# honglianghe/CDNet

Measured on AMD Instinct MI355X. Metric: tiles/sec (train fwd+bwd+Adam), 256x256, higher is better.
Workload: dtype fp32

## Files before the change

cdnet_amd/_lib.py:

```python
import ctypes as C
import os

_HERE = os.path.dirname(os.path.abspath(__file__))
LIB_PATH = os.environ.get('CDNET_LIB_PATH') or os.path.join(_HERE, 'libcdnet_hip.so')

_vp, _i, _sz, _f, _u = C.c_void_p, C.c_int, C.c_size_t, C.c_float, C.c_uint

class WgradReduceDesc(C.Structure):
    _fields_ = [('slab', C.c_void_p), ('dw', C.c_void_p)] + [(n, C.c_int) for n in (
        'ksplit', 'npar', 'ci_blocks', 'co_blocks', 'taps', 'CI', 'CO', 'Csrc_real', 'Cin_real', 'src_coff', 'Cout', 'mode', 'block0', 'blocks')]

class DilatedConvArgs(C.Structure):
    _fields_ = [(n, C.c_void_p) for n in ('in_', 'w', 'scale', 'shift', 'out')] + [(n, C.c_int) for n in (
        'N', 'H', 'W', 'Cin', 'in_cstride', 'Cout', 'out_cstride', 'out_coff', 'taps', 'dilation', 'leaky')] + [
        ('slope', C.c_float), ('f32', C.c_int), ('out_nchw', C.c_int)]

class DilatedBwdDataArgs(C.Structure):
    _fields_ = [(n, C.c_void_p) for n in ('g', 'w', 'dx')] + [(n, C.c_int) for n in (
        'N', 'H', 'W', 'Cout', 'g_cstride', 'Cin', 'dx_cstride', 'dx_coff', 'taps', 'dilation', 'accumulate', 'f32')]

class DilatedWgradArgs(C.Structure):
    _fields_ = [(n, C.c_void_p) for n in ('x', 'g', 'dw', 'ws')] + [('ws_bytes', C.c_size_t)] + [(n, C.c_int) for n in (
        'N', 'H', 'W', 'Cin', 'x_cstride', 'Cout', 'g_cstride', 'taps', 'dilation')]

class SliceBnFwdArgs(C.Structure):
    _fields_ = [(n, C.c_void_p) for n in ('z', 'out', 'gamma', 'beta', 'running_mean', 'running_var', 'mean', 'invstd', 'ws')] + [
        ('ws_floats', C.c_size_t), ('P', C.c_longlong)] + [(n, C.c_int) for n in ('C', 'z_cstride', 'out_cstride', 'out_coff')] + [
        (n, C.c_float) for n in ('eps', 'momentum', 'p_drop')] + [('layer', C.c_int), ('key', C.c_ulonglong)]

class SliceBnBwdArgs(C.Structure):
    _fields_ = [(n, C.c_void_p) for n in ('dy', 'z', 'mean', 'invstd', 'gamma', 'dgamma', 'dbeta', 'g', 'ws')] + [
        ('ws_floats', C.c_size_t), ('P', C.c_longlong)] + [(n, C.c_int) for n in ('C', 'z_cstride', 'dy_cstride', 'dy_coff', 'g_cstride')] + [
        (n, C.c_float) for n in ('slope', 'p_drop')] + [('layer', C.c_int), ('key', C.c_ulonglong)]


SIGNATURES = {
    'cdnet_abi_version': (_i, []),
    'cdnet_abi_sizeof': (_sz, [C.c_char_p]),
    'cdnet_last_error': (C.c_char_p, []),
    'cdnet_build_info': (C.c_char_p, []),
    'cdnet_spin': (_i, [_i, _vp]),
    'cdnet_box_copy': (_i, [_vp, _vp, _sz, _vp]),
    'cdnet_box_mfma': (_i, [_vp, _vp, _vp, _i, _i, _i, _vp]),
    'cdnet_ddm_codes': (_i, [_vp, _i, _i, _i, _i, _vp, _i, _i, _vp, _vp, _vp]),
    'cdnet_ddm_normalize': (_i, [_vp, _vp, _i, _i, _i, _vp, _vp]),
    'cdnet_probmaps': (_i, [_vp, _vp, _i, _i, _i, _i, _vp, _vp, _vp]),
    'cdnet_tta_boost_argmax': (_i, [_vp, _vp, _vp, _vp, _i, _i, _vp, _i, _i, _vp, _vp, _vp, _vp, _vp, _vp]),
    'cdnet_fuse_sum': (_i, [_vp, _i, _i, _i, _i, _i, _i, _vp, _i, _i, _vp]),
    'cdnet_upsample_bilinear_backward': (_i, [_vp, _i, _i, _i, _i, _i, _i, _i, _i, _vp, _vp]),
    'cdnet_s2d_to_nhwc': (_i, [_vp, _i, _i, _i, _i, _vp, _vp]),
    'cdnet_fuse_sum_f32': (_i, [_vp, _i, _i, _i, _i, _i, _i, _vp, _i, _i, _vp]),
    'cdnet_upsample_bilinear_backward_f32': (_i, [_vp, _i, _i, _i, _i, _i, _i, _i, _i, _vp, _vp]),
    'cdnet_s2d_to_nhwc_f32': (_i, [_vp, _i, _i, _i, _i, _vp, _vp]),
    'cdnet_bn_backward_stats': (_i, [_vp, _vp, _vp, _vp, _vp, _sz, _vp, _vp]),
    'cdnet_bn_backward_apply': (_i, [_vp, _vp, _vp, _vp]),
    'cdnet_bn_backward_finalize': (_i, [_vp, _vp, _vp, _vp, _vp, _i, _vp, _vp]),
    'cdnet_conv_ws_eligible': (_i, [_vp]),
    'cdnet_grad_sum': (_i, [_vp, _i, _vp, C.c_longlong, _i, _vp, _vp]),
    'cdnet_grad_sum_f32': (_i, [_vp, _i, _vp, C.c_longlong, _i, _vp, _vp]),
    'cdnet_label_pair_histogram': (_i, [_vp, _vp, _i, _i, _i, _i, _vp, _vp, _vp, _vp, _vp, _vp]),
    'cdnet_remap_label': (_i, [_vp, _i, _i, _i, _vp, _vp, _vp, _vp]),
    'cdnet_label_areas': (_i, [_vp, _i, _i, _i, _vp, _vp, _vp]),
    'cdnet_label_apply': (_i, [_vp, _i, _i, _i, _vp, _vp, _vp]),
    'cdnet_label_csr_workspace_bytes': (_sz, [_i]),
    'cdnet_label_csr': (_i, [_vp, _i, _i, _i, _vp, _sz, _vp, _vp, _vp, _vp, _vp]),
    'cdnet_hausdorff_tile_pixels': (_i, []),
    'cdnet_hausdorff_chunk_pixels': (_i, []),
    'cdnet_hausdorff_pairs': (_i, [_vp] * 8 + [_i, _i, _i, _vp, _i, _vp, _i, _vp, _vp, _vp]),
    'cdnet_watershed_workspace_bytes': (_sz, [_i, _i, _i]),
    'cdnet_watershed_process': (_i, [_vp, _i, _i, _i, _i, _vp, _sz, _vp, _vp, _vp, _vp]),
    'cdnet_fill_label_process': (_i, [_vp, _i, _i, _i, _i, _vp, _sz, _vp, _vp]),
    'cdnet_label_process': (_i, [_vp, _i, _i, _i, _i, _vp, _sz, _vp, _vp]),
    'cdnet_instance_redilate_workspace_bytes': (_sz, [_i, _i, _i, _i]),
    'cdnet_instance_redilate': (_i, [_vp, _i, _i, _i, _i, _i, _vp, _sz, _vp, _vp, _vp]),
    'cdnet_instance_redilate_lds_rows': (_i, []),
    'cdnet_instance_redilate_lds_cols': (_i, []),
    'cdnet_label_count': (_i, [_vp, _i, _i, _i, _vp, _vp, _vp, _vp]),
    'cdnet_tile_postproc_workspace_bytes': (_sz, [_i, _i, _i, _i]),
    'cdnet_tile_postproc': (_i, [_vp, _vp, _vp, _i, _i, _i, _i, _vp, _i, _i, _i, _i, _vp, _sz] + [_vp] * 10),
    'cdnet_cc_workspace_bytes': (_sz, [_i, _i, _i]),
    'cdnet_cc_chain': (_i, [_vp, _i, _i, _i, _i, _i, _i, _vp, _sz, _vp, _vp, _vp, _vp, _vp, _vp]),
    'cdnet_mask_views_argmax': (_i, [_vp, _i, _i, _i, _vp, _i, _i, _vp, _vp, _vp]),
    'cdnet_tile_mask_postproc_workspace_bytes': (_sz, [_i, _i, _i, _i]),
    'cdnet_tile_mask_postproc': (_i, [_vp, _i, _i, _i, _i, _i, _i, _vp, _sz] + [_vp] * 8),
    'cdnet_dilate_labels': (_i, [_vp, _i, _i, _i, _i, _vp, _vp]),
    'cdnet_conv_packed_weight_elems': (_sz, [_i] * 6),
    'cdnet_pack_conv_weights': (_i, [_vp, _vp] + [_i] * 7 + [_vp]),
    'cdnet_pack_conv_weights_scaled': (_i, [_vp, _vp, _vp] + [_i] * 7 + [_vp]),
    'cdnet_pack_batch_table_bytes': (_sz, [_i]),
    'cdnet_pack_conv_weights_batch': (_i, [_vp, _i, _vp, _sz, _i, _vp]),
    'cdnet_conv_forward': (_i, [_vp, _vp]),
    'cdnet_dilated_packed_weight_elems': (_sz, [_i, _i, _i, _i]),
    'cdnet_dilated_pack_weights': (_i, [_vp, _vp, _i, _i, _i, _i, _vp]),
    'cdnet_dilated_conv_forward': (_i, [_vp, _vp]),
    'cdnet_dilated_pack_weights_bwd': (_i, [_vp, _vp, _i, _i, _i, _i, _vp]),
    'cdnet_dilated_conv_backward_data': (_i, [_vp, _vp]),
    'cdnet_dilated_wgrad_workspace_bytes': (_sz, [_i] * 6),
    'cdnet_dilated_conv_backward_weight': (_i, [_vp, _vp]),
    'cdnet_slice_bn_workspace_floats': (_sz, [C.c_longlong, _i]),
    'cdnet_slice_bn_train_forward': (_i, [_vp, _vp]),
    'cdnet_slice_bn_train_backward': (_i, [_vp, _vp]),
    'cdnet_dropout_mask': (_i, [C.c_ulonglong, _i, _sz, _f, _vp, _vp]),
    'cdnet_src_materialize': (_i, [_vp, _i, _i, _i, _vp, _vp]),
    'cdnet_input_pack': (_i, [_vp, _i, _i, _i, _i, _vp, _vp]),
    'cdnet_input_pack_f32': (_i, [_vp, _i, _i, _i, _i, _vp, _vp]),
    'cdnet_bn_fold_eval': (_i, [_vp, _vp, _vp, _vp, _vp, _f, _i, _vp, _vp, _vp]),
    'cdnet_bn_finalize_train': (_i, [_vp, _i, _i, _f, _vp, _vp, _vp, _f, _f, _vp, _vp, _vp, _vp, _vp, _vp, _vp]),
    'cdnet_dam_head_forward': (_i, [_vp, _vp, _vp, _vp, _i, _i, _i, _vp, _vp, _vp, _vp]),
    'cdnet_final_conv1x1': (_i, [_vp, _vp, _vp, _i, _i, _i, _i, _vp, _vp]),
    'cdnet_bias_grad_workspace_floats': (_sz, [_i]),
    'cdnet_bias_grad': (_i, [_vp, _sz, _i, _vp, _sz, _vp, _vp]),
    'cdnet_bias_grad_f32': (_i, [_vp, _sz, _i, _vp, _sz, _vp, _vp]),
    'cdnet_final_conv1x1_backward_workspace_floats': (_sz, []),
    'cdnet_final_conv1x1_backward': (_i, [_vp, _vp, _vp, _i, _i, _i, _i, _vp, _vp, _sz, _vp, _vp, _vp]),
    'cdnet_conv_wgrad_slab_floats': (_sz, [_i] * 6),
    'cdnet_conv_backward_weight': (_i, [_vp, _i, _i, _i, _vp] + [_i] * 9 + [_vp, _vp, _i, _vp]),
    'cdnet_conv_backward_weight_last_form': (_i, []),
    'cdnet_wgrad_reduce_desc_fill': (_i, [_i] * 9 + [_vp, _vp, _i, _i, _vp]),
    'cdnet_wgrad_reduce_batch': (_i, [_vp, _i, _i, _vp]),
    'cdnet_bn_backward_workspace_floats': (_sz, [_i]),
    'cdnet_bn_backward': (_i, [_vp, _vp, _vp, _vp, _vp, _sz, _vp, _vp, _vp]),
    'cdnet_dam_head_backward_workspace_floats': (_sz, [_i, _i, _i]),
    'cdnet_dam_head_backward': (_i, [_vp] * 7 + [_i, _i, _i, _vp, _vp, _vp, _vp, _sz, _vp, _vp]),
    'cdnet_dam_head_backward_fused_blocks': (_i, []),
    'cdnet_dam_head_backward_fused_scratch_bytes': (_i, []),
    'cdnet_dam_head_backward_fused_workspace_floats': (_sz, []),
    'cdnet_dam_head_backward_fused': (_i, [_vp] * 7 + [_i, _i, _i, _vp, _vp, _vp, _vp, _sz, _vp, _vp]),
    'cdnet_dam_loss_workspace_floats': (_sz, [_i, _i]),
    'cdnet_dam_loss': (_i, [_vp] * 7 + [_i, _i, _i, _i, _vp, _sz, _vp, _vp, _vp, _vp, _vp]),
    'cdnet_dam_loss_classes_workspace_floats': (_sz, [_i, _i, _i]),
    'cdnet_dam_loss_classes': (_i, [_vp] * 7 + [_i, _i, _i, _i, _i, _vp, _sz, _vp, _vp, _vp, _vp, _vp]),
    'cdnet_dam_loss_terms': (_i, [_vp] * 7 + [_i, _i, _i, _i, _i, _vp, _sz, _vp, _vp, _vp, _vp, _vp, _u]),
    'cdnet_mask_loss_workspace_floats': (_sz, [_i, _i]),
    'cdnet_mask_loss': (_i, [_vp, _vp, _vp, _i, _i, _i, _u, _vp, _sz, _vp, _vp, _vp]),
    'cdnet_variance_loss_workspace_bytes': (_sz, [_i, _i, _i, _i]),
    'cdnet_variance_loss': (_i, [_vp, _vp, _i, _i, _i, _i, _i, _f, _vp, _sz, _vp, _vp, _vp, _vp, _vp, _vp]),
    'cdnet_boundary_loss_workspace_bytes': (_sz, [_i, _i, _i, _i, _i]),
    'cdnet_boundary_loss': (_i, [_vp, _vp, _i, _i, _i, _i, _i, _f, _vp, _sz, _vp, _vp, _vp, _vp]),
    'cdnet_boundary_loss_scratch_bytes': (_i, []),
    'cdnet_dam_val_sums_workspace_floats': (_sz, [_i, _i]),
    'cdnet_dam_val_sums': (_i, [_vp] * 8 + [_i, _i, _i, _vp, _sz, _vp, _vp]),
    'cdnet_dam_val_sums_classes_workspace_floats': (_sz, [_i, _i, _i]),
    'cdnet_dam_val_sums_classes': (_i, [_vp] * 8 + [_i, _i, _i, _i, _vp, _sz, _vp, _vp]),
    'cdnet_adam_step': (_i, [_vp, _vp, _vp, _vp, _sz, _f, _f, _f, _f, _f, _i, _f, _vp]),
    'cdnet_moment_step': (_i, [_vp, _vp, _vp, _vp, _vp, _sz, C.c_double, C.c_double, _f, _i, _i, _f, _f, _f, _f, _i, _f, _vp]),
    'cdnet_sgd_step': (_i, [_vp, _vp, _vp, _sz, _f, _f, _f, _i, _f, _vp]),
    'cdnet_window_pack': (_i, [_vp] + [_i] * 9 + [_vp, _vp]),
    'cdnet_window_pack_f32': (_i, [_vp] + [_i] * 9 + [_vp, _vp]),
    'cdnet_window_stitch': (_i, [_vp] + [_i] * 9 + [_vp, _vp]),
    'cdnet_label_encoding_workspace_bytes': (_sz, [_i, _i, _i, _i]),
    'cdnet_label_encoding_instances_workspace_bytes': (_sz, [_i, _i, _i, _i]),
    'cdnet_label_encoding_instances': (_i, [_vp, _i, _i, _i, _i, _vp, _vp, _vp, _sz, _vp, _vp, _vp, _vp, _vp, _vp]),
    'cdnet_augment_workspace_bytes': (_sz, [_i, _i, _i]),
    'cdnet_augment_batch': (_i, [_vp, _vp, _i, _i, _vp, _vp, _sz, _vp, _vp, _vp, _i, _vp, _vp, _vp]),
    'cdnet_augment_geo_workspace_bytes': (_sz, [_i, _i, _i, _i]),
    'cdnet_augment_batch_geo': (_i, [_vp, _vp, _vp, _vp, _i, _i, _i, _vp, _vp, _sz, _vp, _vp, _vp, _i, _vp, _vp, _vp]),
    'cdnet_label_encoding': (_i, [_vp, _i, _i, _i, _i, _vp, _vp, _vp, _sz, _vp, _vp, _vp, _vp, _vp, _vp]),
    'cdnet_weight_map_radius': (_i, [C.c_double, C.c_double]),
    'cdnet_weight_map': (_i, [_vp, _i, _i, C.c_double, C.c_double, _vp, _vp]),
}

_lib = None


class CdnetHipError(RuntimeError):
    pass


def load():
    global _lib
    if _lib is not None:
        return _lib
    import torch
    if not os.path.exists(LIB_PATH):
        raise CdnetHipError('libcdnet_hip.so is not built: run `python -m cdnet_amd.csrc.build` '
                            '(or __graft_entry__.build()). There is no CPU fallback.')
    lib = C.CDLL(LIB_PATH)
    for name, (res, args) in SIGNATURES.items():
        fn = getattr(lib, name)
        fn.restype = res
        fn.argtypes = args
    if lib.cdnet_abi_version() != 5:
        raise CdnetHipError('ABI version mismatch (libcdnet_hip.so is version %d, this binding 5): rebuild with python -m cdnet_amd.csrc.build' % lib.cdnet_abi_version())
    _lib = lib
    return lib


def check(status, what=''):
    if status != 0:
        msg = load().cdnet_last_error().decode(errors='replace')
        raise CdnetHipError('%s failed (code %d): %s' % (what, status, msg))


def call(name, *args):
    check(getattr(load(), name)(*args), name)


def entry(name, f32):
    return name + '_f32' if f32 else name


_RAW_STREAM = None


def stream_ptr():
    global _RAW_STREAM
    if _RAW_STREAM is None:
        import torch
        get, dev = getattr(torch._C, '_cuda_getCurrentRawStream', None), getattr(torch._C, '_cuda_getDevice', None)
        if get is not None and dev is not None:
            _RAW_STREAM = lambda: get(dev())
        else:
            _RAW_STREAM = lambda: torch.cuda.current_stream().cuda_stream
    return C.c_void_p(_RAW_STREAM())


def ptr(t):
    if t is None:
        return None
    assert t.is_cuda and t.is_contiguous(), 'ABI needs contiguous device tensors'
    return C.c_void_p(t.data_ptr())
```

cdnet_amd/csrc/bn_bwd.hip:

```cpp
#include "train_util.h"
#include "bn_sums.h"

using namespace cdnet;

namespace {

struct GradIn {
    const unsigned short *g;
    int Hg, Wg;
    int oy, ox;
    int pooled;
    int coff, cstride;
};

struct BnBwdArgs {
    const unsigned short *raw;
    const unsigned short *res;
    int f16;
    const float *scale, *shift;
    int relu;
    const float *mean, *invstd;
    GradIn gin[3];
    int ngin;
    int N, H, W, C;
// ... 356 lines not shown
                if (RES) v = outmask ? r[u][j] : v + r[u][j];
                float gs = g[u][0][j];
#pragma unroll
                for (int k = 1; k < NG; ++k) gs += g[u][k][j];
                const float dz = (!valid || (relu && !(v > 0.f))) ? 0.f : gs;
                const float xh = (x[u][j] - mu[j]) * is[j];
                if (APPLY) { o[j] = k1[j] * (dz - k2[j] - xh * k3[j]); z[j] = dz; }
                else { s1[j] += dz; s2[j] = fmaf(dz, xh, s2[j]); z[j] = dz; }
            }
            if (APPLY && valid) {
                const unsigned pw = A.rev ? npix - 1 - p : p;
                *reinterpret_cast<f32x4 *>(draw + (size_t)pw * A.C + c0) = o;
                if (RES) *reinterpret_cast<f32x4 *>(dzo + (size_t)pw * A.C + c0) = z;
            }
            if (!APPLY && RES && dzo && valid) *reinterpret_cast<f32x4 *>(dzo + (size_t)p * A.C + c0) = z;
        }
    }
    if (!APPLY) bn_write_partial<4>(A.partial, A.C, VPP, s1, s2);
}

template <int NF, bool APPLY>
__global__ __launch_bounds__(256) void bn_bwd_window32_kernel(BnBwdArgs A, int kp) {
    const int VPP = A.C / 4;
    const int slot = (int)threadIdx.x % VPP, c0 = slot * 4;
    float sc[4], sh[4], mu[4], is[4], k1[4], k2[4], k3[4], s1[4], s2[4];
    bn_load_const(A, c0, APPLY, sc, sh, mu, is, k1, k2, k3);
#pragma unroll
    for (int j = 0; j < 4; ++j) { s1[j] = 0.f; s2[j] = 0.f; }
    const unsigned H = A.H, W = A.W, Hp = (H + 1) / 2, Wp = (W + 1) / 2, nwin = (unsigned)A.N * Hp * Wp;
    const unsigned ppb = 256 / VPP;
    const bool relu = A.relu != 0;
    const GradIn gp = A.gin[kp];
    const float *gpool_p = reinterpret_cast<const float *>(gp.g);
    const float *raw = reinterpret_cast<const float *>(A.raw);
    float *draw = reinterpret_cast<float *>(A.draw);
    const float *gf[NF > 0 ? NF : 1];
    int gcs[NF > 0 ? NF : 1], gco[NF > 0 ? NF : 1];
    {
        int m = 0;
        for (int k = 0; k < A.ngin && m < NF; ++k)
            if (k != kp) { gf[m] = reinterpret_cast<const float *>(A.gin[k].g); gcs[m] = A.gin[k].cstride; gco[m] = A.gin[k].coff; ++m; }
    }
    for (unsigned w0 = first_pixel(ppb, VPP); w0 < nwin; w0 += gridDim.x * ppb) {
        const unsigned w = (APPLY && A.rev) ? nwin - 1 - w0 : w0;
        const unsigned n = w / (Hp * Wp), r = w - n * Hp * Wp;
        const unsigned py = r / Wp, px = r - py * Wp;
        f32x4 x[4], g[4][NF > 0 ? NF : 1], gv;
        unsigned pix[4];
        bool ok[4];
#pragma unroll
        for (int q = 0; q < 4; ++q) {
            unsigned yy = 2 * py + (q >> 1), xx = 2 * px + (q & 1);
            ok[q] = yy < H && xx < W;
            yy = yy < H ? yy : H - 1;
            xx = xx < W ? xx : W - 1;
            pix[q] = (n * H + yy) * W + xx;
            x[q] = *reinterpret_cast<const f32x4 *>(raw + (size_t)pix[q] * A.C + c0);
#pragma unroll
            for (int m = 0; m < NF; ++m)
                g[q][m] = *reinterpret_cast<const f32x4 *>(gf[m] + (size_t)pix[q] * gcs[m] + gco[m] + c0);
        }
        const bool pok = py < (unsigned)gp.Hg && px < (unsigned)gp.Wg;
        {
            const unsigned cy = pok ? py : 0, cx = pok ? px : 0;
            gv = *reinterpret_cast<const f32x4 *>(gpool_p + (((size_t)n * gp.Hg + cy) * gp.Wg + cx) * gp.cstride + gp.coff + c0);
        }
        f32x4 o[4];
#pragma unroll
        for (int j = 0; j < 4; ++j) {
            float a[4];
#pragma unroll
            for (int q = 0; q < 4; ++q) {
                const float v = fmaf(x[q][j], sc[j], sh[j]);
                a[q] = relu ? fmaxf(v, 0.f) : v;
            }
            int bi = 0;
            float best = a[0];
#pragma unroll
            for (int q = 1; q < 4; ++q)
                if (ok[q] && a[q] > best) { best = a[q]; bi = q; }
            const float gpool = pok ? gv[j] : 0.f;
#pragma unroll
            for (int q = 0; q < 4; ++q) {
                const float pt = (bi == q) ? gpool : 0.f;
                float gsum;
                if (NF == 0) gsum = 0.f + pt;
                else if (NF == 1) gsum = (0.f + (kp == 0 ? pt : g[q][0][j])) + (kp == 0 ? g[q][0][j] : pt);
                else gsum = ((0.f + (kp == 0 ? pt : g[q][0][j])) + (kp == 0 ? g[q][0][j] : (kp == 1 ? pt : g[q][NF - 1][j]))) +
                            (kp == 2 ? pt : g[q][NF - 1][j]);
                const float dz = (!ok[q] || (relu && !(a[q] > 0.f))) ? 0.f : gsum;
                const float xh = (x[q][j] - mu[j]) * is[j];
                if (APPLY) o[q][j] = k1[j] * (dz - k2[j] - xh * k3[j]);
                else { s1[j] += dz; s2[j] = fmaf(dz, xh, s2[j]); }
            }
        }
        if (APPLY) {
#pragma unroll
            for (int q = 0; q < 4; ++q)
                if (ok[q]) *reinterpret_cast<f32x4 *>(draw + (size_t)pix[q] * A.C + c0) = o[q];
        }
    }
    if (!APPLY) bn_write_partial<4>(A.partial, A.C, VPP, s1, s2);
}

template <bool F32, bool APPLY>
__global__ __launch_bounds__(256) void bn_bwd_generic_kernel(BnBwdArgs A) {
    const int VPP = A.C / 8;
    const int slot = (int)threadIdx.x % VPP, c0 = slot * 8;
    float sc[8], sh[8], mu[8], is[8], k1[8], k2[8], k3[8], s1[8], s2[8];
    bn_load_const(A, c0, APPLY, sc, sh, mu, is, k1, k2, k3);
#pragma unroll
    for (int j = 0; j < 8; ++j) { s1[j] = 0.f; s2[j] = 0.f; }
    const unsigned HW = (unsigned)(A.H * A.W), npix = (unsigned)A.N * HW;
    const unsigned ppb = 256 / VPP;
    const unsigned step = gridDim.x * ppb;
    for (unsigned p0 = first_pixel(ppb, VPP); p0 < npix; p0 += step * BN_U) {
        float dz[BN_U][8], xh[BN_U][8];
#pragma unroll
        for (int u = 0; u < BN_U; ++u) {
            const unsigned p = p0 + u * step;
            if (p < npix) dz8_at<F32>(A, p, HW, c0, sc, sh, mu, is, dz[u], xh[u]);
            else if (!APPLY) {
#pragma unroll
                for (int j = 0; j < 8; ++j) { dz[u][j] = 0.f; xh[u][j] = 0.f; }
            }
        }
#pragma unroll
        for (int u = 0; u < BN_U; ++u) {
            const unsigned p = p0 + u * step;
            if (!APPLY) {
#pragma unroll
                for (int j = 0; j < 8; ++j) { s1[j] += dz[u][j]; s2[j] = fmaf(dz[u][j], xh[u][j], s2[j]); }
                continue;
            }
            if (p >= npix) continue;
            float o32[8];
#pragma unroll
            for (int j = 0; j < 8; ++j) o32[j] = k1[j] * (dz[u][j] - k2[j] - xh[u][j] * k3[j]);
            if (F32) {
                if (A.draw) stf8(A.draw, (size_t)p * A.C + c0, o32);
                if (A.dz_out) stf8(A.dz_out, (size_t)p * A.C + c0, dz[u]);
                continue;
            }
            V16 o, z;
#pragma unroll
            for (int j = 0; j < 8; ++j) { o.h[j] = f2bf(o32[j]); z.h[j] = f2bf(dz[u][j]); }
            if (A.draw) *reinterpret_cast<uint4 *>(A.draw + (size_t)p * A.C + c0) = o.u;
            if (A.dz_out) *reinterpret_cast<uint4 *>(A.dz_out + (size_t)p * A.C + c0) = z.u;
        }
    }
    if (!APPLY) bn_write_partial<8>(A.partial, A.C, VPP, s1, s2);
}

__global__ __launch_bounds__(256) void bn_bwd_finalize_kernel(const float *__restrict__ partial, int nb, int C, float M, const float *gamma,
                                                              const float *invstd, float *dgamma, float *dbeta, float *k1, float *k2,
                                                              float *k3) {
    const int c = blockIdx.x;
    double s1, s2;
    bn_sum_partials(partial, nb, C, c, s1, s2);
    if (threadIdx.x == 0) {
        if (dbeta) dbeta[c] = (float)s1;
        if (dgamma) dgamma[c] = (float)s2;
        k1[c] = gamma[c] * invstd[c];
        k2[c] = (float)(s1 / M);
        k3[c] = (float)(s2 / M);
    }
}

__global__ void bn_ktab_copy_kernel(const float *scale, const float *shift, const float *mean, const float *invstd, int C, float *ktab) {
    const int c = blockIdx.x * blockDim.x + threadIdx.x;
    if (c < C) { ktab[c] = scale[c]; ktab[C + c] = shift[c]; ktab[2 * C + c] = mean[c]; ktab[3 * C + c] = invstd[c]; }
}

}

static int fill_bn_args(const cdnet_bn_bwd_args *a, BnBwdArgs &A, const char *who) {
    CDNET_REQUIRE(a && a->raw, "%s: null pointer", who);
    CDNET_REQUIRE(a->C % 8 == 0 && a->C >= 8 && a->C <= 2048 , "%s: C=%d unsupported", who, a->C);
    CDNET_REQUIRE(a->ngin >= 1 && a->ngin <= 3, "%s: ngin=%d", who, a->ngin);
    A.raw = a->raw; A.res = a->res; A.f16 = a->f16; A.scale = a->scale; A.shift = a->shift; A.relu = a->relu;
    A.mean = a->mean; A.invstd = a->invstd;
    for (int k = 0; k < 3; ++k) {
        A.gin[k].g = a->gin[k].g; A.gin[k].Hg = a->gin[k].Hg; A.gin[k].Wg = a->gin[k].Wg;
        A.gin[k].oy = a->gin[k].oy; A.gin[k].ox = a->gin[k].ox; A.gin[k].pooled = a->gin[k].pooled;
        A.gin[k].coff = a->gin[k].coff; A.gin[k].cstride = a->gin[k].cstride ? a->gin[k].cstride : a->C;
        if (k < a->ngin) CDNET_REQUIRE(a->gin[k].g, "%s: null gradient input %d", who, k);
    }
    A.ngin = a->ngin; A.N = a->N; A.H = a->H; A.W = a->W; A.C = a->C;
    A.partial = nullptr; A.k1 = A.k2 = A.k3 = nullptr; A.draw = nullptr; A.dz_out = nullptr;
    return CDNET_OK;
}

enum BnPath { BN_WINDOW, BN_FLAT, BN_GENERIC };
struct BnPlan {
    BnPath path;
    bool f32;
    int nb;
    int kp, nflat;
    bool flat_sources;
};

static size_t bn_npix(const BnBwdArgs &A) { return (size_t)A.N * A.H * A.W; }

static BnPlan bn_plan_plain(const BnBwdArgs &A) {
    const bool f32 = A.f16 == 2;
    return BnPlan{BN_FLAT, f32, bn_grid(bn_npix(A), A.C, f32 ? 4 : 8, BN_U), 0, 0, true};
}

static BnPlan bn_plan(const BnBwdArgs &A, const void *draw, const void *dz_out) {
    bool simple = true;
    int npool = 0, kp = 0, nflat = 0;
    for (int k = 0; k < A.ngin; ++k) {
        const GradIn &g = A.gin[k];
        const bool same = !g.pooled && g.oy == 0 && g.ox == 0 && g.Hg == A.H && g.Wg == A.W;
        simple = simple && same;
        if (g.pooled) { ++npool; kp = k; }
        else if (same) ++nflat;
    }
    const bool window = npool == 1 && nflat == A.ngin - 1 && nflat <= 2 && A.mean && A.scale && !A.res && draw && !dz_out;
    const bool flat = !window && simple && A.mean && A.scale && draw && ((A.res != nullptr) == (dz_out != nullptr));
    const bool f32 = A.f16 == 2, fits32 = A.C <= 1024;
    BnPlan P{BN_GENERIC, f32, 0, kp, nflat, flat};
    if (window && (!f32 || (fits32 && A.shift && A.invstd))) P.path = BN_WINDOW;
    else if (flat && (!f32 || fits32)) P.path = BN_FLAT;
    const int V = f32 && P.path != BN_GENERIC ? 4 : 8;
    P.nb = window ? bn_grid((size_t)A.N * ((A.H + 1) / 2) * ((A.W + 1) / 2), A.C, V, 1) : bn_grid(bn_npix(A), A.C, V, BN_U);
    return P;
}

template <bool APPLY>
static void launch(const BnPlan &P, const BnBwdArgs &A, hipStream_t st) {
    auto window = [&](auto nf) {
        constexpr int NF = decltype(nf)::value;
        if (P.f32) bn_bwd_window32_kernel<NF, APPLY><<<P.nb, 256, 0, st>>>(A, P.kp);
        else bn_bwd_window_kernel<NF, APPLY><<<P.nb, 256, 0, st>>>(A, P.kp);
    };
    auto flat = [&](auto ng, auto res) {
        constexpr int NG = decltype(ng)::value;
        constexpr bool RES = decltype(res)::value;
        if (P.f32) bn_bwd_flat32_kernel<NG, RES, APPLY><<<P.nb, 256, 0, st>>>(A);
        else bn_bwd_flat_kernel<NG, RES, APPLY><<<P.nb, 256, 0, st>>>(A);
    };
    using std::integral_constant;
    using std::true_type;
    using std::false_type;
    switch (P.path) {
        case BN_WINDOW:
            if (P.nflat == 0) window(integral_constant<int, 0>{});
            else if (P.nflat == 1) window(integral_constant<int, 1>{});
            else window(integral_constant<int, 2>{});
            break;
        case BN_FLAT:
            switch (A.ngin * 2 + (A.res ? 1 : 0)) {
                case 2: flat(integral_constant<int, 1>{}, false_type{}); break;
                case 3: flat(integral_constant<int, 1>{}, true_type{}); break;
                case 4: flat(integral_constant<int, 2>{}, false_type{}); break;
                case 5: flat(integral_constant<int, 2>{}, true_type{}); break;
                case 6: flat(integral_constant<int, 3>{}, false_type{}); break;
                default: flat(integral_constant<int, 3>{}, true_type{}); break;
            }
            break;
        case BN_GENERIC:
            if (P.f32) bn_bwd_generic_kernel<true, APPLY><<<P.nb, 256, 0, st>>>(A);
            else bn_bwd_generic_kernel<false, APPLY><<<P.nb, 256, 0, st>>>(A);
            break;
    }
}

static void bn_finalize(const BnBwdArgs &A, const float *partial, int nb, const float *gamma, float *dgamma, float *dbeta, float *k,
                        hipStream_t st) {
    bn_bwd_finalize_kernel<<<A.C, 256, 0, st>>>(partial, nb, A.C, (float)bn_npix(A), gamma, A.invstd, dgamma, dbeta, k, k + A.C, k + 2 * A.C);
}

static void bn_set_coeffs(BnBwdArgs &A, const float *k) { A.k1 = k; A.k2 = k + A.C; A.k3 = k + 2 * A.C; }

static BnBwdArgs bn_dz_as_source(const BnBwdArgs &A, const unsigned short *dz) {
    BnBwdArgs B = A;
    B.ngin = 1;
    B.gin[0].g = dz; B.gin[0].Hg = A.H; B.gin[0].Wg = A.W; B.gin[0].oy = 0; B.gin[0].ox = 0; B.gin[0].pooled = 0;
    B.gin[0].coff = 0; B.gin[0].cstride = A.C;
    B.res = nullptr; B.relu = 0; B.dz_out = nullptr;
    return B;
}

extern "C" int cdnet_bn_backward(const cdnet_bn_bwd_args *a, const float *gamma, float *dgamma, float *dbeta, float *workspace,
                                 size_t workspace_floats, uint16_t *draw, uint16_t *dz_out, void *stream) {
    BnBwdArgs A;
    int rc = fill_bn_args(a, A, "cdnet_bn_backward");
    if (rc) return rc;
    hipStream_t st = (hipStream_t)stream;
    const size_t npix = bn_npix(A);
    CDNET_REQUIRE(npix * (size_t)A.C < ((size_t)1 << 32) && npix < ((size_t)1 << 31), "cdnet_bn_backward: tensor too large for 32-bit pixel indexing");
    const BnPlan P = bn_plan(A, draw, dz_out);
    CDNET_REQUIRE(A.relu != 2 || (P.flat_sources && A.res), "cdnet_bn_backward: relu = 2 (mask from the stored output) needs same-size gradient sources and res");
    static const bool dz_reuse = !(getenv("CDNET_BN_DZ_REUSE") && atoi(getenv("CDNET_BN_DZ_REUSE")) == 0);
    const bool reuse = dz_reuse && P.path == BN_FLAT && A.mean && A.res && dz_out;
    A.draw = draw;
    A.rev = 1;
    if (A.mean) {
        CDNET_REQUIRE(gamma && A.invstd && workspace, "cdnet_bn_backward: BatchNorm layer needs gamma/invstd/workspace");
        const size_t need = (size_t)P.nb * 2 * A.C + 3 * (size_t)A.C;
        if (workspace_floats < need) { set_error("cdnet_bn_backward: workspace %zu < %zu floats", workspace_floats, need); return CDNET_E_WORKSPACE; }
        A.partial = workspace;
        A.dz_out = dz_reuse ? dz_out : nullptr;
        float *k = workspace + (size_t)P.nb * 2 * A.C;
        launch<false>(P, A, st);
        bn_finalize(A, A.partial, P.nb, gamma, dgamma, dbeta, k, st);
        bn_set_coeffs(A, k);
    }
    A.dz_out = dz_out;
    launch<true>(P, reuse ? bn_dz_as_source(A, dz_out) : A, st);
    return check_launch("cdnet_bn_backward");
}

static bool bn_plain_case(const BnBwdArgs &A, bool masked = false) {
    const GradIn &g = A.gin[0];
    return A.ngin == 1 && !g.pooled && g.oy == 0 && g.ox == 0 && g.Hg == A.H && g.Wg == A.W && A.mean && A.scale && A.shift && A.invstd && !A.res &&
           (A.relu == 1 || (masked && A.relu == 0)) && (g.cstride == 0 || g.cstride == A.C) && g.coff == 0;
}

extern "C" int cdnet_bn_backward_stats(const cdnet_bn_bwd_args *a, const float *gamma, float *dgamma, float *dbeta, float *workspace,
                                       size_t workspace_floats, float *ktab, void *stream) {
    BnBwdArgs A;
    int rc = fill_bn_args(a, A, "cdnet_bn_backward_stats");
    if (rc) return rc;
    CDNET_REQUIRE(bn_plain_case(A) && A.f16 != 2 && gamma && workspace && ktab, "cdnet_bn_backward_stats: plain 16-bit case only (one same-size gradient, BatchNorm + ReLU, no residual)");
    hipStream_t st = (hipStream_t)stream;
    const size_t npix = bn_npix(A);
    CDNET_REQUIRE(npix * (size_t)A.C < ((size_t)1 << 32) && npix < ((size_t)1 << 31), "cdnet_bn_backward_stats: tensor too large for 32-bit pixel indexing");
    const BnPlan P = bn_plan_plain(A);
    const size_t need = (size_t)P.nb * 2 * A.C;
    if (workspace_floats < need) { set_error("cdnet_bn_backward_stats: workspace %zu < %zu floats", workspace_floats, need); return CDNET_E_WORKSPACE; }
    A.partial = workspace;
    A.rev = 0;
    bn_ktab_copy_kernel<<<cdiv(A.C, 256), 256, 0, st>>>(A.scale, A.shift, A.mean, A.invstd, A.C, ktab);
    launch<false>(P, A, st);
    bn_finalize(A, A.partial, P.nb, gamma, dgamma, dbeta, ktab + 4 * A.C, st);
    return check_launch("cdnet_bn_backward_stats");
}

extern "C" int cdnet_bn_backward_finalize(const cdnet_bn_bwd_args *a, const float *gamma, float *dgamma, float *dbeta, const float *partial,
                                          int nb, float *ktab, void *stream) {
    BnBwdArgs A;
    int rc = fill_bn_args(a, A, "cdnet_bn_backward_finalize");
    if (rc) return rc;
    CDNET_REQUIRE(bn_plain_case(A) && gamma && partial && ktab && nb >= 1, "cdnet_bn_backward_finalize: plain case only");
    bn_finalize(A, partial, nb, gamma, dgamma, dbeta, ktab + 4 * A.C, (hipStream_t)stream);
    return check_launch("cdnet_bn_backward_finalize");
}

extern "C" int cdnet_bn_backward_apply(const cdnet_bn_bwd_args *a, const float *ktab, uint16_t *draw, void *stream) {
    BnBwdArgs A;
    int rc = fill_bn_args(a, A, "cdnet_bn_backward_apply");
    if (rc) return rc;
    CDNET_REQUIRE(bn_plain_case(A, true) && ktab && draw, "cdnet_bn_backward_apply: plain case only");
    CDNET_REQUIRE(A.f16 != 2 || A.C <= 1024, "cdnet_bn_backward_apply(f32): C=%d > 1024", A.C);
    A.rev = 1;
    A.draw = draw;
    bn_set_coeffs(A, ktab + 4 * A.C);
    launch<true>(bn_plan_plain(A), A, (hipStream_t)stream);
    return check_launch("cdnet_bn_backward_apply");
}

extern "C" size_t cdnet_bn_backward_workspace_floats(int C) { return (size_t)BN_MAX_BLOCKS * 2 * C + 3 * (size_t)C; }
```

cdnet_amd/csrc/bn_sums.h:

```cpp
#pragma once
#include <hip/hip_runtime.h>

namespace cdnet {

__device__ __forceinline__ void bn_sum_partials(const float *__restrict__ part, int T, int C, int c, double &s, double &q) {
    __shared__ double s_s[256], s_q[256];
    const int lane = threadIdx.x;
    s = 0.0; q = 0.0;
    for (int t = lane; t < T; t += 256) {
        s += (double)part[((size_t)t * 2) * C + c];
        q += (double)part[((size_t)t * 2 + 1) * C + c];
    }
    s_s[lane] = s; s_q[lane] = q;
    __syncthreads();
#pragma unroll
    for (int o = 128; o > 0; o >>= 1) {
        if (lane < o) { s_s[lane] += s_s[lane + o]; s_q[lane] += s_q[lane + o]; }
        __syncthreads();
    }
    s = s_s[0]; q = s_q[0];
}

}
```

cdnet_amd/csrc/conv.hip:

```cpp
#include <type_traits>
#include <vector>
#include "common.h"
#include "conv_args.h"
#include "launch.h"
#include "xform.h"
#include "stage16.h"
#include <stdlib.h>

using namespace cdnet;

namespace {

__device__ int g_dbg_dummy;

struct PackDesc {
    const float *w;
    unsigned short *out;
    int Cout, Cin, KH, KW, CK, BN, nchunk, ntile, TAPS, mode, parity;
    unsigned block0, nblocks;
    int split;
    const float *scale;
};

__device__ __forceinline__ void pack_range(const PackDesc &d, size_t first, size_t stride) {
    const float *__restrict__ w = d.w;
    unsigned short *__restrict__ out = d.out;
    const int Cout = d.Cout, Cin = d.Cin, KH = d.KH, KW = d.KW, CK = d.CK, BN = d.BN, nchunk = d.nchunk, TAPS = d.TAPS, mode = d.mode,
              parity = d.parity;
    const size_t total = (size_t)d.ntile * nchunk * TAPS * (CK / 16) * 2 * BN * (d.split ? 2 : 1);
    for (size_t i = first; i < total; i += stride) {
        size_t r = i;
        int tap = r % TAPS; r /= TAPS;
        int col = r % BN; r /= BN;
        int half = r % 2; r /= 2;
        int kc = r % (CK / 16); r /= (CK / 16);
        int hl = 0;
        if (d.split) { hl = r % 2; r /= 2; }
        int chunk = r % nchunk; r /= nchunk;
        int tile = (int)r;
        int co = tile * BN + col;
        const size_t ovec = ((((((size_t)tile * nchunk + chunk) * (d.split ? 2 : 1) + hl) * TAPS + tap) * (CK / 16) + kc) * 2 + half) * BN + col;
        unsigned short o8[8];
#pragma unroll
        for (int j = 0; j < 8; ++j) {
        int ci = chunk * CK + kc * 16 + half * 8 + j;
        float v = 0.f;
        if (co < Cout && ci < Cin) {
            if (mode == 0) {
                v = w[(((size_t)co * Cin + ci) * KH + tap / KW) * KW + tap % KW];
            } else if (mode == 1) {
                int kh = KH - 1 - tap / KW, kw = KW - 1 - tap % KW;
                v = w[(((size_t)ci * Cout + co) * KH + kh) * KW + kw];
            } else if (mode == 2) {
                int a = parity >> 1, b = parity & 1, ty = tap >> 1, tx = tap & 1;
                int kh = a == 0 ? (ty == 0 ? 1 : 3) : (ty == 0 ? 0 : 2);
                int kw = b == 0 ? (tx == 0 ? 1 : 3) : (tx == 0 ? 0 : 2);
                v = w[(((size_t)ci * Cout + co) * 4 + kh) * 4 + kw];
            } else if (mode == 3) {
                int a = parity >> 1, b = parity & 1;
                v = w[(((size_t)ci * Cout + co) * 2 + a) * 2 + b];
            } else if (mode == 7) {
                const int Ct = Cout / 4;
                const int a = co / (2 * Ct), b = (co / Ct) & 1, c = co % Ct;
                const int tf = 8 - tap;
                const int kh = 2 * (tf / 3 - 1) + a + 1, kw = 2 * (tf % 3 - 1) + b + 1;
                if (kh >= 0 && kh < 3 && kw >= 0 && kw < 3) v = w[(((size_t)ci * Ct + c) * 3 + kh) * 3 + kw];
            } else {
                const int Ct = Cin / 4;
                const int a = ci / (2 * Ct), b = (ci / Ct) & 1, c = ci % Ct;
                if (mode == 4) {
                    const int kh = 2 * (tap / 3) + a - 1, kw = 2 * (tap % 3) + b - 1;
                    if (kh >= 0 && kh < 4 && kw >= 0 && kw < 4) v = w[(((size_t)co * Ct + c) * 4 + kh) * 4 + kw];
                } else if (mode == 5) {
                    v = w[(((size_t)co * Ct + c) * 2 + a) * 2 + b];
                } else {
                    const int kh = 2 * (tap / 3 - 1) + a + 1, kw = 2 * (tap % 3 - 1) + b + 1;
                    if (kh >= 0 && kh < 3 && kw >= 0 && kw < 3) v = w[(((size_t)co * Ct + c) * 3 + kh) * 3 + kw];
                }
            }
        }
        if (d.scale && co < Cout) v *= d.scale[co];
        const unsigned short hi = f2bf(v);
        o8[j] = hl ? f2bf(v - bf2f(hi)) : hi;
        }
        uint4 ov;
        ov.x = o8[0] | ((unsigned)o8[1] << 16); ov.y = o8[2] | ((unsigned)o8[3] << 16);
        ov.z = o8[4] | ((unsigned)o8[5] << 16); ov.w = o8[6] | ((unsigned)o8[7] << 16);
        reinterpret_cast<uint4 *>(out)[ovec] = ov;
    }
}

__global__ void pack_weights_kernel(PackDesc d) {
    pack_range(d, (size_t)blockIdx.x * blockDim.x + threadIdx.x, (size_t)gridDim.x * blockDim.x);
}

__global__ void pack_weights_batch_kernel(const PackDesc *__restrict__ table, int n) {
    int lo = 0, hi = n - 1;
    while (lo < hi) {
        const int mid = (lo + hi + 1) >> 1;
        if (table[mid].block0 <= blockIdx.x) lo = mid; else hi = mid - 1;
    }
    const PackDesc d = table[lo];
    pack_range(d, (size_t)(blockIdx.x - d.block0) * blockDim.x + threadIdx.x, (size_t)d.nblocks * blockDim.x);
}

__device__ __forceinline__ V16 max8(V16 a, V16 b, bool nonneg) {
    V16 o;
    if (nonneg) {
        o.u = __builtin_bit_cast(uint4, xf_max_nonneg_bf8(__builtin_bit_cast(u32x4, a.u), __builtin_bit_cast(u32x4, b.u)));
        return o;
    }
#pragma unroll
    for (int j = 0; j < 8; ++j) o.h[j] = bf2f(a.h[j]) >= bf2f(b.h[j]) ? a.h[j] : b.h[j];
    return o;
}

constexpr int XF_MAX = 2048;

__device__ __forceinline__ void load_chan_xf(ChanXf &t, const ConvSrc &s, const float *xf, int xfs, int c) {
    t.on = s.scale != nullptr;
    if (!t.on) return;
    const float4 *ps = reinterpret_cast<const float4 *>(xf ? xf + c : s.scale + c);
    const float4 *ph = reinterpret_cast<const float4 *>(xf ? xf + xfs + c : s.shift + c);
    float4 a = ps[0], b = ps[1], cc = ph[0], d = ph[1];
    t.sc[0] = a.x; t.sc[1] = a.y; t.sc[2] = a.z; t.sc[3] = a.w; t.sc[4] = b.x; t.sc[5] = b.y; t.sc[6] = b.z; t.sc[7] = b.w;
    t.sh[0] = cc.x; t.sh[1] = cc.y; t.sh[2] = cc.z; t.sh[3] = cc.w; t.sh[4] = d.x; t.sh[5] = d.y; t.sh[6] = d.z; t.sh[7] = d.w;
}

template <int TH, int CK>
struct HaloImg {
    static constexpr bool SWZ = (TH == 16 && CK == 16);
    static constexpr int PSTR = SWZ ? CK * 2 : CK * 2 + 16;
    __device__ __forceinline__ static int off(int pix, int hy, int slot) { return pix * PSTR + (SWZ ? ((slot ^ (hy & 1)) * 16) : slot * 16); }
};

template <int TH, int TW, int CK>
__device__ __forceinline__ void stage_input(const ConvSrc &s, int cc0, int n, int y0, int x0, int H, int W,
                                            unsigned char *lds_a, int tid, const float *xf = nullptr, int xfs = 0) {
    constexpr int VPP = CK / 8;
    constexpr int HW_ = TW + 2, NPIX = (TH + 2) * (TW + 2);
    const int slot = tid % VPP;
    ChanXf t;
    load_chan_xf(t, s, xf, xfs, cc0 + slot * 8);
    const bool relu = s.relu != 0;
    const bool f16 = s.f16 != 0;
    const bool plain = !t.on && !relu && s.res == nullptr && !f16;
    const int Hl = s.pool ? (s.Hs + (s.pool == 2)) / 2 : s.Hs, Wl = s.pool ? (s.Ws + (s.pool == 2)) / 2 : s.Ws;
    const size_t rs = s.row_stride ? (size_t)s.row_stride : (size_t)s.Ws * s.C;
    const size_t img = (size_t)n * s.Hs * rs;
    for (int v = tid; v < NPIX * VPP; v += 256) {
        const int pix = v / VPP;
        const int hy = pix / HW_, hx = pix - hy * HW_;
        const int y = y0 - 1 + hy, x = x0 - 1 + hx;
        V16 val;
        val.u = make_uint4(0, 0, 0, 0);
        const int ys = y - s.off_y, xs = x - s.off_x;
        if (y >= 0 && y < H && x >= 0 && x < W && ys >= 0 && ys < Hl && xs >= 0 && xs < Wl) {
            if (!s.pool) {
                const size_t e = img + (size_t)ys * rs + (size_t)xs * s.C + cc0 + slot * 8;
                V16 raw;
                raw.u = *reinterpret_cast<const uint4 *>(s.x + e);
                if (plain) val = raw;
                else if (s.res) { V16 r; r.u = *reinterpret_cast<const uint4 *>(s.res + e); val = xform8(raw, &r, t, relu, f16); }
                else val = xform8(raw, nullptr, t, relu, f16);
            } else {
#pragma unroll
                for (int q = 0; q < 4; ++q) {
                    const int yy = 2 * ys + (q >> 1), xx = 2 * xs + (q & 1);
                    if (q != 0 && (yy >= s.Hs || xx >= s.Ws)) continue;
                    const size_t e = img + (size_t)yy * rs + (size_t)xx * s.C + cc0 + slot * 8;
                    V16 raw;
                    raw.u = *reinterpret_cast<const uint4 *>(s.x + e);
                    V16 tv = plain ? raw : xform8(raw, nullptr, t, relu, f16);
                    val = q == 0 ? tv : max8(val, tv, relu);
                }
            }
        }
        *reinterpret_cast<uint4 *>(lds_a + HaloImg<TH, CK>::off(pix, hy, slot)) = val.u;
    }
}

#ifndef CDNET_CONV_XCD
#define CDNET_CONV_XCD 1
#endif
#ifndef CDNET_CONV_GLDS
#define CDNET_CONV_GLDS 1
#endif
#ifndef CDNET_CONV_ADEPTH
#define CDNET_CONV_ADEPTH 1
#endif
template <int TH, int TW, int CK, int BN, int TAPS>
struct ConvLds {
    static constexpr bool DEEP = (CK == 16 && TH == 16);
    static constexpr bool GLDS = CDNET_CONV_GLDS && DEEP;
    static constexpr int ADEPTH = DEEP ? CDNET_CONV_ADEPTH : 1;
    static constexpr int PSTR = HaloImg<TH, CK>::PSTR;
    static constexpr int A_BYTES = (TH + 2) * (TW + 2) * PSTR;
    static constexpr int B_BYTES = TAPS * CK * BN * 2;
    static constexpr int STAGE = A_BYTES + (GLDS ? 2 : 1) * B_BYTES;
    static constexpr int OUT_BYTES = TH * TW * (BN * 2 + 8);
    static constexpr int STATS_BYTES = 4 * 2 * BN * 4;
    static constexpr int MAIN = ((STAGE > OUT_BYTES + STATS_BYTES ? STAGE : OUT_BYTES + STATS_BYTES) + 15) / 16 * 16;
    static int bytes(int ctot) { return MAIN + 2 * ((ctot + 7) / 8 * 8) * 4; }
};

template <int TH, int TW, int CK, int BN, int TAPS>
struct Prefetch {
    static constexpr int VPP = CK / 8;
    static constexpr int NPIX = (TH + 2) * (TW + 2);
    static constexpr int NA = (NPIX * VPP + 255) / 256;
    static constexpr bool GLDS = ConvLds<TH, TW, CK, BN, TAPS>::GLDS;
    static constexpr int NB = (TAPS * CK * BN * 2 / 16 + 255) / 256;
    static constexpr int ADEPTH = ConvLds<TH, TW, CK, BN, TAPS>::ADEPTH;
    struct ASlot {
        uint4 a[NA];
        unsigned valid;
        bool pooled;
    };
    ASlot s[ADEPTH];
    uint4 b[GLDS ? 1 : NB];
    int eoff[2][NA];
    unsigned tvalid[2];
};

template <int SI, int TH, int TW, int CK, int BN, int TAPS>
__device__ __forceinline__ void prep_source(Prefetch<TH, TW, CK, BN, TAPS> &P, const ConvSrc &s, int y0, int x0, int H, int W, int tid) {
    using PF = Prefetch<TH, TW, CK, BN, TAPS>;
    constexpr int HW_ = TW + 2;
    const int slot = tid % PF::VPP;
    const int rs = s.row_stride ? s.row_stride : s.Ws * s.C;
    P.tvalid[SI] = 0;
#pragma unroll
    for (int i = 0; i < PF::NA; ++i) {
        const int v = tid + i * 256;
        const int pix = v / PF::VPP;
        const int hy = pix / HW_, hx = pix - hy * HW_;
        const int y = y0 - 1 + hy, x = x0 - 1 + hx;
        const int ys = y - s.off_y, xs = x - s.off_x;
        const bool inr = v < PF::NPIX * PF::VPP;
        const bool ok = inr && (unsigned)y < (unsigned)H && (unsigned)x < (unsigned)W && (unsigned)ys < (unsigned)s.Hs && (unsigned)xs < (unsigned)s.Ws;
        P.eoff[SI][i] = ok ? ys * rs + xs * s.C + slot * 8 : -1;
// ... 870 lines not shown
    };
    auto serial_epilogue = [&](const f32x16 (&P)[MPW][NPW], int j) {
        const int par = j & 1;
        if (STATS) {
#pragma unroll
            for (int u = 0; u < NU; ++u) stat_unit(P, u, par);
            stats_tile = t_lo + j;
            stats_par = par;
        }
#pragma unroll
        for (int u = 0; u < NU; ++u) img_unit(P, u);
    };

    __syncthreads();
    tile_step(F_{}, accA, accB, 0);
    int j = 1;
    for (; j + 1 < ntl; j += 2) {
        tile_step(T_{}, accB, accA, j);
        tile_step(T_{}, accA, accB, j + 1);
    }
    if (j < ntl) {
        tile_step(T_{}, accB, accA, j);
        serial_epilogue(accB, j);
    } else {
        serial_epilogue(accA, ntl - 1);
    }
    __syncthreads();
    flush_stats();
#ifdef CDNET_WS_STAMPS
    if (stamp_on) { for (int i = 0; i < sn; ++i) g_ws_stamps[i] = s_stamp[i]; g_ws_stamps[sn] = 0; }
#endif
}

template <int BN, int TAPS>
int try_launch_conv_ws(const ConvArgs &A, hipStream_t st, bool dry_run = false) {
    using L = WsLds<BN, TAPS>;
    int ctot = 0;
    if (A.ws == 2) return -1;
    if (A.eres) return -1;
    if (A.nchunk < 4 || A.nchunk % 4 != 0) return -1;
    if ((A.src[0].C / 16) & 1) return -1;
    const bool stream = A.nchunk != 4;
    if (A.H % 16 != 0 || A.W % 16 != 0) return -1;
    for (int i = 0; i < A.nsrc; ++i) {
        if (A.src[i].pool || A.src[i].relu == 3) return -1;
        ctot += A.src[i].C;
        if (!in_mover_reach(A.src[i], (long long)A.N * A.npar, 2)) return -1;
    }
#ifdef CDNET_WS_STAMPS
    const int smem = L::bytes(4, ctot, 2) + 2 * 384 * 8;
#else
    const int smem = L::bytes(4, ctot, 2);
#endif
    if (smem > 160 * 1024) return -1;
    const int T = (A.W / 16) * (A.H / 16) * A.N;
    int n_cu = 0;
    if (const int rc = cu_count(&n_cu)) return rc;
    const int ctiles = cdiv(A.Cout, BN);
    const int Gmax = n_cu / ctiles > 0 ? n_cu / ctiles : 1;
    if (!(A.debug & CONV_DBG_PERSIST_SMALL) && ((long long)T * A.nchunk < 12LL * Gmax || (T < Gmax && A.nchunk < 16))) return -1;
    bool all_plain = true, all_fast = true;
    for (int i = 0; i < A.nsrc; ++i) {
        const ConvSrc &s = A.src[i];
        all_plain = all_plain && !s.scale && !s.relu && !s.res && !s.f16;
        all_fast = all_fast && s.scale && s.relu && !s.res && s.f16 == 1;
    }
    dim3 grid(persistent_grid(n_cu, ctiles, T, 0, 0), ctiles, 1);
    const int xf = all_plain ? 0 : (all_fast ? 1 : 2);
    if (dry_run) return CDNET_OK;
    return with_bool(A.stats != nullptr, [&](auto st_c) {
        return with_int<0, 1, 2>(xf, [&](auto xf_c) {
            return with_bool(stream, [&](auto sm_c) {
                return launch_lds<conv_ws_kernel<BN, TAPS, decltype(xf_c)::value, decltype(st_c)::value, decltype(sm_c)::value>>(
                    grid, 512, 160 * 1024, smem, st, "hipFuncSetAttribute(conv_ws)", "conv_ws_kernel", A);
            });
        });
    });
}

template <int TAPS>
int dispatch_conv(const ConvArgs &A, hipStream_t st) {
    const int key = A.tile * 10000 + A.CK * 100 + (A.BN == 128 ? 99 : A.BN);
    switch (key) {
        case 16 * 10000 + 16 * 100 + 32: return launch_conv<16, 16, 16, 32, 4, 1, TAPS>(A, st);
        case 16 * 10000 + 16 * 100 + 64: return launch_conv<16, 16, 16, 64, 4, 1, TAPS>(A, st);
        case 16 * 10000 + 32 * 100 + 32: return launch_conv<16, 16, 32, 32, 4, 1, TAPS>(A, st);
        case 16 * 10000 + 32 * 100 + 64: return launch_conv<16, 16, 32, 64, 4, 1, TAPS>(A, st);
        case 16 * 10000 + 32 * 100 + 99: return launch_conv<16, 16, 32, 128, 2, 2, TAPS>(A, st);
        case 16 * 10000 + 64 * 100 + 64: return launch_conv<16, 16, 64, 64, 4, 1, TAPS>(A, st);
        case 8 * 10000 + 32 * 100 + 64: return launch_conv<8, 8, 32, 64, 2, 2, TAPS>(A, st);
        case 8 * 10000 + 32 * 100 + 99: return launch_conv<8, 8, 32, 128, 2, 2, TAPS>(A, st);
        case 8 * 10000 + 64 * 100 + 64: return launch_conv<8, 8, 64, 64, 2, 2, TAPS>(A, st);
        default:
            set_error("cdnet_conv: unsupported configuration tile=%d CK=%d BN=%d", A.tile, A.CK, A.BN);
            return CDNET_E_ARG;
    }
}

__global__ __launch_bounds__(256) void materialize_kernel(const ConvSrc s, int N, int H, int W, unsigned short *__restrict__ out) {
    const int VPP = s.C / 8;
    const size_t total = (size_t)N * H * W * VPP;
    const bool relu = s.relu != 0, f16 = s.f16 != 0;
    const int Hl = s.pool ? (s.Hs + (s.pool == 2)) / 2 : s.Hs, Wl = s.pool ? (s.Ws + (s.pool == 2)) / 2 : s.Ws;
    const size_t rs = s.row_stride ? (size_t)s.row_stride : (size_t)s.Ws * s.C;
    for (size_t i = (size_t)blockIdx.x * 256 + threadIdx.x; i < total; i += (size_t)gridDim.x * 256) {
        const int slot = (int)(i % VPP);
        const size_t pix = i / VPP;
        const int x = (int)(pix % W), y = (int)((pix / W) % H), n = (int)(pix / ((size_t)W * H));
        ChanXf t;
        load_chan_xf(t, s, nullptr, 0, slot * 8);
        const bool plain = !t.on && !relu && s.res == nullptr && !f16;
        const size_t img = (size_t)n * s.Hs * rs;
        V16 val;
        val.u = make_uint4(0, 0, 0, 0);
        const int ys = y - s.off_y, xs = x - s.off_x;
        if (ys >= 0 && ys < Hl && xs >= 0 && xs < Wl) {
            if (!s.pool) {
                const size_t e = img + (size_t)ys * rs + (size_t)xs * s.C + slot * 8;
                V16 raw;
                raw.u = *reinterpret_cast<const uint4 *>(s.x + e);
                if (plain) val = raw;
                else if (s.res) { V16 r; r.u = *reinterpret_cast<const uint4 *>(s.res + e); val = xform8(raw, &r, t, relu, f16); }
                else val = xform8(raw, nullptr, t, relu, f16);
            } else {
                V16 raw[4];
                bool ok[4];
#pragma unroll
                for (int q = 0; q < 4; ++q) {
                    int yy = 2 * ys + (q >> 1), xx = 2 * xs + (q & 1);
                    ok[q] = q == 0 || (yy < s.Hs && xx < s.Ws);
                    yy = yy < s.Hs ? yy : s.Hs - 1;
                    xx = xx < s.Ws ? xx : s.Ws - 1;
                    raw[q].u = *reinterpret_cast<const uint4 *>(s.x + img + (size_t)yy * rs + (size_t)xx * s.C + slot * 8);
                }
#pragma unroll
                for (int q = 0; q < 4; ++q) {
                    const V16 tv = plain ? raw[q] : xform8(raw[q], nullptr, t, relu, f16);
                    val = q == 0 ? tv : (ok[q] ? max8(val, tv, relu) : val);
                }
            }
        }
        *reinterpret_cast<uint4 *>(out + pix * s.C + slot * 8) = val.u;
    }
}

}

extern "C" size_t cdnet_conv_packed_weight_elems(int Cout, int Cin_padded_chunks, int taps, int CK, int BN, int npar) {
    return (size_t)npar * cdiv(Cout, BN) * Cin_padded_chunks * taps * CK * BN;
}

static int fill_pack_desc(PackDesc &d, const float *w, void *packed, int Cout, int Cin, int KH, int KW, int CK, int BN, int mode, int p,
                          const char *who) {
    const int split = (mode & 16) ? 1 : 0;
    mode &= 15;
    CDNET_REQUIRE(w && packed, "%s: null pointer", who);
    CDNET_REQUIRE(CK % 16 == 0 && BN % 32 == 0 && Cin % CK == 0 && mode >= 0 && mode <= 7, "%s: Cin=%d CK=%d BN=%d mode=%d", who, Cin, CK, BN, mode);
    const int taps = mode == 2 ? 4 : (mode == 3 ? 1 : ((mode == 4 || mode == 6 || mode == 7) ? 9 : (mode == 5 ? 1 : KH * KW)));
    const int nchunk = Cin / CK, ntile = cdiv(Cout, BN);
    const size_t per = (size_t)ntile * nchunk * taps * CK * BN * (split ? 2 : 1);
    d.split = split;
    d.scale = nullptr;
    d.w = w; d.out = (unsigned short *)packed + (size_t)p * per;
    d.Cout = Cout; d.Cin = Cin; d.KH = KH; d.KW = KW; d.CK = CK; d.BN = BN; d.nchunk = nchunk; d.ntile = ntile; d.TAPS = taps; d.mode = mode;
    d.parity = p;
    d.block0 = 0;
    d.nblocks = (unsigned)((per + 2047) / 2048);
    if (d.nblocks > 4096) d.nblocks = 4096;
    return CDNET_OK;
}

extern "C" int cdnet_pack_conv_weights(const float *w, void *packed, int Cout, int Cin, int KH, int KW, int CK, int BN,
                                       int mode, void *stream) {
    const int npar = ((mode & 15) == 2 || (mode & 15) == 3) ? 4 : 1;
    for (int p = 0; p < npar; ++p) {
        PackDesc d;
        int rc = fill_pack_desc(d, w, packed, Cout, Cin, KH, KW, CK, BN, mode, p, "cdnet_pack_conv_weights");
        if (rc) return rc;
        pack_weights_kernel<<<d.nblocks, 256, 0, (hipStream_t)stream>>>(d);
    }
    return check_launch("cdnet_pack_conv_weights");
}

extern "C" int cdnet_pack_conv_weights_scaled(const float *w, const float *cout_scale, void *packed, int Cout, int Cin, int KH, int KW, int CK,
                                              int BN, int mode, void *stream) {
    CDNET_REQUIRE(cout_scale && (mode & 15) == 0, "cdnet_pack_conv_weights_scaled: forward Conv2d packs (mode 0) with a scale vector");
    PackDesc d;
    int rc = fill_pack_desc(d, w, packed, Cout, Cin, KH, KW, CK, BN, mode, 0, "cdnet_pack_conv_weights_scaled");
    if (rc) return rc;
    d.scale = cout_scale;
    pack_weights_kernel<<<d.nblocks, 256, 0, (hipStream_t)stream>>>(d);
    return check_launch("cdnet_pack_conv_weights_scaled");
}

extern "C" size_t cdnet_pack_batch_table_bytes(int n_jobs) { return (size_t)n_jobs * 4 * sizeof(PackDesc); }

extern "C" int cdnet_pack_conv_weights_batch(const cdnet_pack_job *jobs, int n_jobs, void *table, size_t table_bytes, int upload,
                                             void *stream) {
    CDNET_REQUIRE(jobs && n_jobs > 0 && table, "cdnet_pack_conv_weights_batch: null pointer / no jobs");
    CDNET_REQUIRE(table_bytes >= cdnet_pack_batch_table_bytes(n_jobs), "cdnet_pack_conv_weights_batch: table too small");
    static thread_local std::vector<PackDesc> host;
    host.clear();
    unsigned blocks = 0;
    for (int j = 0; j < n_jobs; ++j) {
        const cdnet_pack_job &J = jobs[j];
        const int npar = ((J.mode & 15) == 2 || (J.mode & 15) == 3) ? 4 : 1;
        for (int p = 0; p < npar; ++p) {
            PackDesc d;
            int rc = fill_pack_desc(d, J.w, J.packed, J.Cout, J.Cin, J.KH, J.KW, J.CK, J.BN, J.mode, p, "cdnet_pack_conv_weights_batch");
            if (rc) return rc;
            d.block0 = blocks;
            blocks += d.nblocks;
            host.push_back(d);
        }
    }
    hipStream_t st = (hipStream_t)stream;
    if (upload) {
        if (hipMemcpyAsync(table, host.data(), host.size() * sizeof(PackDesc), hipMemcpyHostToDevice, st) != hipSuccess ||
            hipStreamSynchronize(st) != hipSuccess)
            return check_launch("cdnet_pack_conv_weights_batch(upload)");
    }
    pack_weights_batch_kernel<<<blocks, 256, 0, st>>>((const PackDesc *)table, (int)host.size());
    return check_launch("cdnet_pack_conv_weights_batch");
}

extern "C" int cdnet_conv_forward(const cdnet_conv_args *args, void *stream) {
    CDNET_REQUIRE(args, "cdnet_conv_forward: null args");
    const ConvArgs &A = *reinterpret_cast<const ConvArgs *>(args);
    CDNET_REQUIRE(A.nsrc >= 1 && A.nsrc <= 2 && A.w && (A.out || A.dot_out), "cdnet_conv_forward: bad pointers / nsrc=%d", A.nsrc);
    CDNET_REQUIRE(!A.dot_out || (A.dot_w && !A.f32 && !A.pool_out), "cdnet_conv_forward: dot_out needs dot_w, the 16-bit path and no pool_out");
    CDNET_REQUIRE(A.N > 0 && A.H > 0 && A.W > 0 && A.Cout > 0 && A.Cout % 8 == 0, "cdnet_conv_forward: bad size (Cout must be a multiple of 8)");
    {
        int ctot_xf = 0;
        for (int i = 0; i < A.nsrc; ++i) ctot_xf += A.src[i].C;
        CDNET_REQUIRE(ctot_xf <= XF_MAX, "cdnet_conv_forward: %d source channels exceed the %d-entry scale/shift table", ctot_xf, XF_MAX);
    }
    CDNET_REQUIRE(A.ws == 0 || A.ws == 2, "cdnet_conv_forward: ws must be 0 or 2 (BatchNorm-backward statistics epilogue)");
    if (A.f32) {
        CDNET_REQUIRE(A.f32 == 1, "cdnet_conv_forward: f32 must be 0 or 1");
        for (int i = 0; i < A.nsrc; ++i)
            CDNET_REQUIRE(A.src[i].f16 == 2, "cdnet_conv_forward(f32): every source must be fp32 (f16 = 2)");
    } else {
        for (int i = 0; i < A.nsrc; ++i)
            CDNET_REQUIRE(A.src[i].f16 == 0 || A.src[i].f16 == 1, "cdnet_conv_forward: fp32 sources need args.f32 = 1");
    }
    if (A.eres && A.ws != 2) {
        CDNET_REQUIRE(A.ostride == 1 && A.npar == 1 && A.out_coff == 0 && A.out_cstride == A.Cout && !A.stats && !A.orelu &&
                      !A.out_f16 && ((A.eres_scale == nullptr) == (A.eres_shift == nullptr)),
                      "cdnet_conv_forward: fused residual epilogue needs a dense bf16 output, no statistics and no ReLU before the add");
    }
    int nchunk = 0;
    for (int i = 0; i < A.nsrc; ++i) {
        CDNET_REQUIRE(A.src[i].x && A.src[i].C % A.CK == 0, "cdnet_conv_forward: source %d channels %d not a multiple of CK=%d",
                      i, A.src[i].C, A.CK);
        CDNET_REQUIRE(!(A.src[i].pool && A.src[i].res), "cdnet_conv_forward: pool+residual source unsupported");
        nchunk += A.src[i].C / A.CK;
    }
    const bool padded = A.nchunk == nchunk + 1 && A.taps == 9 && A.nsrc == 2 && !A.f32;
    CDNET_REQUIRE(nchunk == A.nchunk || padded, "cdnet_conv_forward: nchunk %d != %d", A.nchunk, nchunk);
    CDNET_REQUIRE((A.taps == 9 && A.npar == 1 && A.ostride == 1) || (A.taps == 1 && A.npar == 1 && A.ostride == 1) ||
                  (A.taps == 4 && A.npar == 4 && A.ostride == 2) || (A.taps == 1 && A.npar == 4 && A.ostride == 2),
                  "cdnet_conv_forward: taps=%d npar=%d ostride=%d", A.taps, A.npar, A.ostride);
    CDNET_REQUIRE(A.out_cstride % 8 == 0 && A.out_coff % 8 == 0, "cdnet_conv_forward: output channel slice must be 16-byte aligned");
    hipStream_t st = (hipStream_t)stream;
    CDNET_REQUIRE(A.taps1 == 0 || A.taps1 == A.taps || (A.taps1 == 1 && A.taps == 9 && A.nsrc == 2), "cdnet_conv_forward: taps1 = %d (0, taps, or 1 beside a nine-tap first source)", A.taps1);
    if (A.f32) return conv_forward_f32(A, st);
    {
        const int rc = conv_forward_ws16(A, st);
        if (rc >= 0) return rc;
        CDNET_REQUIRE(A.taps1 == 0 || A.taps1 == A.taps, "cdnet_conv_forward: a one-tap second source runs on conv_ws16_kernel only (ask cdnet_conv_ws_eligible)");
        CDNET_REQUIRE(!A.pool_out, "cdnet_conv_forward: the fused max-pool output needs conv_ws16_kernel's out-image form (ask cdnet_conv_ws_eligible)");
        CDNET_REQUIRE(!A.dot_out, "cdnet_conv_forward: the fused 1x1 classifier (dot_out) needs conv_ws16_kernel's out-image form with resident weights (ask cdnet_conv_ws_eligible)");
        CDNET_REQUIRE(!padded, "cdnet_conv_forward: a padding chunk (nchunk = real + 1) runs on conv_ws16_kernel only (ask cdnet_conv_ws_eligible)");
    }
    static const int dbg = getenv("CDNET_CONV_DEBUG") ? atoi(getenv("CDNET_CONV_DEBUG")) : 0;
    if (!(A.debug & CONV_DBG_ONE_TILE) && A.taps == 9 && A.npar == 1 && A.ostride == 1 && A.tile == 16 && A.CK == 16 && (A.BN == 64 || A.BN == 32)) {
        const int rc = A.BN == 64 ? try_launch_conv_ws<64, 9>(A, st) : try_launch_conv_ws<32, 9>(A, st);
        if (rc >= 0) return rc;
    }
    for (int i = 0; i < A.nsrc; ++i)
        CDNET_REQUIRE(A.src[i].relu >= 0 && A.src[i].relu <= 2, "cdnet_conv_forward: source %d: relu = %d (the BatchNorm-backward source of round 2, relu = 3, was removed)", i, A.src[i].relu);
    CDNET_REQUIRE(A.ws != 2, "cdnet_conv_forward: the BatchNorm-backward statistics epilogue (ws = 2) exists in fp32 mode on conv_ws32_kernel only "
                             "(ask cdnet_conv_ws_eligible first)");
    if (dbg) { ConvArgs B = A; B.debug = dbg; if (B.taps == 9) return dispatch_conv<9>(B, st); }
    if (A.debug & CONV_DBG_ONE_TILE) { ConvArgs B = A; B.debug = 0; if (B.taps == 9) return dispatch_conv<9>(B, st); if (B.taps == 4) return dispatch_conv<4>(B, st); return dispatch_conv<1>(B, st); }
    if (A.taps == 9) return dispatch_conv<9>(A, st);
    if (A.taps == 4) return dispatch_conv<4>(A, st);
    return dispatch_conv<1>(A, st);
}

extern "C" int cdnet_conv_ws_eligible(const cdnet_conv_args *args) {
    if (!args) return 0;
    const ConvArgs &A = *reinterpret_cast<const ConvArgs *>(args);
    if (A.f32) return (!A.dot_out && conv_forward_f32_ws(A, nullptr, true) == CDNET_OK) ? 1 : 0;
    if (conv_forward_ws16(A, nullptr, true) == CDNET_OK) return 2;
    if ((A.taps1 != 0 && A.taps1 != A.taps) || A.pool_out || A.dot_out) return 0;
    if (A.debug & CONV_DBG_ONE_TILE) return 0;
    if (!(A.taps == 9 && A.npar == 1 && A.ostride == 1 && A.tile == 16 && A.CK == 16 && (A.BN == 64 || A.BN == 32))) return 0;
    const int rc = A.BN == 64 ? try_launch_conv_ws<64, 9>(A, nullptr, true) : try_launch_conv_ws<32, 9>(A, nullptr, true);
    return rc == CDNET_OK ? 1 : 0;
}

extern "C" int cdnet_src_materialize(const cdnet_conv_src *src, int N, int H, int W, uint16_t *out, void *stream) {
    CDNET_REQUIRE(src && out && src->x && N > 0 && H > 0 && W > 0, "cdnet_src_materialize: bad args");
    const ConvSrc &s = *reinterpret_cast<const ConvSrc *>(src);
    CDNET_REQUIRE(s.C >= 8 && s.C % 8 == 0 && s.Hs > 0 && s.Ws > 0, "cdnet_src_materialize: C=%d must be a multiple of 8", s.C);
    CDNET_REQUIRE(!(s.pool && s.res), "cdnet_src_materialize: pooled sources carry no residual");
    CDNET_REQUIRE((s.scale == nullptr) == (s.shift == nullptr), "cdnet_src_materialize: scale and shift come together");
    if (s.f16 == 2) return materialize_f32(s, N, H, W, out, (hipStream_t)stream);
    const size_t total = (size_t)N * H * W * (s.C / 8);
    size_t g = (total + 255) / 256;
    g = g > 8192 ? 8192 : g;
    materialize_kernel<<<(int)g, 256, 0, (hipStream_t)stream>>>(s, N, H, W, out);
    return check_launch("cdnet_src_materialize");
}
```

cdnet_amd/csrc/dilated_train.hip:

```cpp
#include "common.h"
#include "bn_sums.h"
#include "launch.h"
#include "split_bf16.h"

using namespace cdnet;

namespace {

constexpr int STRIP = 32;
constexpr int ROW = 36;
constexpr int WG_WAVES = 4;
constexpr int WGRAD_WGS = 512;

__device__ __forceinline__ f32x4 load4(const float *p, bool ok, int c, int cend) {
    f32x4 v = {0.f, 0.f, 0.f, 0.f};
    if (ok && c < cend) {
        v = *reinterpret_cast<const f32x4 *>(p);
#pragma unroll
        for (int j = 0; j < 4; ++j) v[j] = c + j < cend ? v[j] : 0.f;
    }
    return v;
}

__device__ __forceinline__ void frag(const float *tile, int s, int h, int i, u32x4 &hi, u32x4 &lo) {
// ... 25 lines not shown
__global__ __launch_bounds__(WG_WAVES * 64) void dilated_wgrad_kernel(const cdnet_dilated_wgrad_args A, const WgradGeom G) {
    __shared__ __attribute__((aligned(16))) float s_g[STRIP * ROW];
    __shared__ __attribute__((aligned(16))) float s_x[WG_WAVES][STRIP * ROW];
    const int tid = threadIdx.x, lane = tid & 63, wave = tid >> 6, i = lane & 31, h = lane >> 5;
    const int co0 = blockIdx.z * 32, ci0 = ((int)blockIdx.y * WG_WAVES + wave) * 32;
    const bool live = ci0 < A.Cin;
    float *sx = s_x[wave];

    f32x16 acc[TAPS];
#pragma unroll
    for (int t = 0; t < TAPS; ++t)
#pragma unroll
        for (int r = 0; r < 16; ++r) acc[t][r] = 0.f;

    const int q0 = blockIdx.x * G.strips_per_slab;
    const int q1 = q0 + G.strips_per_slab < G.nstrips ? q0 + G.strips_per_slab : G.nstrips;
    for (int q = q0; q < q1; ++q) {
        const int x0 = (q % G.tiles_x) * STRIP, row = q / G.tiles_x, y = row % A.H, n = row / A.H;
        __syncthreads();
        {
            const int pp = tid >> 3, c = co0 + (tid & 7) * 4;
            const bool ok = x0 + pp < A.W;
            const size_t off = (((size_t)n * A.H + y) * A.W + (size_t)(ok ? x0 + pp : 0)) * (size_t)A.g_cstride + (size_t)(c < A.Cout ? c : 0);
            *reinterpret_cast<f32x4 *>(&s_g[pp * ROW + (tid & 7) * 4]) = load4(A.g + off, ok, c, A.Cout);
        }
        __syncthreads();
        u32x4 ah[2], al[2];
#pragma unroll
        for (int s = 0; s < 2; ++s) frag(s_g, s, h, i, ah[s], al[s]);
#pragma unroll
        for (int tap = 0; tap < TAPS; ++tap) {
            const long long dy = TAPS == 9 ? (long long)(tap / 3 - 1) * A.dilation : 0;
            const long long dx = TAPS == 9 ? (long long)(tap % 3 - 1) * A.dilation : 0;
            const long long yy = y + dy;
            long long lo = -(x0 + dx), hi = (long long)A.W - 1 - x0 - dx;
            if (lo < 0) lo = 0;
            if (hi > A.W - 1 - x0) hi = A.W - 1 - x0;
            if (hi > STRIP - 1) hi = STRIP - 1;
            if (yy < 0 || yy >= A.H || lo > hi) continue;
            if (live) {
#pragma unroll
                for (int k = 0; k < 4; ++k) {
                    const int idx = lane + 64 * k, pp = idx >> 3, c = ci0 + (idx & 7) * 4;
                    const long long px = x0 + pp + dx;
                    const bool ok = pp >= lo && pp <= hi;
                    const size_t off = (((size_t)n * A.H + (size_t)yy) * A.W + (size_t)(ok ? px : 0)) * (size_t)A.x_cstride + (size_t)(c < A.Cin ? c : 0);
                    *reinterpret_cast<f32x4 *>(&sx[pp * ROW + (idx & 7) * 4]) = load4(A.x + off, ok, c, A.Cin);
                }
            }
            __syncthreads();
            if (live) {
#pragma unroll
                for (int s = 0; s < 2; ++s) {
                    u32x4 bh, bl;
                    frag(sx, s, h, i, bh, bl);
                    const bf16x8 a_hi = __builtin_bit_cast(bf16x8, ah[s]), a_lo = __builtin_bit_cast(bf16x8, al[s]);
                    const bf16x8 b_hi = __builtin_bit_cast(bf16x8, bh), b_lo = __builtin_bit_cast(bf16x8, bl);
                    acc[tap] = mfma3(acc[tap], a_hi, a_lo, b_hi, b_lo);
                }
            }
        }
    }
    if (!live) return;
    float *slab = static_cast<float *>(A.ws) + (size_t)blockIdx.x * TAPS * G.CoP * G.CiP;
#pragma unroll
    for (int tap = 0; tap < TAPS; ++tap)
#pragma unroll
        for (int r = 0; r < 16; ++r) {
            const int co = co0 + (r & 3) + 8 * (r >> 2) + 4 * h;
            slab[((size_t)tap * G.CoP + co) * G.CiP + ci0 + i] = acc[tap][r];
        }
}

__global__ __launch_bounds__(256) void dilated_wgrad_reduce_kernel(const float *ws, float *dw, int Cin, int Cout, int taps, const WgradGeom G) {
    const size_t e = (size_t)blockIdx.x * blockDim.x + threadIdx.x, total = (size_t)Cout * Cin * taps;
    if (e >= total) return;
    const int tap = (int)(e % taps), ci = (int)((e / taps) % Cin), co = (int)(e / taps / Cin);
    const size_t per = (size_t)taps * G.CoP * G.CiP;
    const float *p = ws + ((size_t)tap * G.CoP + co) * G.CiP + ci;
    float s = 0.f;
    for (int k = 0; k < G.nslab; ++k) s += p[(size_t)k * per];
    dw[e] = s;
}

__host__ __device__ __forceinline__ unsigned long long mix64(unsigned long long z) {
    z = (z ^ (z >> 30)) * 0xBF58476D1CE4E5B9ull;
    z = (z ^ (z >> 27)) * 0x94D049BB133111EBull;
    return z ^ (z >> 31);
}

__host__ __device__ __forceinline__ unsigned long long layer_key(unsigned long long key, int layer) {
    return mix64(key + 0x9E3779B97F4A7C15ull * (unsigned long long)(unsigned)(layer + 1));
}

__host__ __device__ __forceinline__ unsigned drop_threshold(float p) { return (unsigned)(p * 16777216.0f); }

__device__ __forceinline__ bool keep(unsigned long long lkey, unsigned long long idx, unsigned thr) {
    return (unsigned)(mix64(lkey + 0x9E3779B97F4A7C15ull * (idx + 1)) >> 40) >= thr;
}

__global__ __launch_bounds__(256) void dropout_mask_kernel(unsigned long long lkey, size_t count, unsigned thr, uint8_t *mask) {
    for (size_t i = (size_t)blockIdx.x * blockDim.x + threadIdx.x; i < count; i += (size_t)gridDim.x * blockDim.x)
        mask[i] = keep(lkey, i, thr) ? 1 : 0;
}

constexpr int BN_TILES = 1024;

struct BnGeom { int T; long long tile; };

BnGeom bn_geom(long long P) {
    BnGeom G;
    long long T = (P + 63) / 64;
    if (T > BN_TILES) T = BN_TILES;
    G.tile = (P + T - 1) / T;
    G.T = (int)((P + G.tile - 1) / G.tile);
    return G;
}

template <bool BWD>
__global__ __launch_bounds__(256) void bn_tile_sums_kernel(const float *__restrict__ z, int zs, const float *__restrict__ dy, int dys, int dyo,
                                                           const float *__restrict__ mean, const float *__restrict__ invstd, long long P, int C,
                                                           long long tile, unsigned long long lkey, unsigned thr, float keep_scale,
                                                           float *__restrict__ part) {
    __shared__ float s_a[8][32], s_b[8][32];
    const int cl = threadIdx.x & 31, r = threadIdx.x >> 5, c = blockIdx.y * 32 + cl;
    const long long p0 = (long long)blockIdx.x * tile, p1 = p0 + tile < P ? p0 + tile : P;
    float a = 0.f, b = 0.f;
    if (c < C) {
        const float mu = BWD ? mean[c] : 0.f, is = BWD ? invstd[c] : 0.f;
        for (long long p = p0 + r; p < p1; p += 8) {
            const float v = z[(size_t)p * zs + c];
            if constexpr (BWD) {
                float d = dy[(size_t)p * dys + dyo + c];
                if (thr) d = keep(lkey, (unsigned long long)p * C + c, thr) ? d * keep_scale : 0.f;
                a += d;
                b += d * ((v - mu) * is);
            } else {
                a += v;
                b += v * v;
            }
        }
    }
    s_a[r][cl] = a;
    s_b[r][cl] = b;
    __syncthreads();
    if (r == 0 && c < C) {
#pragma unroll
        for (int k = 1; k < 8; ++k) { a += s_a[k][cl]; b += s_b[k][cl]; }
        part[((size_t)blockIdx.x * 2) * C + c] = a;
        part[((size_t)blockIdx.x * 2 + 1) * C + c] = b;
    }
}

__global__ __launch_bounds__(256) void bn_bwd_final_kernel(const float *__restrict__ part, int T, int C, float *dgamma, float *dbeta) {
    const int c = blockIdx.x;
    double s, q;
    bn_sum_partials(part, T, C, c, s, q);
    if (threadIdx.x == 0) {
        dbeta[c] = (float)s;
        dgamma[c] = (float)q;
    }
}

__global__ __launch_bounds__(256) void bn_fwd_apply_kernel(const float *__restrict__ z, int zs, const float *__restrict__ scale,
                                                           const float *__restrict__ shift, size_t total, int C, unsigned long long lkey,
                                                           unsigned thr, float keep_scale, float *__restrict__ out, int os, int oo) {
    for (size_t e = (size_t)blockIdx.x * blockDim.x + threadIdx.x; e < total; e += (size_t)gridDim.x * blockDim.x) {
        const int c = (int)(e % C);
        const size_t p = e / C;
        float v = z[p * zs + c] * scale[c] + shift[c];
        if (thr) v = keep(lkey, e, thr) ? v * keep_scale : 0.f;
        out[p * os + oo + c] = v;
    }
}

__global__ __launch_bounds__(256) void bn_bwd_apply_kernel(const float *__restrict__ z, int zs, const float *__restrict__ dy, int dys, int dyo,
                                                           const float *__restrict__ mean, const float *__restrict__ invstd,
                                                           const float *__restrict__ gamma, const float *__restrict__ dgamma,
                                                           const float *__restrict__ dbeta, size_t total, int C, float inv_count, float slope,
                                                           unsigned long long lkey, unsigned thr, float keep_scale, float *__restrict__ g, int gs) {
    for (size_t e = (size_t)blockIdx.x * blockDim.x + threadIdx.x; e < total; e += (size_t)gridDim.x * blockDim.x) {
        const int c = (int)(e % C);
        const size_t p = e / C;
        const float v = z[p * zs + c];
        float d = dy[p * dys + dyo + c];
        if (thr) d = keep(lkey, e, thr) ? d * keep_scale : 0.f;
        const float xhat = (v - mean[c]) * invstd[c];
        const float dz = gamma[c] * invstd[c] * (d - dbeta[c] * inv_count - xhat * (dgamma[c] * inv_count));
        g[p * gs + c] = v > 0.f ? dz : slope * dz;
    }
}

}

extern "C" size_t cdnet_dilated_wgrad_workspace_bytes(int N, int H, int W, int Cin, int Cout, int taps) {
    if (N < 1 || H < 1 || W < 1 || Cin < 1 || Cout < 1 || (taps != 1 && taps != 9)) return 0;
    if ((long long)N * H * cdiv(W, STRIP) >= (1ll << 31)) return 0;
    const WgradGeom G = wgrad_geom(N, H, W, Cin, Cout);
    return (size_t)G.nslab * taps * G.CoP * G.CiP * sizeof(float);
}

extern "C" int cdnet_dilated_conv_backward_weight(const cdnet_dilated_wgrad_args *args, void *stream) {
    CDNET_REQUIRE(args, "cdnet_dilated_conv_backward_weight: null args");
    const cdnet_dilated_wgrad_args &A = *args;
    CDNET_REQUIRE(A.x && A.g && A.dw && A.ws, "cdnet_dilated_conv_backward_weight: null x / g / dw / ws");
    CDNET_REQUIRE(A.taps == 1 || A.taps == 9, "cdnet_dilated_conv_backward_weight: taps %d (1 or 9)", A.taps);
    CDNET_REQUIRE(A.dilation >= 1, "cdnet_dilated_conv_backward_weight: dilation %d < 1", A.dilation);
    CDNET_REQUIRE(A.N >= 1 && A.H >= 1 && A.W >= 1 && A.Cin >= 1 && A.Cout >= 1,
                  "cdnet_dilated_conv_backward_weight: N %d H %d W %d Cin %d Cout %d must be positive", A.N, A.H, A.W, A.Cin, A.Cout);
    CDNET_REQUIRE(A.x_cstride >= A.Cin && A.x_cstride % 8 == 0,
                  "cdnet_dilated_conv_backward_weight: x_cstride %d must be a multiple of 8 and >= Cin %d", A.x_cstride, A.Cin);
    CDNET_REQUIRE(A.g_cstride >= A.Cout && A.g_cstride % 8 == 0,
                  "cdnet_dilated_conv_backward_weight: g_cstride %d must be a multiple of 8 and >= Cout %d", A.g_cstride, A.Cout);
    CDNET_REQUIRE((long long)A.N * A.H * cdiv(A.W, STRIP) < (1ll << 31), "cdnet_dilated_conv_backward_weight: image too large");
    const size_t need = cdnet_dilated_wgrad_workspace_bytes(A.N, A.H, A.W, A.Cin, A.Cout, A.taps);
    CDNET_REQUIRE(A.ws_bytes >= need, "cdnet_dilated_conv_backward_weight: workspace of %zu bytes, %zu needed", A.ws_bytes, need);
    const WgradGeom G = wgrad_geom(A.N, A.H, A.W, A.Cin, A.Cout);
    const dim3 grid((unsigned)G.nslab, (unsigned)cdiv(cdiv(A.Cin, 32), WG_WAVES), (unsigned)cdiv(A.Cout, 32));
    if (A.taps == 9) dilated_wgrad_kernel<9><<<grid, WG_WAVES * 64, 0, (hipStream_t)stream>>>(A, G);
    else dilated_wgrad_kernel<1><<<grid, WG_WAVES * 64, 0, (hipStream_t)stream>>>(A, G);
    const size_t total = (size_t)A.Cout * A.Cin * A.taps;
    dilated_wgrad_reduce_kernel<<<(unsigned)((total + 255) / 256), 256, 0, (hipStream_t)stream>>>(static_cast<const float *>(A.ws), A.dw, A.Cin,
                                                                                               A.Cout, A.taps, G);
    return check_launch("cdnet_dilated_conv_backward_weight");
}

extern "C" int cdnet_dropout_mask(unsigned long long key, int layer, size_t count, float p_drop, uint8_t *mask, void *stream) {
    CDNET_REQUIRE(mask, "cdnet_dropout_mask: null mask");
    CDNET_REQUIRE(count >= 1, "cdnet_dropout_mask: count must be positive");
    CDNET_REQUIRE(p_drop >= 0.f && p_drop < 1.f, "cdnet_dropout_mask: p_drop %g outside [0, 1)", (double)p_drop);
    CDNET_REQUIRE(layer >= 0, "cdnet_dropout_mask: layer %d < 0", layer);
    dropout_mask_kernel<<<lin_grid(count, 8192), 256, 0, (hipStream_t)stream>>>(layer_key(key, layer), count, drop_threshold(p_drop), mask);
    return check_launch("cdnet_dropout_mask");
}

extern "C" size_t cdnet_slice_bn_workspace_floats(long long P, int C) {
    if (P < 1 || C < 1) return 0;
    return (size_t)bn_geom(P).T * 2 * C + 2 * (size_t)C;
}

extern "C" int cdnet_slice_bn_train_forward(const cdnet_slice_bn_fwd_args *args, void *stream) {
    CDNET_REQUIRE(args, "cdnet_slice_bn_train_forward: null args");
    const cdnet_slice_bn_fwd_args &A = *args;
    CDNET_REQUIRE(A.z && A.out && A.gamma && A.beta && A.mean && A.invstd && A.ws, "cdnet_slice_bn_train_forward: null pointer");
    CDNET_REQUIRE((A.running_mean == nullptr) == (A.running_var == nullptr), "cdnet_slice_bn_train_forward: one running statistic without the other");
    CDNET_REQUIRE(A.P >= 1 && A.C >= 1, "cdnet_slice_bn_train_forward: P %lld, C %d must be positive", A.P, A.C);
    CDNET_REQUIRE(A.z_cstride >= A.C, "cdnet_slice_bn_train_forward: z_cstride %d < C %d", A.z_cstride, A.C);
    CDNET_REQUIRE(A.out_coff >= 0 && (long long)A.out_coff + A.C <= A.out_cstride,
                  "cdnet_slice_bn_train_forward: out_coff %d + C %d exceeds out_cstride %d", A.out_coff, A.C, A.out_cstride);
    CDNET_REQUIRE((const void *)A.z != (const void *)A.out, "cdnet_slice_bn_train_forward: out must not be z");
    CDNET_REQUIRE(A.p_drop >= 0.f && A.p_drop < 1.f, "cdnet_slice_bn_train_forward: p_drop %g outside [0, 1)", (double)A.p_drop);
    CDNET_REQUIRE(A.layer >= 0, "cdnet_slice_bn_train_forward: layer %d < 0", A.layer);
    CDNET_REQUIRE(A.ws_floats >= cdnet_slice_bn_workspace_floats(A.P, A.C), "cdnet_slice_bn_train_forward: workspace of %zu floats, %zu needed",
                  A.ws_floats, cdnet_slice_bn_workspace_floats(A.P, A.C));
    const BnGeom G = bn_geom(A.P);
    hipStream_t st = (hipStream_t)stream;
    float *part = A.ws, *scale = A.ws + (size_t)G.T * 2 * A.C, *shift = scale + A.C;
    const unsigned long long lkey = layer_key(A.key, A.layer);
    const unsigned thr = drop_threshold(A.p_drop);
    const float ks = 1.f / (1.f - A.p_drop);
    bn_tile_sums_kernel<false><<<dim3((unsigned)G.T, (unsigned)cdiv(A.C, 32)), 256, 0, st>>>(A.z, A.z_cstride, nullptr, 0, 0, nullptr, nullptr, A.P,
                                                                                            A.C, G.tile, lkey, thr, ks, part);
    int rc = check_launch("cdnet_slice_bn_train_forward");
    if (rc) return rc;
    rc = cdnet_bn_finalize_train(part, G.T, A.C, (float)A.P, A.gamma, A.beta, nullptr, A.eps, A.momentum, A.running_mean, A.running_var, scale,
                                 shift, A.mean, A.invstd, stream);
    if (rc) return rc;
    const size_t total = (size_t)A.P * A.C;
    bn_fwd_apply_kernel<<<lin_grid(total, 8192), 256, 0, st>>>(A.z, A.z_cstride, scale, shift, total, A.C, lkey, thr, ks, A.out, A.out_cstride,
                                                          A.out_coff);
    return check_launch("cdnet_slice_bn_train_forward");
}

extern "C" int cdnet_slice_bn_train_backward(const cdnet_slice_bn_bwd_args *args, void *stream) {
    CDNET_REQUIRE(args, "cdnet_slice_bn_train_backward: null args");
    const cdnet_slice_bn_bwd_args &A = *args;
    CDNET_REQUIRE(A.dy && A.z && A.mean && A.invstd && A.gamma && A.dgamma && A.dbeta && A.g && A.ws, "cdnet_slice_bn_train_backward: null pointer");
    CDNET_REQUIRE(A.P >= 1 && A.C >= 1, "cdnet_slice_bn_train_backward: P %lld, C %d must be positive", A.P, A.C);
    CDNET_REQUIRE(A.z_cstride >= A.C, "cdnet_slice_bn_train_backward: z_cstride %d < C %d", A.z_cstride, A.C);
    CDNET_REQUIRE(A.g_cstride >= A.C, "cdnet_slice_bn_train_backward: g_cstride %d < C %d", A.g_cstride, A.C);
    CDNET_REQUIRE(A.dy_coff >= 0 && (long long)A.dy_coff + A.C <= A.dy_cstride,
                  "cdnet_slice_bn_train_backward: dy_coff %d + C %d exceeds dy_cstride %d", A.dy_coff, A.C, A.dy_cstride);
    CDNET_REQUIRE((const void *)A.g != (const void *)A.dy && (const void *)A.g != (const void *)A.z, "cdnet_slice_bn_train_backward: g must not be dy or z");
    CDNET_REQUIRE(A.p_drop >= 0.f && A.p_drop < 1.f, "cdnet_slice_bn_train_backward: p_drop %g outside [0, 1)", (double)A.p_drop);
    CDNET_REQUIRE(A.layer >= 0, "cdnet_slice_bn_train_backward: layer %d < 0", A.layer);
    CDNET_REQUIRE(A.ws_floats >= cdnet_slice_bn_workspace_floats(A.P, A.C), "cdnet_slice_bn_train_backward: workspace of %zu floats, %zu needed",
                  A.ws_floats, cdnet_slice_bn_workspace_floats(A.P, A.C));
    const BnGeom G = bn_geom(A.P);
    hipStream_t st = (hipStream_t)stream;
    const unsigned long long lkey = layer_key(A.key, A.layer);
    const unsigned thr = drop_threshold(A.p_drop);
    const float ks = 1.f / (1.f - A.p_drop);
    bn_tile_sums_kernel<true><<<dim3((unsigned)G.T, (unsigned)cdiv(A.C, 32)), 256, 0, st>>>(A.z, A.z_cstride, A.dy, A.dy_cstride, A.dy_coff, A.mean,
                                                                                           A.invstd, A.P, A.C, G.tile, lkey, thr, ks, A.ws);
    bn_bwd_final_kernel<<<A.C, 256, 0, st>>>(A.ws, G.T, A.C, A.dgamma, A.dbeta);
    const size_t total = (size_t)A.P * A.C;
    bn_bwd_apply_kernel<<<lin_grid(total, 8192), 256, 0, st>>>(A.z, A.z_cstride, A.dy, A.dy_cstride, A.dy_coff, A.mean, A.invstd, A.gamma, A.dgamma,
                                                          A.dbeta, total, A.C, 1.f / (float)A.P, A.slope, lkey, thr, ks, A.g, A.g_cstride);
    return check_launch("cdnet_slice_bn_train_backward");
}
```

cdnet_amd/csrc/model.hip:

```cpp
#include <algorithm>
#include "common.h"
#include "head_feat.h"
#include "bn_sums.h"
#include "launch.h"
#include "xform.h"

using namespace cdnet;

namespace {

__device__ __forceinline__ float bf2f(unsigned short u) { return __uint_as_float((unsigned)u << 16); }
__device__ __forceinline__ unsigned short f2bf(float f) {
    __bf16 b = (__bf16)f;
    return __builtin_bit_cast(unsigned short, b);
}
__device__ __forceinline__ float h2f(unsigned short u) { return (float)__builtin_bit_cast(_Float16, u); }

__global__ __launch_bounds__(256) void input_pack_kernel(const float *__restrict__ x, int N, int C, int plane,
                                                         unsigned short *__restrict__ out) {
    const size_t total = (size_t)N * plane;
    for (size_t i = (size_t)blockIdx.x * blockDim.x + threadIdx.x; i < total; i += (size_t)gridDim.x * blockDim.x) {
        const size_t n = i / plane, p = i - n * plane;
        unsigned short v[16];
#pragma unroll
        for (int c = 0; c < 16; ++c) v[c] = c < C ? f2bf(x[(n * C + c) * plane + p]) : (unsigned short)0;
        uint4 *dst = reinterpret_cast<uint4 *>(out + i * 16);
        dst[0] = *reinterpret_cast<const uint4 *>(v);
        dst[1] = *reinterpret_cast<const uint4 *>(v + 8);
    }
}

__global__ __launch_bounds__(256) void input_pack_f32_kernel(const float *__restrict__ x, int N, int C, int plane, float *__restrict__ out) {
    const size_t total = (size_t)N * plane;
    for (size_t i = (size_t)blockIdx.x * blockDim.x + threadIdx.x; i < total; i += (size_t)gridDim.x * blockDim.x) {
        const size_t n = i / plane, p = i - n * plane;
        float v[16];
#pragma unroll
        for (int c = 0; c < 16; ++c) v[c] = c < C ? x[(n * C + c) * plane + p] : 0.f;
        float4 *dst = reinterpret_cast<float4 *>(out + i * 16);
#pragma unroll
        for (int k = 0; k < 4; ++k) dst[k] = make_float4(v[4 * k], v[4 * k + 1], v[4 * k + 2], v[4 * k + 3]);
    }
}

__global__ void bn_fold_eval_kernel(const float *g, const float *b, const float *rm, const float *rv, const float *bias,
                                    float eps, int C, float *scale, float *shift) {
    int c = blockIdx.x * blockDim.x + threadIdx.x;
    if (c >= C) return;
    float s = g[c] / sqrtf(rv[c] + eps);
    scale[c] = s;
    shift[c] = b[c] + ((bias ? bias[c] : 0.f) - rm[c]) * s;
}

__global__ __launch_bounds__(256) void bn_finalize_train_kernel(const float *__restrict__ stats, int T, int C, float count,
                                                                const float *g, const float *b, const float *bias,
                                                                float eps, float momentum, float *rm, float *rv,
                                                                float *scale, float *shift, float *mean_out,
                                                                float *invstd_out) {
    const int c = blockIdx.x;
    double s, q;
    bn_sum_partials(stats, T, C, c, s, q);
    if (threadIdx.x == 0) {
        double mean = s / count;
        double var = q / count - mean * mean;
        if (var < 0) var = 0;
        float invstd = (float)(1.0 / sqrt(var + (double)eps));
        float sc = g[c] * invstd;
        scale[c] = sc;
        shift[c] = b[c] - (float)mean * sc;
        if (mean_out) mean_out[c] = (float)mean;
        if (invstd_out) invstd_out[c] = invstd;
        if (rm) {
            float mb = (float)mean + (bias ? bias[c] : 0.f);
            rm[c] = (1.f - momentum) * rm[c] + momentum * mb;
            float unb = (float)(var * (count / (count > 1.f ? count - 1.f : 1.f)));
            rv[c] = (1.f - momentum) * rv[c] + momentum * unb;
        }
    }
}

template <int NC>
__device__ __forceinline__ void load_feat_f32(const HeadFeat &f, size_t pix, int c0, const float *s_sc, const float *s_sh, float *v) {
    const float4 *pr = reinterpret_cast<const float4 *>(reinterpret_cast<const float *>(f.raw) + pix * 64 + c0);
    const float4 *ps = f.res ? reinterpret_cast<const float4 *>(reinterpret_cast<const float *>(f.res) + pix * 64 + c0) : nullptr;
#pragma unroll
    for (int q = 0; q < NC / 4; ++q) {
        const float4 r = pr[q];
        float x[4] = {r.x, r.y, r.z, r.w};
        float rr[4] = {0.f, 0.f, 0.f, 0.f};
        if (ps) { const float4 t = ps[q]; rr[0] = t.x; rr[1] = t.y; rr[2] = t.z; rr[3] = t.w; }
#pragma unroll
        for (int j = 0; j < 4; ++j) {
            float t = x[j];
            if (f.scale) t = fmaf(t, s_sc[c0 + q * 4 + j], s_sh[c0 + q * 4 + j]);
            if (ps) t += rr[j];
            if (f.relu) t = fmaxf(t, 0.f);
            v[q * 4 + j] = t;
        }
    }
}

__device__ __forceinline__ void load_feat64(const HeadFeat &f, size_t pix, const float *s_sc, const float *s_sh, float *v) {
    if (f.f16 == 2) { load_feat_f32<64>(f, pix, 0, s_sc, s_sh, v); return; }
    const uint4 *pr = reinterpret_cast<const uint4 *>(f.raw + pix * 64);
    const uint4 *ps = f.res ? reinterpret_cast<const uint4 *>(f.res + pix * 64) : nullptr;
#pragma unroll
    for (int q = 0; q < 8; ++q) {
        uint4 r = pr[q];
        const unsigned short *h = reinterpret_cast<const unsigned short *>(&r);
        uint4 rr = make_uint4(0, 0, 0, 0);
        if (ps) rr = ps[q];
        const unsigned short *hr = reinterpret_cast<const unsigned short *>(&rr);
#pragma unroll
        for (int j = 0; j < 8; ++j) {
            float x = f.f16 ? h2f(h[j]) : bf2f(h[j]);
            if (f.scale || ps || f.relu) {
                if (f.scale) x = fmaf(x, s_sc[q * 8 + j], s_sh[q * 8 + j]);
                if (ps) x += f.f16 ? h2f(hr[j]) : bf2f(hr[j]);
                if (f.relu) x = fmaxf(x, 0.f);
                x = bf2f(f2bf(x));
            }
            v[q * 8 + j] = x;
        }
    }
}

struct FeatRaw16 {
    uint4 r[2], s[2];
};
__device__ __forceinline__ void load_raw16(const HeadFeat &f, size_t pix, int q, FeatRaw16 &R) {
    const uint4 *pr = reinterpret_cast<const uint4 *>(f.raw + pix * 64 + q * 16);
    R.r[0] = pr[0];
    R.r[1] = pr[1];
    R.s[0] = R.s[1] = make_uint4(0, 0, 0, 0);
    if (f.res) {
        const uint4 *ps = reinterpret_cast<const uint4 *>(f.res + pix * 64 + q * 16);
        R.s[0] = ps[0];
        R.s[1] = ps[1];
    }
}
__device__ __forceinline__ void feat_from_raw16(const HeadFeat &f, const FeatRaw16 &R, int q, const float *s_sc, const float *s_sh, float *v) {
    const bool has_res = f.res != nullptr;
    const bool fast = f.f16 && f.scale && f.relu;
#pragma unroll
    for (int h2 = 0; h2 < 2; ++h2) {
        const uint4 r = R.r[h2], rr = R.s[h2];
        if (f.f16 && !f.scale && f.relu && has_res) {
            xf_addrelu_f16_to_f32(__builtin_bit_cast(u32x4, r), __builtin_bit_cast(u32x4, rr), v + h2 * 8);
            continue;
        }
        if (fast) {
            const u32x4 a = __builtin_bit_cast(u32x4, r), b = __builtin_bit_cast(u32x4, rr);
            const int c0 = q * 16 + h2 * 8;
            if (has_res) xf_bnrelu_f16_to_f32<true>(a, b, s_sc + c0, s_sh + c0, v + h2 * 8);
            else xf_bnrelu_f16_to_f32<false>(a, a, s_sc + c0, s_sh + c0, v + h2 * 8);
            continue;
        }
        const unsigned short *h = reinterpret_cast<const unsigned short *>(&r);
        const unsigned short *hr = reinterpret_cast<const unsigned short *>(&rr);
#pragma unroll
        for (int j = 0; j < 8; ++j) {
            const int c = q * 16 + h2 * 8 + j;
            float x = f.f16 ? h2f(h[j]) : bf2f(h[j]);
            if (f.scale || has_res || f.relu) {
                if (f.scale) x = fmaf(x, s_sc[c], s_sh[c]);
                if (has_res) x += f.f16 ? h2f(hr[j]) : bf2f(hr[j]);
                if (f.relu) x = fmaxf(x, 0.f);
                x = bf2f(f2bf(x));
            }
            v[h2 * 8 + j] = x;
        }
    }
}
__device__ __forceinline__ void load_feat16(const HeadFeat &f, size_t pix, int q, const float *s_sc, const float *s_sh, float *v) {
    if (f.f16 == 2) { load_feat_f32<16>(f, pix, q * 16, s_sc, s_sh, v); return; }
    FeatRaw16 R;
    load_raw16(f, pix, q, R);
    feat_from_raw16(f, R, q, s_sc, s_sh, v);
}

template <int FM>
__global__ __launch_bounds__(256, (FM == 2 ? 1 : 4)) void dam_head_fwd_kernel(HeadFeat f1, HeadFeat f2, HeadFeat f3, const HeadW *__restrict__ hw,
                                                           int N, int plane, float *__restrict__ mask,
                                                           float *__restrict__ point, float *__restrict__ dirn) {
    __shared__ HeadW w;
    __shared__ float s_sc[3][64], s_sh[3][64];
    {
        const float *src = reinterpret_cast<const float *>(hw);
        float *dst = reinterpret_cast<float *>(&w);
        for (int i = threadIdx.x; i < (int)(sizeof(HeadW) / 4); i += 256) dst[i] = src[i];
        if (threadIdx.x < 64) {
            const HeadFeat *fs[3] = {&f1, &f2, &f3};
#pragma unroll
            for (int k = 0; k < 3; ++k) {
                s_sc[k][threadIdx.x] = fs[k]->scale ? fs[k]->scale[threadIdx.x] : 1.f;
                s_sh[k][threadIdx.x] = fs[k]->scale ? fs[k]->shift[threadIdx.x] : 0.f;
            }
        }
    }
    __syncthreads();
    const size_t total = (size_t)N * plane;
    const int q = threadIdx.x & 3;
    const bool all16 = FM != 2 || (f1.f16 != 2 && f2.f16 != 2 && f3.f16 != 2);
    auto conv = [&](const HeadFeat &f, const FeatRaw16 &R, int k, float *v) {
        if (FM == 1) {
#pragma unroll
            for (int h2 = 0; h2 < 2; ++h2)
                xf_bnrelu_f16_to_f32<true>(__builtin_bit_cast(u32x4, R.r[h2]), __builtin_bit_cast(u32x4, R.s[h2]), s_sc[k] + q * 16 + h2 * 8,
                                           s_sh[k] + q * 16 + h2 * 8, v + h2 * 8);
        } else {
            feat_from_raw16(f, R, q, s_sc[k], s_sh[k], v);
        }
    };
    auto fetch = [&](const HeadFeat &f, size_t pix, FeatRaw16 &R) {
// ... 470 lines not shown
    const size_t total = (size_t)N * Hs * Ws * VPP;
    const float sy = (float)Hs / (float)H, sx = (float)Ws / (float)W;
    for (size_t i = (size_t)blockIdx.x * blockDim.x + threadIdx.x; i < total; i += (size_t)gridDim.x * blockDim.x) {
        const int slot = (int)(i % VPP);
        const size_t pix = i / VPP;
        const int xs = (int)(pix % Ws), ys = (int)((pix / Ws) % Hs), n = (int)(pix / ((size_t)Ws * Hs));
        float acc[8];
#pragma unroll
        for (int j = 0; j < 8; ++j) acc[j] = 0.f;
        int ylo, yhi, xlo, xhi;
        upsample_window(ys, Hs, H, ylo, yhi);
        upsample_window(xs, Ws, W, xlo, xhi);
        for (int y = ylo; y < yhi; ++y) {
            float fy = ((float)y + 0.5f) * sy - 0.5f;
            fy = fy < 0.f ? 0.f : fy;
            const int y0 = (int)fy, y1 = y0 + (y0 < Hs - 1 ? 1 : 0);
            const float ly = fy - (float)y0;
            const float wy = (y0 == ys ? 1.f - ly : 0.f) + (y1 == ys ? ly : 0.f);
            if (wy == 0.f) continue;
            for (int x = xlo; x < xhi; ++x) {
                float fx = ((float)x + 0.5f) * sx - 0.5f;
                fx = fx < 0.f ? 0.f : fx;
                const int x0 = (int)fx, x1 = x0 + (x0 < Ws - 1 ? 1 : 0);
                const float lx = fx - (float)x0;
                const float wx = (x0 == xs ? 1.f - lx : 0.f) + (x1 == xs ? lx : 0.f);
                if (wx == 0.f) continue;
                float v[8];
                if (F32) {
                    const float4 *q = reinterpret_cast<const float4 *>(reinterpret_cast<const float *>(dout) + (((size_t)n * H + y) * W + x) * cstride + coff + slot * 8);
                    const float4 a = q[0], b = q[1];
                    v[0] = a.x; v[1] = a.y; v[2] = a.z; v[3] = a.w; v[4] = b.x; v[5] = b.y; v[6] = b.z; v[7] = b.w;
                } else {
                    bf8_to_f32(*reinterpret_cast<const uint4 *>(dout + (((size_t)n * H + y) * W + x) * cstride + coff + slot * 8), v);
                }
                const float wgt = wy * wx;
#pragma unroll
                for (int j = 0; j < 8; ++j) acc[j] = fmaf(wgt, v[j], acc[j]);
            }
        }
        if (F32) {
            float4 *o = reinterpret_cast<float4 *>(reinterpret_cast<float *>(din) + pix * C + slot * 8);
            o[0] = make_float4(acc[0], acc[1], acc[2], acc[3]);
            o[1] = make_float4(acc[4], acc[5], acc[6], acc[7]);
            continue;
        }
        unsigned short oh[8];
#pragma unroll
        for (int j = 0; j < 8; ++j) oh[j] = f2bf(acc[j]);
        uint4 ou;
        ou.x = oh[0] | ((unsigned)oh[1] << 16); ou.y = oh[2] | ((unsigned)oh[3] << 16);
        ou.z = oh[4] | ((unsigned)oh[5] << 16); ou.w = oh[6] | ((unsigned)oh[7] << 16);
        *reinterpret_cast<uint4 *>(din + pix * C + slot * 8) = ou;
    }
}

template <typename VT>
__global__ __launch_bounds__(256) void s2d_to_nhwc_kernel(const unsigned short *__restrict__ in_, int N, int H2, int W2, int C,
                                                          unsigned short *__restrict__ out_) {
    constexpr int EPV = 16 / sizeof(VT);
    const VT *in = reinterpret_cast<const VT *>(in_);
    VT *out = reinterpret_cast<VT *>(out_);
    const int VPP = C / EPV;
    const size_t total = (size_t)N * H2 * W2 * 4 * VPP;
    for (size_t i = (size_t)blockIdx.x * blockDim.x + threadIdx.x; i < total; i += (size_t)gridDim.x * blockDim.x) {
        const int slot = (int)(i % VPP);
        size_t r = i / VPP;
        const int ab = (int)(r & 3); r >>= 2;
        const int x2 = (int)(r % W2), y2 = (int)((r / W2) % H2), n = (int)(r / ((size_t)W2 * H2));
        const int a = ab >> 1, b = ab & 1;
        const uint4 v = *reinterpret_cast<const uint4 *>(in + (((size_t)n * H2 + y2) * W2 + x2) * 4 * C + (size_t)ab * C + slot * EPV);
        *reinterpret_cast<uint4 *>(out + (((size_t)n * 2 * H2 + 2 * y2 + a) * 2 * W2 + 2 * x2 + b) * C + slot * EPV) = v;
    }
}

struct GradSumArgs { const unsigned short *g[6]; int cstride[6], coff[6]; int nterm; const unsigned short *mask; size_t npix; int C; unsigned short *out; };

template <bool F32>
__global__ __launch_bounds__(256) void grad_sum_kernel(const GradSumArgs A) {
    const int VPP = A.C / 8;
    const size_t total = A.npix * VPP;
    for (size_t i = (size_t)blockIdx.x * blockDim.x + threadIdx.x; i < total; i += (size_t)gridDim.x * blockDim.x) {
        const int slot = (int)(i % VPP);
        const size_t pix = i / VPP;
        float acc[8], v[8];
#pragma unroll
        for (int j = 0; j < 8; ++j) acc[j] = 0.f;
        auto load8 = [&](const unsigned short *base, size_t e) {
            if (F32) {
                const float4 *p = reinterpret_cast<const float4 *>(reinterpret_cast<const float *>(base) + e);
                const float4 a = p[0], b = p[1];
                v[0] = a.x; v[1] = a.y; v[2] = a.z; v[3] = a.w; v[4] = b.x; v[5] = b.y; v[6] = b.z; v[7] = b.w;
            } else {
                bf8_to_f32(*reinterpret_cast<const uint4 *>(base + e), v);
            }
        };
#pragma unroll
        for (int k = 0; k < 6; ++k) {
            if (k < A.nterm) {
                load8(A.g[k], pix * A.cstride[k] + A.coff[k] + slot * 8);
#pragma unroll
                for (int j = 0; j < 8; ++j) acc[j] += v[j];
            }
        }
        if (A.mask) {
            load8(A.mask, pix * A.C + slot * 8);
#pragma unroll
            for (int j = 0; j < 8; ++j) acc[j] = v[j] > 0.f ? acc[j] : 0.f;
        }
        if (F32) {
            float4 *o = reinterpret_cast<float4 *>(reinterpret_cast<float *>(A.out) + pix * A.C + slot * 8);
            o[0] = make_float4(acc[0], acc[1], acc[2], acc[3]);
            o[1] = make_float4(acc[4], acc[5], acc[6], acc[7]);
        } else {
            unsigned short oh[8];
#pragma unroll
            for (int j = 0; j < 8; ++j) oh[j] = f2bf(acc[j]);
            uint4 ou;
            ou.x = oh[0] | ((unsigned)oh[1] << 16); ou.y = oh[2] | ((unsigned)oh[3] << 16);
            ou.z = oh[4] | ((unsigned)oh[5] << 16); ou.w = oh[6] | ((unsigned)oh[7] << 16);
            *reinterpret_cast<uint4 *>(A.out + pix * A.C + slot * 8) = ou;
        }
    }
}

}

extern "C" int cdnet_input_pack(const float *x, int N, int C, int H, int W, void *out, void *stream) {
    CDNET_REQUIRE(x && out, "cdnet_input_pack: null pointer");
    CDNET_REQUIRE(N > 0 && C > 0 && C <= 16 && H > 0 && W > 0, "cdnet_input_pack: bad size (C=%d must be <= 16)", C);
    input_pack_kernel<<<lin_grid((size_t)N * H * W, 4096), 256, 0, (hipStream_t)stream>>>(x, N, C, H * W, (unsigned short *)out);
    return check_launch("cdnet_input_pack");
}

extern "C" int cdnet_input_pack_f32(const float *x, int N, int C, int H, int W, float *out, void *stream) {
    CDNET_REQUIRE(x && out, "cdnet_input_pack_f32: null pointer");
    CDNET_REQUIRE(N > 0 && C > 0 && C <= 16 && H > 0 && W > 0, "cdnet_input_pack_f32: bad size (C=%d must be <= 16)", C);
    input_pack_f32_kernel<<<lin_grid((size_t)N * H * W, 4096), 256, 0, (hipStream_t)stream>>>(x, N, C, H * W, out);
    return check_launch("cdnet_input_pack_f32");
}

extern "C" int cdnet_bn_fold_eval(const float *gamma, const float *beta, const float *running_mean, const float *running_var,
                                  const float *conv_bias, float eps, int C, float *scale, float *shift, void *stream) {
    CDNET_REQUIRE(gamma && beta && running_mean && running_var && scale && shift && C > 0, "cdnet_bn_fold_eval: bad args");
    bn_fold_eval_kernel<<<cdiv(C, 256), 256, 0, (hipStream_t)stream>>>(gamma, beta, running_mean, running_var, conv_bias, eps, C,
                                                                      scale, shift);
    return check_launch("cdnet_bn_fold_eval");
}

extern "C" int cdnet_bn_finalize_train(const float *stats, int T, int C, float count, const float *gamma, const float *beta,
                                       const float *conv_bias, float eps, float momentum, float *running_mean,
                                       float *running_var, float *scale, float *shift, float *save_mean,
                                       float *save_invstd, void *stream) {
    CDNET_REQUIRE(stats && gamma && beta && scale && shift && T > 0 && C > 0 && count > 0, "cdnet_bn_finalize_train: bad args");
    bn_finalize_train_kernel<<<C, 256, 0, (hipStream_t)stream>>>(stats, T, C, count, gamma, beta, conv_bias, eps, momentum,
                                                                         running_mean, running_var, scale, shift, save_mean,
                                                                         save_invstd);
    return check_launch("cdnet_bn_finalize_train");
}

extern "C" int cdnet_dam_head_forward(const cdnet_head_feat *f1, const cdnet_head_feat *f2, const cdnet_head_feat *f3,
                                      const float *head_weights, int N, int H, int W, float *mask, float *point,
                                      float *direction, void *stream) {
    CDNET_REQUIRE(f1 && f2 && f3 && head_weights && mask && point && direction, "cdnet_dam_head_forward: null pointer");
    CDNET_REQUIRE(f1->raw && f2->raw && N > 0 && H > 0 && W > 0, "cdnet_dam_head_forward: bad args");
    const HeadFeat a = mk_hf(*f1), b = mk_hf(*f2), c = mk_hf(*f3);
    auto plain = [](const HeadFeat &f) { return f.f16 == 0 && !f.scale && !f.relu && !f.res; };
    auto train = [](const HeadFeat &f) { return f.f16 == 1 && f.scale && f.relu && f.res; };
    const int grid = lin_grid((size_t)N * H * W * 4, 4096);
    const HeadW *hw = reinterpret_cast<const HeadW *>(head_weights);
    const size_t total = (size_t)N * H * W;
    const int mgrid = (int)std::min<size_t>(2048, (total + 127) / 128);
    if (!c.raw) {
        CDNET_REQUIRE(plain(a) && plain(b), "cdnet_dam_head_forward: f3->raw = NULL (point given) needs plain bf16 f1 / f2");
        dam_head_mfma_kernel<false, false><<<mgrid, 256, 0, (hipStream_t)stream>>>(a.raw, b.raw, nullptr, hw, total, H * W, mask, point, direction);
        return check_launch("cdnet_dam_head_forward");
    }
    if (plain(a) && plain(b) && plain(c)) {
        dam_head_mfma_kernel<true, false><<<mgrid, 256, 0, (hipStream_t)stream>>>(a.raw, b.raw, c.raw, hw, total, H * W, mask, point, direction);
        return check_launch("cdnet_dam_head_forward");
    }
    auto plain32 = [](const HeadFeat &f) { return f.f16 == 2 && !f.scale && !f.relu && !f.res; };
    if (plain32(a) && plain32(b) && plain32(c)) {
        const int g32 = (int)std::min<size_t>(4096, (total + 63) / 64);
        dam_head_mfma_kernel<true, true><<<g32, 256, 0, (hipStream_t)stream>>>(a.raw, b.raw, c.raw, hw, total, H * W, mask, point, direction);
        return check_launch("cdnet_dam_head_forward");
    }
    if (train(a) && train(b) && train(c)) dam_head_fwd_kernel<1><<<grid, 256, 0, (hipStream_t)stream>>>(a, b, c, hw, N, H * W, mask, point, direction);
    else dam_head_fwd_kernel<2><<<grid, 256, 0, (hipStream_t)stream>>>(a, b, c, hw, N, H * W, mask, point, direction);
    return check_launch("cdnet_dam_head_forward");
}

extern "C" int cdnet_final_conv1x1(const cdnet_head_feat *f, const float *w, const float *b, int K, int N, int H, int W,
                                   float *out, void *stream) {
    CDNET_REQUIRE(f && f->raw && w && b && out, "cdnet_final_conv1x1: null pointer");
    CDNET_REQUIRE(K >= 1 && K <= 32 && N > 0 && H > 0 && W > 0, "cdnet_final_conv1x1: K=%d must be in [1,32]", K);
    final_conv1x1_kernel<<<lin_grid((size_t)N * H * W, 4096), 256, 0, (hipStream_t)stream>>>(mk_hf(*f), w, b, K, N, H * W, out);
    return check_launch("cdnet_final_conv1x1");
}

extern "C" int cdnet_window_pack(const float *img, int C, int H, int W, int view_xform, int tile_h, int tile_w, int stride, int ny,
                                 int nx, void *out_bf16_nhwc16, void *stream) {
    CDNET_REQUIRE(img && out_bf16_nhwc16, "cdnet_window_pack: null pointer");
    CDNET_REQUIRE(C > 0 && C <= 16 && H > 0 && W > 0 && tile_h > 0 && tile_w > 0 && stride > 0 && ny > 0 && nx > 0 &&
                  view_xform >= 0 && view_xform < 8, "cdnet_window_pack: bad arguments");
    window_pack_kernel<<<lin_grid((size_t)ny * nx * tile_h * tile_w, 4096), 256, 0, (hipStream_t)stream>>>(
        img, C, H, W, view_xform, tile_h, tile_w, stride, ny, nx, (unsigned short *)out_bf16_nhwc16);
    return check_launch("cdnet_window_pack");
}

extern "C" int cdnet_window_pack_f32(const float *img, int C, int H, int W, int view_xform, int tile_h, int tile_w, int stride, int ny,
                                     int nx, float *out_f32_nhwc16, void *stream) {
    CDNET_REQUIRE(img && out_f32_nhwc16, "cdnet_window_pack_f32: null pointer");
    CDNET_REQUIRE(C > 0 && C <= 16 && H > 0 && W > 0 && tile_h > 0 && tile_w > 0 && stride > 0 && ny > 0 && nx > 0 &&
                  view_xform >= 0 && view_xform < 8, "cdnet_window_pack_f32: bad arguments");
    window_pack_f32_kernel<<<lin_grid((size_t)ny * nx * tile_h * tile_w, 4096), 256, 0, (hipStream_t)stream>>>(
        img, C, H, W, view_xform, tile_h, tile_w, stride, ny, nx, out_f32_nhwc16);
    return check_launch("cdnet_window_pack_f32");
}

extern "C" int cdnet_window_stitch(const float *tiles, int K, int tile_h, int tile_w, int stride, int overlap, int ny, int nx, int Hv,
                                   int Wv, float *out, void *stream) {
    CDNET_REQUIRE(tiles && out, "cdnet_window_stitch: null pointer");
    CDNET_REQUIRE(K > 0 && tile_h > 0 && tile_w > 0 && stride > 0 && ny > 0 && nx > 0 && Hv > 0 && Wv > 0 && overlap >= 0,
                  "cdnet_window_stitch: bad arguments");
    CDNET_REQUIRE((ny - 1) * stride + tile_h >= Hv && (nx - 1) * stride + tile_w >= Wv, "cdnet_window_stitch: windows do not cover the view");
    CDNET_REQUIRE((ny == 1 || tile_h >= stride + overlap / 2) && (nx == 1 || tile_w >= stride + overlap / 2),
                  "cdnet_window_stitch: tile %d x %d is smaller than stride + overlap / 2 = %d", tile_h, tile_w, stride + overlap / 2);
    window_stitch_kernel<<<lin_grid((size_t)K * Hv * Wv, 4096), 256, 0, (hipStream_t)stream>>>(tiles, K, tile_h, tile_w, stride, overlap / 2,
                                                                                         ny, nx, Hv, Wv, out);
    return check_launch("cdnet_window_stitch");
}


static int fuse_sum_impl(const cdnet_fuse_term *terms, int nterm, int N, int H, int W, int C, int relu, void *out, int out_cstride, int out_coff,
                         void *stream, bool f32) {
    CDNET_REQUIRE(terms && out && nterm >= 1 && nterm <= 4, "cdnet_fuse_sum: 1..4 terms");
    CDNET_REQUIRE(N > 0 && H > 0 && W > 0 && C >= 8 && C % 8 == 0, "cdnet_fuse_sum: bad size (C %% 8)");
    FuseArgs A;
    for (int k = 0; k < 4; ++k) {
        if (k < nterm) {
            CDNET_REQUIRE(terms[k].x && terms[k].Hs > 0 && terms[k].Ws > 0 && terms[k].Hs <= H && terms[k].Ws <= W, "cdnet_fuse_sum: term %d", k);
            CDNET_REQUIRE((terms[k].f16 == 2) == f32, "cdnet_fuse_sum: term %d storage %d does not match the %s entry point", k, terms[k].f16,
                          f32 ? "fp32" : "16-bit");
            A.t[k].x = terms[k].x; A.t[k].Hs = terms[k].Hs; A.t[k].Ws = terms[k].Ws;
            A.t[k].scale = terms[k].scale; A.t[k].shift = terms[k].shift; A.t[k].f16 = terms[k].f16;
            CDNET_REQUIRE((terms[k].scale == nullptr) == (terms[k].shift == nullptr), "cdnet_fuse_sum: scale and shift come together");
        } else { A.t[k].x = nullptr; A.t[k].Hs = A.t[k].Ws = 0; A.t[k].scale = A.t[k].shift = nullptr; A.t[k].f16 = 0; }
    }
    A.nterm = nterm; A.N = N; A.H = H; A.W = W; A.C = C; A.relu = relu; A.out = reinterpret_cast<unsigned short *>(out);
    A.out_cstride = out_cstride ? out_cstride : C; A.out_coff = out_coff;
    CDNET_REQUIRE(A.out_cstride % 8 == 0 && out_coff % 8 == 0 && out_coff + C <= A.out_cstride, "cdnet_fuse_sum: output channel slice");
    const size_t total = (size_t)N * H * W * (C / 8);
    const int grid = lin_grid(total, 4096);
    CDNET_REQUIRE(f32 || total < (1ull << 31), "cdnet_fuse_sum: more than 2^31 output vectors (the 16-bit kernels index in 32 bits)");
    if (f32) fuse_sum_kernel<true><<<grid, 256, 0, (hipStream_t)stream>>>(A);
    else {
        switch (nterm) {
            case 1: fuse_sum16_kernel<1><<<grid, 256, 0, (hipStream_t)stream>>>(A); break;
            case 2: fuse_sum16_kernel<2><<<grid, 256, 0, (hipStream_t)stream>>>(A); break;
            case 3: fuse_sum16_kernel<3><<<grid, 256, 0, (hipStream_t)stream>>>(A); break;
            default: fuse_sum16_kernel<4><<<grid, 256, 0, (hipStream_t)stream>>>(A); break;
        }
    }
    return check_launch("cdnet_fuse_sum");
}

extern "C" int cdnet_fuse_sum(const cdnet_fuse_term *terms, int nterm, int N, int H, int W, int C, int relu, uint16_t *out, int out_cstride,
                              int out_coff, void *stream) {
    return fuse_sum_impl(terms, nterm, N, H, W, C, relu, out, out_cstride, out_coff, stream, false);
}

extern "C" int cdnet_fuse_sum_f32(const cdnet_fuse_term *terms, int nterm, int N, int H, int W, int C, int relu, float *out, int out_cstride,
                                  int out_coff, void *stream) {
    return fuse_sum_impl(terms, nterm, N, H, W, C, relu, out, out_cstride, out_coff, stream, true);
}

static int upsample_bwd_impl(const void *dout, int N, int H, int W, int C, int dout_cstride, int dout_coff, int Hs, int Ws, void *din, void *stream,
                             bool f32) {
    CDNET_REQUIRE(dout && din && N > 0 && H >= Hs && W >= Ws && Hs > 0 && Ws > 0 && C % 8 == 0 && C >= 8, "cdnet_upsample_bilinear_backward: bad args");
    const int cs = dout_cstride ? dout_cstride : C;
    CDNET_REQUIRE(cs % 8 == 0 && dout_coff % 8 == 0 && dout_coff + C <= cs, "cdnet_upsample_bilinear_backward: channel slice");
    CDNET_REQUIRE((2ll * Hs + 1) * H + Hs < (1ll << 31) && (2ll * Ws + 1) * W + Ws < (1ll << 31),
                  "cdnet_upsample_bilinear_backward: (2 Hs + 1) H does not fit 32 bits");
    const unsigned short *d = reinterpret_cast<const unsigned short *>(dout);
    unsigned short *o = reinterpret_cast<unsigned short *>(din);
    if (f32) upsample_bwd_kernel<true><<<lin_grid((size_t)N * Hs * Ws * (C / 8), 4096), 256, 0, (hipStream_t)stream>>>(d, N, H, W, C, cs, dout_coff, Hs, Ws, o);
    else upsample_bwd_kernel<false><<<lin_grid((size_t)N * Hs * Ws * (C / 8), 4096), 256, 0, (hipStream_t)stream>>>(d, N, H, W, C, cs, dout_coff, Hs, Ws, o);
    return check_launch("cdnet_upsample_bilinear_backward");
}

extern "C" int cdnet_upsample_bilinear_backward(const uint16_t *dout, int N, int H, int W, int C, int dout_cstride, int dout_coff, int Hs, int Ws,
                                                uint16_t *din, void *stream) {
    return upsample_bwd_impl(dout, N, H, W, C, dout_cstride, dout_coff, Hs, Ws, din, stream, false);
}

extern "C" int cdnet_upsample_bilinear_backward_f32(const float *dout, int N, int H, int W, int C, int dout_cstride, int dout_coff, int Hs, int Ws,
                                                    float *din, void *stream) {
    return upsample_bwd_impl(dout, N, H, W, C, dout_cstride, dout_coff, Hs, Ws, din, stream, true);
}

extern "C" int cdnet_s2d_to_nhwc(const uint16_t *in, int N, int H2, int W2, int C, uint16_t *out, void *stream) {
    CDNET_REQUIRE(in && out && N > 0 && H2 > 0 && W2 > 0 && C % 8 == 0 && C >= 8, "cdnet_s2d_to_nhwc: bad args");
    s2d_to_nhwc_kernel<unsigned short><<<lin_grid((size_t)N * H2 * W2 * 4 * (C / 8), 4096), 256, 0, (hipStream_t)stream>>>(in, N, H2, W2, C, out);
    return check_launch("cdnet_s2d_to_nhwc");
}

extern "C" int cdnet_s2d_to_nhwc_f32(const float *in, int N, int H2, int W2, int C, float *out, void *stream) {
    CDNET_REQUIRE(in && out && N > 0 && H2 > 0 && W2 > 0 && C % 4 == 0 && C >= 4, "cdnet_s2d_to_nhwc_f32: bad args");
    s2d_to_nhwc_kernel<float><<<lin_grid((size_t)N * H2 * W2 * 4 * (C / 4), 4096), 256, 0, (hipStream_t)stream>>>(
// ... 27 lines not shown
```

cdnet_amd/models/dam/model_unet_rev1.py:

```python
import torch
import torch.nn as nn

from ... import _lib, runtime
from ...runtime import ConvLayer, Src, pooled, pad_offsets

VGG16_CFG = [64, 64, 'M', 128, 128, 'M', 256, 256, 256, 'M', 512, 512, 512, 'M', 512, 512, 512, 'M']


def vgg16_bn_features():
    layers, c = [], 3
    for v in VGG16_CFG:
        if v == 'M':
            layers.append(nn.MaxPool2d(kernel_size=2, stride=2))
        else:
            layers += [nn.Conv2d(c, v, kernel_size=3, padding=1), nn.BatchNorm2d(v), nn.ReLU(inplace=True)]
            c = v
    return nn.Sequential(*layers)


class revAttention(nn.Module):
    def __init__(self, in_channels):
        super().__init__()
        self.Conv1x1 = nn.Conv2d(in_channels, 1, kernel_size=1, bias=False)


def get_backbone(name, pretrained=True):
    if name != 'vgg16_bn':
        raise NotImplementedError('{} backbone model is not implemented so far.'.format(name))
    return vgg16_bn_features(), ['5', '12', '22', '32', '42'], '43'


class UpsampleBlock(nn.Module):
    def __init__(self, ch_in, ch_out=None, skip_in=0, use_bn=True, parametric=True):
        super().__init__()
        assert parametric and use_bn, 'only the parametric (transposed-conv) + BatchNorm decoder is on the CDNet path'
        self.up = nn.ConvTranspose2d(ch_in, ch_out, kernel_size=(4, 4), stride=2, padding=1, output_padding=0, bias=False)
        self.bn1 = nn.BatchNorm2d(ch_out)
        self.relu = nn.ReLU(inplace=True)
        self.conv2 = nn.Conv2d(ch_out + skip_in, ch_out, kernel_size=(3, 3), stride=1, padding=1, bias=False)
        self.bn2 = nn.BatchNorm2d(ch_out)


class ResidualUnit(nn.Module):
    def __init__(self, in_channels, out_channels):
        super().__init__()
        self.conv1 = nn.Conv2d(in_channels, out_channels, kernel_size=3, padding=1, bias=False)
        self.bn1 = nn.BatchNorm2d(out_channels)
        self.relu1 = nn.ReLU(inplace=True)
        self.conv2 = nn.Conv2d(out_channels, out_channels, kernel_size=3, padding=1, bias=False)
        self.bn2 = nn.BatchNorm2d(out_channels)
        self.relu2 = nn.ReLU(inplace=True)
        self.conv_1x1 = nn.Conv2d(in_channels, out_channels, kernel_size=1)


class _RU:

    def __init__(self, name, m):
        self.c1 = ConvLayer(name + '.conv1', 'conv3', m.conv1.weight, None, m.bn1)
        self.c2 = ConvLayer(name + '.conv2', 'conv3', m.conv2.weight, None, m.bn2)
        self.cr = ConvLayer(name + '.conv_1x1', 'conv1', m.conv_1x1.weight, m.conv_1x1.bias, None)
        self.cr.bias_grad_from = self.c2

    def layers(self):
        return [self.c1, self.c2, self.cr]

    def forward(self, x, training, store=False, dot=None):
        relu2 = not runtime.DEBUG_NORELU
        if not training:
            f = runtime.residual_unit_eval(self.c1, self.c2, self.cr, x, relu2, dot=dot)
            if f is not None:
                return f
        if runtime.RU_FUSE:
            h = self.c1.forward([x], training, relu=True)
            y = self.c2.forward([h], training, relu=False, out_dtype=runtime.raw_dtype())
            f = self.cr.forward([x], training, eres=Src(y.x, y.scale, y.shift, relu=relu2))
            self.c2.node_relu, self.c2.node_res = (2 if relu2 else 0), f.x
            self.cr.fused_res_of = self.c2
            return f
        self.cr.fused_res_of = None
        r = self.cr.forward([x], training, out_dtype=runtime.raw_dtype())
        h = self.c1.forward([x], training, relu=True)
        y = self.c2.forward([h], training, relu=False, out_dtype=runtime.raw_dtype())
        self.c2.node_relu, self.c2.node_res = relu2, r.x
        out = Src(y.x, y.scale, y.shift, relu=relu2, res=r.x)
        if store and runtime.RU_MATERIALIZE:
            lazy, out = out, runtime.materialize(out)
            out.grad_to = (lazy.x, 0)
        return out


class Unet(nn.Module):
    VARIANT = 'rev1'
    DIRECTION_OUT = 9

    def __init__(self, backbone_name='vgg16_bn', pretrained=True, encoder_freeze=False, classes=21,
                 decoder_filters=(256, 128, 64, 32, 16), parametric_upsampling=True, shortcut_features='default',
                 decoder_use_batchnorm=True):
        super().__init__()
        self.backbone_name = backbone_name
        self.backbone, self.shortcut_features, self.bb_out_name = get_backbone(backbone_name, pretrained=pretrained)
        shortcut_chs, bb_out_chs = [64, 128, 256, 512, 512], 512
        decoder_filters = decoder_filters[:len(self.shortcut_features)]
        decoder_filters_in = [bb_out_chs] + list(decoder_filters[:-1])
        num_blocks = len(self.shortcut_features)
        self.upsample_blocks = nn.ModuleList()
        for i, (fin, fout) in enumerate(zip(decoder_filters_in, decoder_filters)):
            self.upsample_blocks.append(UpsampleBlock(fin, fout, skip_in=shortcut_chs[num_blocks - i - 1],
                                                      parametric=parametric_upsampling, use_bn=decoder_use_batchnorm))
        self.final_conv = nn.Conv2d(decoder_filters[-1], classes, kernel_size=(1, 1))
        self.replaced_conv1 = False
        self.child0 = nn.Conv2d(1, 64, kernel_size=(3, 3), stride=(1, 1), padding=(1, 1))
        self.child_conv1 = nn.Conv2d(1, 64, kernel_size=(7, 7), stride=(2, 2), padding=(3, 3), bias=False)
        self.mask_feature = ResidualUnit(decoder_filters[-1], 64)
        self.direction_feature = ResidualUnit(64, 64)
        self.point_feature = ResidualUnit(64, 64)
        self.point_conv = nn.Conv2d(64, 1, kernel_size=1)
        self.directionAtt = revAttention(1)
        self.direction_conv = nn.Conv2d(64, self.DIRECTION_OUT, kernel_size=1)
        self.maskAtt = revAttention(self.DIRECTION_OUT)
        self.mask_conv = nn.Conv2d(64, 3, kernel_size=1)
        if self.VARIANT != 'rev1':
            self.residual = ResidualUnit(64, 64)
        if encoder_freeze:
            self.freeze_encoder()
        self._rt = None
        self._head_w = None
        self._head_ver = None

    def freeze_encoder(self):
        for p in self.backbone.parameters():
            p.requires_grad = False

    UNUSED_PREFIXES = ('final_conv.', 'child0.', 'child_conv1.')

    def _build_runtime(self):
        enc, i = [], 0
        mods = list(self.backbone.children())
        while i < len(mods):
            if isinstance(mods[i], nn.Conv2d):
                enc.append(('conv', ConvLayer('backbone.%d' % i, 'conv3', mods[i].weight, mods[i].bias, mods[i + 1]), str(i + 2)))
                i += 3
            else:
                enc.append(('pool', None, str(i)))
                i += 1
        dec = []
        for k, b in enumerate(self.upsample_blocks):
            dec.append((ConvLayer('upsample_blocks.%d.up' % k, 'convT4', b.up.weight, None, b.bn1),
                        ConvLayer('upsample_blocks.%d.conv2' % k, 'conv3', b.conv2.weight, None, b.bn2)))
        self._rt = dict(enc=enc, dec=dec, ru=[_RU('mask_feature', self.mask_feature),
                                               _RU('direction_feature', self.direction_feature),
                                               _RU('point_feature', self.point_feature)])
        if self.VARIANT != 'rev1':
            self._rt['ru_res'] = _RU('residual', self.residual)

    def conv_layers(self):
        if self._rt is None:
            self._build_runtime()
        out = [l for kind, l, _ in self._rt['enc'] if kind == 'conv']
        for up, c2 in self._rt['dec']:
            out += [up, c2]
        for ru in self._rt['ru']:
            out += ru.layers()
        if 'ru_res' in self._rt:
            out += self._rt['ru_res'].layers()
        return out

    def head_weight_block(self):
        ps = [self.point_conv.weight, self.direction_conv.weight, self.mask_conv.weight, self.point_conv.bias,
              self.direction_conv.bias, self.mask_conv.bias, self.directionAtt.Conv1x1.weight, self.maskAtt.Conv1x1.weight]
        if getattr(self, '_head_flat', None) is not None:
            return self._head_flat
        ver = tuple(p._version for p in ps)
        if self._head_w is None or self._head_ver != ver:
            with torch.no_grad():
                self._head_w = torch.cat([p.detach().reshape(-1).float() for p in ps]).contiguous()
            assert self._head_w.numel() == 855
            self._head_ver = ver
        return self._head_w

    def forward_features(self, x, training):
        if self._rt is None:
            self._build_runtime()
        if not x.is_cuda:
            raise RuntimeError('cdnet_amd.models.dam.model_unet_rev1.Unet runs on the MI355X only (no CPU fallback)')
        assert x.shape[1] == 3, 'the CDNet path feeds 3-channel tiles (child0/child_conv1 branches are never taken)'
        return self.forward_features_packed(runtime.input_pack(x.float()), training)

    def forward_features_packed(self, x16, training):
        if self._rt is None:
            self._build_runtime()
        t = Src(x16)
        t.is_input = True
        self._rt['enc'][0][1].needs_input_grad = False
        feats = {}
        enc, tp = self._rt['enc'], None
        for idx, (kind, layer, out_name) in enumerate(enc):
            if kind == 'conv':
                if not training and idx + 1 < len(enc) and enc[idx + 1][0] == 'pool' and not getattr(runtime, 'DEBUG_NORELU', False):
                    t, tp = layer.forward_eval_pool([t])
                else:
                    t = layer.forward([t], training)
            else:
                t, tp = (tp if tp is not None else pooled(t)), None
            if out_name in self.shortcut_features:
                feats[out_name] = t
            if out_name == self.bb_out_name:
                break
        for skip_name, (up, conv2) in zip(self.shortcut_features[::-1], self._rt['dec']):
            skip = feats[skip_name]
            u = up.forward([t], training)
            sh, sw = skip.logical_hw()
            uh, uw = u.logical_hw()
            u.off = pad_offsets((uh, uw), (sh, sw))
            tt = None if training else conv2.forward_eval_swapped([u, skip], H=sh, W=sw)
# ... 60 lines not shown
```

cdnet_amd/runtime.py:

```python
import ctypes as C
import weakref
import torch

from . import _lib, engine
from .engine import Src

BN_EPS = 1e-5
BN_MOMENTUM = 0.1

import os as _os

PRECISION = _os.environ.get('CDNET_PRECISION', 'bf16')
assert PRECISION in ('bf16', 'fp32'), PRECISION


def set_precision(p):
    global PRECISION
    assert p in ('bf16', 'fp32'), p
    if p != PRECISION:
        PRECISION = p
        WEIGHTS_EPOCH[0] += 1


def act_dtype():
    return torch.float32 if PRECISION == 'fp32' else torch.bfloat16


def raw_dtype():
    return torch.float32 if PRECISION == 'fp32' else torch.float16


DEBUG_NORELU = False
TAPE = None
WEIGHTS_EPOCH = [0]
LAYERS = weakref.WeakSet()


class HeadFeat(C.Structure):
    _fields_ = [('raw', C.c_void_p), ('res', C.c_void_p), ('scale', C.c_void_p), ('shift', C.c_void_p),
                ('relu', C.c_int), ('f16', C.c_int)]


def head_feat(s):
    assert not s.pool and s.off == (0, 0) and s.C == 64
    f = HeadFeat()
    f.raw, f.res = s.x.data_ptr(), (None if s.res is None else s.res.data_ptr())
    f.scale = None if s.scale is None else s.scale.data_ptr()
    f.shift = None if s.shift is None else s.shift.data_ptr()
    f.relu = int(s.relu)
    f.f16 = int(s.f16)
    return f


class ConvLayer:

    def __init__(self, name, kind, weight, bias=None, bn=None, cfg_override=None):
        assert kind in ('conv3', 'conv1', 'convT4', 'convT2', 'conv3s2')
        self.name, self.kind, self.weight, self.bias, self.bn = name, kind, weight, bias, bn
        self.cfg_override = cfg_override
        if kind == 'conv3s2':
            self.Cout, self.Cin = weight.shape[0], 4 * weight.shape[1]
        elif kind in ('conv3', 'conv1'):
            self.Cout, self.Cin = weight.shape[0], weight.shape[1]
        else:
            self.Cin, self.Cout = weight.shape[0], weight.shape[1]
        self.taps = {'conv3': 9, 'conv1': 1, 'convT4': 4, 'convT2': 1, 'conv3s2': 9}[kind]
        self.transposed = kind in ('convT4', 'convT2')
        self.pack_mode = {'conv3': 0, 'conv1': 0, 'convT4': 2, 'convT2': 3, 'conv3s2': 6}[kind]
        self.cfg = None
        self.cfg_f32 = False
        self.wp = None
        self.wp_version = None
        self.fold = None
        self.fold_version = None
        dev = weight.device
        if bn is not None:
            self.scale = torch.empty((self.Cout,), dtype=torch.float32, device=dev)
            self.shift = torch.empty((self.Cout,), dtype=torch.float32, device=dev)
            self.save_mean = torch.empty((self.Cout,), dtype=torch.float32, device=dev)
            self.save_invstd = torch.empty((self.Cout,), dtype=torch.float32, device=dev)
        self.stats = None
        self.saved = None
        self.node_relu, self.node_res = True, None
        self.needs_input_grad = True
        self.bias_grad_from = None
        self.wpb, self.wpb_version, self.cfg_bwd = None, None, None
        self.wp_padded = False
        LAYERS.add(self)

    def _version(self):
        v = self.weight._version
        if self.bias is not None:
            v = (v, self.bias._version)
        return v

    def prepare(self, src_channels, H, W, N=16):
        cin_total = sum(src_channels)
        f32 = PRECISION == 'fp32'
        if self.cfg is None or self.cfg_f32 != f32:
            self.cfg = engine.choose_cfg(src_channels, self.Cout, H, W, self.cfg_override, taps=self.taps, transposed=self.transposed, N=N,
                                         f32=f32)
            self.cfg_f32, self.wp, self.cfg_bwd, self.wpb = f32, None, None, None
        ver = (self.weight._version, WEIGHTS_EPOCH[0])
        if self.wp is None or self.wp_version != ver:
            pad = cin_total if cin_total != self.Cin else None
            self.wp_padded = pad is not None
            self.wp = engine.pack_weights(self.weight.detach(), self.cfg, self.pack_mode, Cin_pad=pad, out=self.wp, split=f32)
            self.wp_version = ver

    def backward_pack(self, cin_total, H, W):
        ver = (self.weight._version, WEIGHTS_EPOCH[0])
        f32 = self.cfg_f32
        if self.cfg_bwd is None:
            if self.transposed:
                self.cfg_bwd = engine.choose_cfg([2 * self.Cout, 2 * self.Cout], self.Cin, H, W, taps=(9 if self.kind == 'convT4' else 1), f32=f32)
            else:
                self.cfg_bwd = engine.choose_cfg([self.Cout], cin_total, H, W, taps=self.taps, f32=f32)
        if self.wpb is None or self.wpb_version != ver:
            if self.transposed:
                mode = 4 if self.kind == 'convT4' else 5
                self.wpb = engine.pack_weights(self.weight.detach(), self.cfg_bwd, mode, out=self.wpb, split=f32)
            else:
                assert cin_total == self.Cin, 'the RGB stem never needs an input gradient'
                self.wpb = engine.pack_weights(self.weight.detach(), self.cfg_bwd, 7 if self.kind == 'conv3s2' else 1, out=self.wpb, split=f32)
            self.wpb_version = ver
        return self.wpb, self.cfg_bwd

    def eval_fold(self):
        bn = self.bn
        ver = (bn.weight._version, bn.bias._version, bn.running_mean._version, bn.running_var._version,
               None if self.bias is None else self.bias._version, WEIGHTS_EPOCH[0])
        if self.fold is None or self.fold_version != ver:
            if self.fold is None:
                self.fold = (torch.empty_like(self.scale), torch.empty_like(self.shift))
            _lib.call('cdnet_bn_fold_eval', _lib.ptr(bn.weight.detach()), _lib.ptr(bn.bias.detach()),
                      _lib.ptr(bn.running_mean), _lib.ptr(bn.running_var),
                      None if self.bias is None else _lib.ptr(self.bias.detach()), BN_EPS, self.Cout,
                      _lib.ptr(self.fold[0]), _lib.ptr(self.fold[1]), _lib.stream_ptr())
            self.fold_version = ver
        return self.fold

    def eval_pack(self, src_channels, allow_f32=False):
        if not EVAL_FOLD_WEIGHTS or not getattr(self, 'fold_eval', True) or self.kind not in ('conv3', 'conv1') or self.bn is None:
            return None
        f32 = PRECISION == 'fp32'
        if f32 and not allow_f32:
            return None
        cin_total = sum(src_channels)
        pad = cin_total if cin_total != self.Cin else None
        sc, sh = self.eval_fold()
        ver = (self.weight._version, self.fold_version, WEIGHTS_EPOCH[0], tuple(self.cfg), f32)
        if getattr(self, 'wpe', None) is None or self.wpe_version != ver:
            self.wpe = engine.pack_weights(self.weight.detach(), self.cfg, 0, Cin_pad=pad, out=getattr(self, 'wpe', None), cout_scale=sc, split=f32)
            self.wpe_version = ver
        return self.wpe, sh

    def forward_eval_swapped(self, srcs, relu=True, H=None, W=None):
        if PRECISION != 'bf16' or self.kind != 'conv3' or self.bn is None or len(srcs) != 2 or not EVAL_FOLD_WEIGHTS or not getattr(self, 'fold_eval', True):
            return None
        a, b = srcs
        if (a.C // 16) % 2 == 0 or (b.C // 16) % 2 or a.C % 16 or b.C % 16 or a.C + b.C != self.Cin:
            return None
        if any(s.scale is not None or s.relu or s.res is not None or s.f16 or s.pool for s in srcs):
            return None
        if H is None:
            H, W = b.logical_hw()
        if H % 16 or W % 16:
            return None
        self.prepare([s.C for s in srcs], H, W, a.N)
        if tuple(self.cfg[:2]) != (16, 16):
            return None
        sc, sh = self.eval_fold()
        ver = (self.weight._version, self.fold_version, WEIGHTS_EPOCH[0], tuple(self.cfg), a.C)
        if getattr(self, 'wps', None) is None or self.wps_version != ver:
            w = self.weight.detach()
            wz = torch.zeros((w.shape[0], 16, w.shape[2], w.shape[3]), dtype=w.dtype, device=w.device)
            wperm = torch.cat([w[:, a.C:], w[:, :a.C], wz], 1).contiguous()
            self.wps = engine.pack_weights(wperm, self.cfg, 0, cout_scale=sc)
            self.wps_version = ver
        kw = dict(oshift=sh, orelu=relu and not DEBUG_NORELU, H=H, W=W, pad_chunks=1)
        key = (a.N, H, W, a.C, b.C, a.off, b.off, engine.CONV_DEBUG, PRECISION)
        elig = self.__dict__.setdefault('_swapped_eligible', {})
        if key not in elig:
            elig[key] = engine.conv_forward([b, a], self.wps, self.Cout, self.cfg, 9, query_ws=True, **kw) == 2
        if not elig[key]:
            return None
        out, _ = engine.conv_forward([b, a], self.wps, self.Cout, self.cfg, 9, **kw)
        return Src(out)

    def forward_eval_pool(self, srcs):
        H, W = srcs[0].logical_hw()
        if PRECISION == 'bf16' and H % 2 == 0 and W % 2 == 0:
            self.prepare([s.C for s in srcs], H, W, srcs[0].N)
            ep = self.eval_pack([s.C for s in srcs])
            if ep is not None:
                N = srcs[0].N
                out = torch.empty((N, H, W, self.Cout), dtype=torch.bfloat16, device=srcs[0].x.device)
                pout = torch.empty((N, H // 2, W // 2, self.Cout), dtype=torch.bfloat16, device=srcs[0].x.device)
                kw = dict(oshift=ep[1], orelu=True, H=H, W=W, out=out, pool_out=pout)
                if engine.conv_forward(srcs, ep[0], self.Cout, self.cfg, self.taps, self.transposed, query_ws=True, **kw) == 2:
                    engine.conv_forward(srcs, ep[0], self.Cout, self.cfg, self.taps, self.transposed, **kw)
                    return Src(out), Src(pout)
        if PRECISION == 'fp32' and H % 2 == 0 and W % 2 == 0 and self.bn is not None and not DEBUG_NORELU:
            self.prepare([s.C for s in srcs], H, W, srcs[0].N)
            sc, sh = self.eval_fold()
            N = srcs[0].N
            out = torch.empty((N, H, W, self.Cout), dtype=torch.float32, device=srcs[0].x.device)
            pout = torch.empty((N, H // 2, W // 2, self.Cout), dtype=torch.float32, device=srcs[0].x.device)
            kw = dict(oscale=sc, oshift=sh, orelu=True, H=H, W=W, out=out, pool_out=pout)
            if engine.conv_forward(srcs, self.wp, self.Cout, self.cfg, self.taps, self.transposed, query_ws=True, **kw) == 1:
                engine.conv_forward(srcs, self.wp, self.Cout, self.cfg, self.taps, self.transposed, **kw)
                return Src(out), Src(pout)
        return self.forward(srcs, False), None

    def forward(self, srcs, training, relu=True, H=None, W=None, out_dtype=None, eres=None, debug_or=0):
        if PRECISION == 'fp32':
            out_dtype = torch.float32
        elif out_dtype is None:
            out_dtype = torch.bfloat16
        if H is None:
            H, W = srcs[0].logical_hw()
        if DEBUG_NORELU:
            relu = False
        self.prepare([s.C for s in srcs], H, W, srcs[0].N)
        bias = None if self.bias is None else self.bias.detach()
        if self.bn is None:
            out, _ = engine.conv_forward(srcs, self.wp, self.Cout, self.cfg, self.taps, self.transposed, bias=bias, H=H, W=W,
                                         out_dtype=out_dtype, eres=eres)
            if training:
                self.saved = (srcs, out, H, W)
                self.node_relu, self.node_res = False, None
                if TAPE is not None:
                    TAPE.append(self)
            return Src(out)
        if not training:
            ep = self.eval_pack([s.C for s in srcs])
            if ep is not None:
                out, _ = engine.conv_forward(srcs, ep[0], self.Cout, self.cfg, self.taps, self.transposed, oshift=ep[1],
# ... 237 lines not shown
```

cdnet_amd/trainer.py:

```python
import ctypes as C
import os

import torch

from . import _lib, engine, optim, runtime, streams
from .allreduce import BucketReducer, bucketed_allreduce
from .engine import Src
from .optim import HEAD_PARAMS, FlatState
from .synth import synthetic_batch


class GradIn(C.Structure):
    _fields_ = [('g', C.c_void_p), ('Hg', C.c_int), ('Wg', C.c_int), ('oy', C.c_int), ('ox', C.c_int),
                ('pooled', C.c_int), ('coff', C.c_int), ('cstride', C.c_int), ('pad_', C.c_int)]


class BnBwdArgs(C.Structure):
    _fields_ = [('raw', C.c_void_p), ('res', C.c_void_p), ('scale', C.c_void_p), ('shift', C.c_void_p),
                ('mean', C.c_void_p), ('invstd', C.c_void_p), ('gin', GradIn * 3), ('ngin', C.c_int),
                ('f16', C.c_int), ('relu', C.c_int), ('N', C.c_int), ('H', C.c_int), ('W', C.c_int), ('C', C.c_int)]


_WGRAD_WGS_DEEP, _WGRAD_WGS_SHALLOW = 128, 160
_WGRAD_WGS_KQ = 128
# ... 285 lines not shown
                or owner.saved[1].dtype != torch.float32 or tuple(owner.saved[1].shape) != tuple(f3.x.shape):
            return None
        return owner

    def _classifier_backward(self, key, f, conv, dl):
        N, H, W, _ = f.x.shape
        K = conv.out_channels
        df = self.buf(key, (N, H, W, 64), runtime.act_dtype())
        ws = self._ws('slab', _lib.load().cdnet_final_conv1x1_backward_workspace_floats(), side=True)
        hf = runtime.head_feat(f)
        w = conv.weight.detach().reshape(K, 64)
        _lib.call('cdnet_final_conv1x1_backward', C.byref(hf), _lib.ptr(w), _lib.ptr(dl), K, N, H, W, _lib.ptr(df), _lib.ptr(ws),
                  ws.numel(), _lib.ptr(conv.weight.grad), _lib.ptr(conv.bias.grad), _lib.stream_ptr())
        return _G(df, H, W)

    def _run_tape(self, heads, params):
        grads = {}

        def add(t, g):
            grads.setdefault(id(t), []).append(g)
        for t, g in heads:
            add(t, g)
        self._overlap_begin()
        self._overlap_done(params)
        self._backward_tape(grads, add)

    def _backward_tape(self, grads, add):
        self._cat_cache = {}
        self._rd_pending, self._rd_params, self._rd_bytes = [], [], 0
        if len(self._rd_tables) > 16:
            self._rd_tables.clear()
        self._readers, self._producer, self._bn_partials = {}, {}, {}
        self._tape_pos = {id(Lt): k for k, Lt in enumerate(self.tape)}
        for Lt in self.tape:
            if isinstance(Lt, runtime.FuseNode):
                for t in Lt.saved[0]:
                    self._readers[id(t.x)] = self._readers.get(id(t.x), 0) + 1
                continue
            for sx in Lt.saved[0]:
                self._readers[id(sx.x)] = self._readers.get(id(sx.x), 0) + 1
                if sx.res is not None:
                    self._readers[id(sx.res)] = self._readers.get(id(sx.res), 0) + 1
            self._producer[id(Lt.saved[1])] = Lt
        side = self._side_stream()
        self._side_active = side is not None
        if self._packb_pending:
            torch.cuda.current_stream().wait_event(self._event('packb'))
            self._packb_pending = False
        for k, L in enumerate(reversed(self.tape)):
            if isinstance(L, runtime.FuseNode):
                L.backward(self, grads, add)
                continue
            gl = self.take(grads, id(L.saved[1]))
            if gl is None:
                continue
            owner = getattr(L, 'fused_res_of', None)
            if owner is not None:
                grads.setdefault(id(owner.saved[1]), []).extend(gl)
                owner.deferred_layer = L
                continue
            self._layer_backward(k, L, gl, grads, add, side)
            d = getattr(L, 'deferred_layer', None)
            if d is not None:
                L.deferred_layer = None
                self._layer_backward(('deferred', k), d, self.take(grads, id(d.saved[1])), grads, add, side)
        if side is not None:
            with _on_stream(side):
                self._flush_reduces()
            ev = self._event(-1)
            ev.record(side)
            torch.cuda.current_stream().wait_event(ev)
        else:
            self._flush_reduces()

    def _weights_done(self, params):
        if not self._rd_pending:
            self._overlap_done(params)
            return
        self._rd_params.append(params)
        if self._rd_bytes >= self._rd_mb * (1 << 20):
            self._flush_reduces()

    def _flush_reduces(self):
        if self._rd_pending:
            key = tuple(self._rd_pending)
            tab = self._rd_tables.get(key)
            if tab is None:
                lib = _lib.load()
                descs = (_lib.WgradReduceDesc * len(key))()
                b0 = 0
                for i, a in enumerate(key):
                    _lib.call('cdnet_wgrad_reduce_desc_fill', *a, b0, C.byref(descs[i]))
                    b0 += descs[i].blocks
                dev_tab = torch.frombuffer(bytearray(bytes(descs)), dtype=torch.uint8).to(self.dev)
                tab = self._rd_tables[key] = (dev_tab, len(key), b0)
            _lib.call('cdnet_wgrad_reduce_batch', _lib.ptr(tab[0]), tab[1], tab[2], _lib.stream_ptr())
        for params in self._rd_params:
            self._overlap_done(params)
        self._rd_pending, self._rd_params, self._rd_bytes = [], [], 0

    def _layer_backward(self, k, L, gl, grads, add, side):
        srcs, out, Hl, Wl = L.saved
        No, Ho, Wo, Co = out.shape
        params = (L.weight, L.bias, None if L.bn is None else L.bn.weight, None if L.bn is None else L.bn.bias)
        part = self._bn_partials.pop(id(out), None)
        if len(gl) == 1 and gl[0].masked:
            g = self._bn_backward_masked(L, out, gl[0], add)
        elif part is not None:
            assert len(gl) == 1, (L.name, len(gl))
            a, ktab = self._bn_backward_stats(L, out, gl[0], partial=part)
            g = self.buf(('draw', L.name), (No, Ho, Wo, Co), runtime.act_dtype())
            _lib.call('cdnet_bn_backward_apply', C.byref(a), _lib.ptr(ktab), _lib.ptr(g), _lib.stream_ptr())
        elif L.bn is not None or len(gl) > 1 or gl[0].pooled or gl[0].coff or (gl[0].cstride not in (0, Co)):
            g = self._bn_backward(L, out, gl, add)
        else:
            g = gl[0].t
        if side is None:
            self._weight_backward(L, srcs, g, Hl, Wl)
            self._weights_done(params)
            self._input_backward(L, srcs, g, Hl, Wl, add)
        else:
            ev = self._event(k)
            ev.record()
            beside = _RU_1X1_SIDE and L.kind == 'conv1' and isinstance(k, tuple) and getattr(L, 'needs_input_grad', True)
            if not beside:
                self._input_backward(L, srcs, g, Hl, Wl, add)
            side.wait_event(ev)
            with _on_stream(side):
                if beside:
                    ev2 = self._event(('beside', k))

                    def add_beside(tgt, g_):
                        g_.event = ev2
                        add(tgt, g_)
                    self._input_backward(L, srcs, g, Hl, Wl, add_beside)
                    ev2.record()
                self._weight_backward(L, srcs, g, Hl, Wl)
                self._weights_done(params)

    def _bn_backward_stats(self, L, out, g, partial):
        a = self._bn_args(L, out, [_G(g.t, g.Hg, g.Wg)], res=None, relu=1)
        ktab = self.buf(('ktab', L.name), (7, out.shape[3]), torch.float32)
        bn = L.bn
        _lib.call('cdnet_bn_backward_finalize', C.byref(a), _lib.ptr(bn.weight.detach()), _lib.ptr(bn.weight.grad), _lib.ptr(bn.bias.grad),
                  _lib.ptr(partial), partial.shape[0], _lib.ptr(ktab), _lib.stream_ptr())
        return a, ktab

    def _bn_backward_masked(self, L, out, g, add):
        No, Ho, Wo, Co = out.shape
        a = self._bn_args(L, out, [_G(g.t, g.Hg, g.Wg)], res=None, relu=0)
        draw = self.buf(('draw', L.name), (No, Ho, Wo, Co), runtime.act_dtype())
        ws = self._ws('bn', _lib.load().cdnet_bn_backward_workspace_floats(Co))
        bn = L.bn
        _lib.call('cdnet_bn_backward', C.byref(a), _lib.ptr(bn.weight.detach()), _lib.ptr(bn.weight.grad), _lib.ptr(bn.bias.grad),
                  _lib.ptr(ws), ws.numel(), _lib.ptr(draw), None, _lib.stream_ptr())
        add(L.node_res, _G(g.t, Ho, Wo))
        return draw

    def _stats_fusable(self, L, srcs, H, W, N, wpb, cfgb, cin_total):
        f32 = runtime.PRECISION == 'fp32'
        if not f32 or os.environ.get('CDNET_BN_STATS_FUSE', '1') != '1' or getattr(runtime, 'DEBUG_NORELU', False):
            return None
        if L.kind != 'conv3' or L.transposed or len(srcs) != 1:
            return None
        sx = srcs[0]
        if getattr(sx, 'is_input', False) or sx.scale is None or sx.shift is None or sx.relu is not True or sx.res is not None or sx.pool \
                or tuple(sx.off) != (0, 0) or sx.x.dtype != runtime.raw_dtype() or hasattr(sx, 'grad_to') or sx.row_stride:
            return None
        if f32 and cin_total % 64:
            return None
        P = self._producer.get(id(sx.x))
        if P is None or P.bn is None or getattr(P, 'node_res', None) is not None or getattr(P, 'node_relu', True) is not True \
                or self._readers.get(id(sx.x), 0) != 1 or tuple(sx.x.shape) != (N, H, W, cin_total):
            return None
        key = ('statsfusable', L.name, N, H, W, runtime.PRECISION)
        hit = self._bufs.get(key)
        if hit is None:
            part = torch.zeros((1024, 2, cin_total), dtype=torch.float32, device=self.dev)
            gin = self.buf(('din', L.name), (N, H, W, cin_total), runtime.act_dtype())
            gdummy = self.buf(('draw', L.name), (N, H, W, L.Cout), runtime.act_dtype())
            ok = engine.conv_forward([Src(gdummy)], wpb, cin_total, cfgb, taps=L.taps, out=gin, H=H, W=W, query_ws=True,
                                     bns=(sx.x, P.scale, P.shift, P.save_mean, P.save_invstd, part))
            hit = self._bufs[key] = (part if ok else False)
        if hit is False:
            return None
        return P, hit

    def _bn_args(self, L, out, gl, res, relu):
        a = BnBwdArgs()
        a.raw = out.data_ptr()
        a.res = None if res is None else res.data_ptr()
        if L.bn is not None:
            a.scale, a.shift = L.scale.data_ptr(), L.shift.data_ptr()
            a.mean, a.invstd = L.save_mean.data_ptr(), L.save_invstd.data_ptr()
        a.ngin = len(gl)
        assert 1 <= len(gl) <= 3, (L.name, len(gl))
        for k, g in enumerate(gl):
            a.gin[k].g = g.t.data_ptr()
            a.gin[k].Hg, a.gin[k].Wg, a.gin[k].oy, a.gin[k].ox = g.Hg, g.Wg, g.oy, g.ox
            a.gin[k].pooled, a.gin[k].coff, a.gin[k].cstride = int(g.pooled), g.coff, g.cstride or out.shape[3]
        a.f16 = {torch.bfloat16: 0, torch.float16: 1, torch.float32: 2}[out.dtype]
        a.relu = relu
        a.N, a.H, a.W, a.C = out.shape
        return a

    def _bn_backward(self, L, out, gl, add):
        No, Ho, Wo, Co = out.shape
        res = getattr(L, 'node_res', None)
        has_bn = L.bn is not None
        if len(gl) > 3:
            plain = [g for g in gl if not g.pooled and g.oy == 0 and g.ox == 0 and (g.Hg, g.Wg) == (Ho, Wo)]
            rest = [g for g in gl if g not in plain]
            assert len(rest) <= 2 and len(plain) >= 2, (L.name, len(gl))
            d = self.buf(('gsum', L.name), (No, Ho, Wo, Co), runtime.act_dtype())
            self.grad_sum(plain, None, No * Ho * Wo, Co, d)
            gl = rest + [_G(d, Ho, Wo)]
        a = self._bn_args(L, out, gl, res, int(getattr(L, 'node_relu', True)))
        draw = self.buf(('draw', L.name), (No, Ho, Wo, Co), runtime.act_dtype())
        dz = None
        if res is not None:
            dz = self.buf(('dz', L.name), (No, Ho, Wo, Co), runtime.act_dtype())
        ws = self._ws('bn', _lib.load().cdnet_bn_backward_workspace_floats(Co))
        bn = L.bn
        _lib.call('cdnet_bn_backward', C.byref(a), _lib.ptr(bn.weight.detach()) if has_bn else None,
                  _lib.ptr(bn.weight.grad) if has_bn else None, _lib.ptr(bn.bias.grad) if has_bn else None,
                  _lib.ptr(ws), ws.numel(), _lib.ptr(draw), _lib.ptr(dz), _lib.stream_ptr())
        if res is not None:
            add(getattr(L, 'node_res_grad_to', None) if getattr(L, 'node_res_grad_to', None) is not None else res, _G(dz, Ho, Wo))
            L.node_res_grad_to = None
        return draw

    def _side_stream(self):
        if not WGRAD_STREAM or self.dev.type != 'cuda':
            return None
        if self._wstream is None:
            self._wstream = streams.side_stream(self.dev)
            self._events = {}
        return self._wstream

    def _event(self, k):
        e = self._events.get(k)
        if e is None:
            e = self._events[k] = torch.cuda.Event()
        return e

    def _weight_backward(self, L, srcs, g, H, W):
        lib = _lib.load()
        N = g.shape[0]
        Cout = L.Cout
        cin_total = sum(s.C for s in srcs)
        cin_real = L.Cin
        mode = {'conv3': 0, 'conv1': 0, 'convT4': 2, 'convT2': 3, 'conv3s2': 6}[L.kind]
        taps, npar, ostride = L.taps, (4 if L.transposed else 1), (2 if L.transposed else 1)
        cap = _wgrad_wgs(self._side_active and getattr(L, 'needs_input_grad', True), H * W, Cout)
        coff = 0
        for s in srcs:
            ci_t = _choose_ci_tiles(s.C, Cout)
            CI, CO = ci_t * 32, (4 // ci_t) * 32
            other = -(-s.C // CI) * -(-Cout // CO) * npar
            ntiles = N * (-(-H // 8)) * (-(-W // 16))
            ksplit = max(1, min(ntiles, cap // other if other < cap else 1))
            nslab = lib.cdnet_conv_wgrad_slab_floats(s.C, Cout, taps, npar, ci_t, ksplit)
            defer = self._rd_mb > 0
            slab = self.buf(('wslab', L.name, coff), (nslab,), torch.float32) if defer else self._ws('slab', nslab, side=True)
            cs = engine.ConvSrc()
            s.fill(cs)
            csrc_real = min(s.C, cin_real - coff) if cin_total != cin_real else s.C
            _lib.call('cdnet_conv_backward_weight', C.byref(cs), coff, csrc_real, cin_real, _lib.ptr(g), Cout, N, H, W, taps,
                      npar, ostride, ci_t, ksplit, _lib.ptr(slab), _lib.ptr(L.weight.grad), mode | (_WGRAD_DEFER if defer else 0),
                      _lib.stream_ptr())
            if defer:
                self._rd_pending.append((s.C, coff, csrc_real, cin_real, Cout, taps, npar, ci_t, ksplit, slab.data_ptr(),
                                         L.weight.grad.data_ptr(), mode))
                self._rd_bytes += nslab * 4
            coff += s.C
        if L.bias is not None and L.bn is None:
            owner = getattr(L, 'bias_grad_from', None)
            if owner is not None:
                L.bias.grad.copy_(owner.bn.bias.grad)
            else:
                ws = self._ws('slab', lib.cdnet_bias_grad_workspace_floats(Cout), side=True)
                _lib.call(_lib.entry('cdnet_bias_grad', g.dtype == torch.float32), _lib.ptr(g), g.numel() // Cout, Cout,
                          _lib.ptr(ws), ws.numel(), _lib.ptr(L.bias.grad), _lib.stream_ptr())

    def _input_backward(self, L, srcs, g, H, W, add):
        if not getattr(L, 'needs_input_grad', True):
            return
        N = g.N if isinstance(g, Src) else g.shape[0]
        Cout = L.Cout
        cin_total = sum(s.C for s in srcs)
        wpb, cfgb = L.backward_pack(cin_total, H, W)
        if L.kind == 'conv3s2':
            Cp = cin_total // 4
            gs2d = self.buf(('ds2d', L.name), (N, H, W, cin_total), runtime.act_dtype())
            engine.conv_forward([Src(g)], wpb, cin_total, cfgb, taps=9, out=gs2d, H=H, W=W)
            gin = self.buf(('din', L.name), (N, 2 * H, 2 * W, Cp), runtime.act_dtype())
            _lib.call(_lib.entry('cdnet_s2d_to_nhwc', gin.dtype == torch.float32), _lib.ptr(gs2d), N, H, W, Cp, _lib.ptr(gin),
                      _lib.stream_ptr())
            add(srcs[0].x, _G(gin, 2 * H, 2 * W))
            return
        if not L.transposed:
            gin = self.buf(('din', L.name), (N, H, W, cin_total), runtime.act_dtype())
            fuse = None if isinstance(g, Src) else self._stats_fusable(L, srcs, H, W, N, wpb, cfgb, cin_total)
            if fuse is not None:
                P, part = fuse
                engine.conv_forward([Src(g)], wpb, cin_total, cfgb, taps=L.taps, out=gin, H=H, W=W,
                                    bns=(srcs[0].x, P.scale, P.shift, P.save_mean, P.save_invstd, part))
                self._bn_partials[id(srcs[0].x)] = part
            else:
                engine.conv_forward([g if isinstance(g, Src) else Src(g)], wpb, cin_total, cfgb, taps=L.taps, out=gin, H=H, W=W)
        else:
            gin = self.buf(('din', L.name), (N, H, W, cin_total), runtime.act_dtype())
            views = [Src(g, view=(a * 2 * W * Cout, H, W, 2 * Cout, 4 * W * Cout)) for a in (0, 1)]
            engine.conv_forward(views, wpb, cin_total, cfgb, taps=(9 if L.kind == 'convT4' else 1), out=gin, H=H, W=W)
        coff = 0
        for s in srcs:
            if getattr(s, 'is_input', False):
                coff += s.C
                continue
            tgt, pool = getattr(s, 'grad_to', (s.x, int(s.pool)))
            add(tgt, _G(gin, H, W, oy=s.off[0], ox=s.off[1], pooled=pool, coff=coff, cstride=cin_total))
            coff += s.C

    def _overlap_begin(self):
        self._ar = None
        if not self._reduce_active() or os.environ.get('CDNET_ALLREDUCE_OVERLAP', '1') == '0':
            return
        f = self.flat
        base = f.G.data_ptr()
        pend = {}
        owners = [p for L in self.tape if not isinstance(L, runtime.FuseNode) for p in (L.weight, L.bias, None if L.bn is None else L.bn.weight,
                                                 None if L.bn is None else L.bn.bias) if p is not None]
        for p in owners:
            off = (p.grad.data_ptr() - base) // 4
            if 0 <= off < f.n_used:
                pend[off] = off + p.numel()
        if f.n_head:
            pend[0] = f.n_head
        self._ar = BucketReducer(f.G, f.n_used, self.bucket, pend)

    def _overlap_done(self, params):
        if self._ar is None:
            return
        if params is None:
            self._ar.done([0])
        else:
            base = self.flat.G.data_ptr()
            self._ar.done([(p.grad.data_ptr() - base) // 4 for p in params if p is not None])

    def _reduce_active(self):
        return self.world > 1 or os.environ.get('CDNET_FORCE_ALLREDUCE', '0') == '1'

    def allreduce_and_step(self):
        f = self.flat
        gscale = 1.0
        works = None
        if self._reduce_active():
            if self._ar is not None:
                ranges = self._ar.finish(wait=False)
                works = self._ar.works
                self.ar_stats = dict(buckets=len(works), released_during_backward=self._ar.early)
                self._ar = None
            else:
                bucketed_allreduce(f.G, f.n_used, self.bucket)
            gscale = 1.0 / self.world
        f.step_count += 1
        step = self._rule_stepper(gscale)
        if works is None:
            step(0, f.n_used)
        else:
            for w, (a, b) in zip(works, ranges):
                w.wait()
                step(a, b)
        runtime.WEIGHTS_EPOCH[0] += 1
        self._repack_all()

    def _rule_stepper(self, gscale):
        return optim.stepper(self, gscale)

    def _repack_all(self):
        f = self.flat
        lo, hi = f.P.data_ptr(), f.P.data_ptr() + f.P.numel() * 4
        if self._pack_jobs is not None and self._pack_prec != runtime.PRECISION:
            self._pack_jobs = None
        if self._pack_jobs is None:
            groups = ([], []), ([], [])
            for L in runtime.LAYERS:
                if not (lo <= L.weight.data_ptr() < hi):
                    continue
                w = L.weight.detach()
                if L.wp is not None and not L.wp_padded:
                    groups[0][0].append(engine.pack_job(w, L.cfg, L.pack_mode, L.wp, split=L.cfg_f32)); groups[0][1].append((L, 'wp_version'))
                if L.wpb is not None:
                    mode = (4 if L.kind == 'convT4' else 5) if L.transposed else (7 if L.kind == 'conv3s2' else 1)
                    groups[1][0].append(engine.pack_job(w, L.cfg_bwd, mode, L.wpb, split=L.cfg_f32)); groups[1][1].append((L, 'wpb_version'))
            if not groups[0][0] or not groups[1][0] or self.flat.step_count < 1:
                return
            self._pack_jobs = []
            self._pack_prec = runtime.PRECISION
            for jobs, owners in groups:
                arr = (engine.PackJob * len(jobs))(*jobs)
                nbytes = _lib.load().cdnet_pack_batch_table_bytes(len(jobs))
                table = torch.empty((nbytes,), dtype=torch.uint8, device=f.P.device)
                self._pack_jobs.append((arr, len(jobs), table, owners, [True]))
        side = self._side_stream()
        for k, (arr, n, table, owners, first) in enumerate(self._pack_jobs):
            if k == 1 and side is not None and self._packb_stream:
                ev = self._event('adam')
                ev.record()
                side.wait_event(ev)
                with _on_stream(side):
                    _lib.call('cdnet_pack_conv_weights_batch', C.byref(arr), n, _lib.ptr(table), table.numel(), int(first[0]), _lib.stream_ptr())
                    self._event('packb').record()
                self._packb_pending = True
            else:
                _lib.call('cdnet_pack_conv_weights_batch', C.byref(arr), n, _lib.ptr(table), table.numel(), int(first[0]), _lib.stream_ptr())
            first[0] = False
            for L, attr in owners:
                setattr(L, attr, (L.weight._version, runtime.WEIGHTS_EPOCH[0]))

    def write_bn_counters(self):
        with torch.no_grad():
            unused = tuple(getattr(self.model, 'UNUSED_PREFIXES', ()))
            for name, mod in self.model.named_modules():
                if isinstance(mod, torch.nn.BatchNorm2d) and mod.num_batches_tracked is not None and not (name + '.').startswith(unused or ('\0',)):
                    mod.num_batches_tracked.fill_(self._bn_base + self._forwards)

    def refresh_parameters(self):
        if hasattr(self.model, 'sync_real_parameters') and getattr(self.model, '_rt', None) is not None:
            self.model._ensure_runtime()
        runtime.WEIGHTS_EPOCH[0] += 1

# ... 130 lines not shown
```

include/cdnet_hip.h:

```cpp
#ifndef CDNET_HIP_H
#define CDNET_HIP_H

#include <stddef.h>
#include <stdint.h>

#ifdef __cplusplus
extern "C" {
#endif

#define CDNET_OK            0
#define CDNET_E_ARG         1
#define CDNET_E_WORKSPACE   2
#define CDNET_E_LAUNCH      3

#define CDNET_ABI_VERSION   5

int         cdnet_abi_version(void);
size_t      cdnet_abi_sizeof(const char *struct_name);
const char *cdnet_last_error(void);
const char *cdnet_build_info(void);
int         cdnet_spin(int microseconds, void *stream);
int         cdnet_box_copy(const void *src, void *dst, size_t bytes, void *stream);
int         cdnet_box_mfma(const uint32_t *seed, float *sink, unsigned long long *stamps, int workgroups, int waves_per_wg, int iters, void *stream);

size_t cdnet_tile_postproc_workspace_bytes(int B, int C, int H, int W);
int cdnet_tile_postproc(const float *mask_logits, const float *dir_logits, const float *point, int B, int C, int H, int W,
                        const int8_t *lut_host, int nbr, int extra_zero, int min_area, int radius, void *workspace, size_t workspace_bytes,
                        float *prob, uint8_t *dcm, int32_t *minmax, uint8_t *pred, uint8_t *fill, uint8_t *small, int32_t *label,
                        int32_t *final_, int32_t *counts, void *stream);

int cdnet_ddm_codes(const uint8_t *dcm, int N, int H, int W, int classes, const int8_t *lut_host, int nbr,
                    int extra_zero, uint8_t *code, int32_t *minmax, void *stream);
int cdnet_ddm_normalize(const uint8_t *code, const int32_t *minmax, int N, int H, int W, float *out,
                        void *stream);

int cdnet_probmaps(const float *mask_logits, const float *dir_logits, int N, int C, int H, int W,
                   float *prob, uint8_t *dcm, void *stream);

int cdnet_tta_boost_argmax(const float *probs, const float *points, const uint8_t *codes, const int32_t *minmax,
                           int I, int V, const int *view_xform_host, int H, int W,
                           float *prob_mean, float *point_mean, uint8_t *ddm16, uint8_t *pred,
                           float *pmax_ws, void *stream);

size_t cdnet_watershed_workspace_bytes(int N, int H, int W);
int cdnet_watershed_process(const uint8_t *pred, int N, int H, int W, int min_size, void *workspace, size_t workspace_bytes,
                            uint8_t *dist, int32_t *marker, int32_t *labels, void *stream);
int cdnet_fill_label_process(const uint8_t *pred, int N, int H, int W, int min_size, void *workspace, size_t workspace_bytes,
                             int32_t *labels, void *stream);
int cdnet_label_process(const uint8_t *pred, int N, int H, int W, int min_size, void *workspace, size_t workspace_bytes,
                        int32_t *labels, void *stream);

size_t cdnet_instance_redilate_workspace_bytes(int N, int H, int W, int cap);
int cdnet_instance_redilate(const int32_t *label, int N, int H, int W, int r, int cap, void *workspace, size_t workspace_bytes,
                            int32_t *out, int32_t *err_flag, void *stream);
int cdnet_instance_redilate_lds_rows(void);
int cdnet_instance_redilate_lds_cols(void);
int cdnet_label_count(const int32_t *lab, int N, int plane, int cap, int32_t *seen, int32_t *counts, int32_t *err_flag, void *stream);

size_t cdnet_cc_workspace_bytes(int N, int H, int W);
int cdnet_cc_chain(const uint8_t *pred, int fg_value, int N, int H, int W, int min_area, int radius,
                   void *workspace, size_t workspace_bytes,
                   uint8_t *fill, uint8_t *small, int32_t *label, int32_t *final_, int32_t *counts,
                   void *stream);

int cdnet_mask_views_argmax(const float *logits, int I, int V, int K, const int *view_xform_host, int H, int W, float *prob_mean,
                            uint8_t *pred, void *stream);
size_t cdnet_tile_mask_postproc_workspace_bytes(int B, int K, int H, int W);
int cdnet_tile_mask_postproc(const float *logits, int B, int K, int H, int W, int min_area, int radius, void *workspace, size_t workspace_bytes,
                             float *prob, uint8_t *pred, uint8_t *fill, uint8_t *small, int32_t *label, int32_t *final_, int32_t *counts,
                             void *stream);
int cdnet_dilate_labels(const int32_t *label, int N, int H, int W, int radius, int32_t *out, void *stream);


typedef struct cdnet_conv_src {
    const uint16_t *x;
    const uint16_t *res;
    const float *scale;
    const float *shift;
    int C;
    int Hs, Ws;
    int pool;
    int relu;
    int off_y, off_x;
    int f16;
    int row_stride;
} cdnet_conv_src;

typedef struct cdnet_conv_args {
    cdnet_conv_src src[2];
    int nsrc;
    const uint16_t *w;
    const float *bias;
    const float *oscale;
    const float *oshift;
    int orelu;
    uint16_t *out;
    int Cout, out_cstride, out_coff;
    float *stats;
    int N, H, W;
    int taps;
    int npar;
    int ostride;
    int nchunk;
    int tile, CK, BN;
    int out_f16;
    int debug;
    int ws;
    int f32;
    const uint16_t *eres;
    const float *eres_scale, *eres_shift;
    int eres_f16, eres_relu;
    int taps1;
    int pad_;
    uint16_t *pool_out;
    const float *dot_w;
    const float *dot_b;
    float *dot_out;
} cdnet_conv_args;

size_t cdnet_conv_packed_weight_elems(int Cout, int nchunk, int taps, int CK, int BN, int npar);
#define CDNET_PACK_SPLIT 16
int cdnet_pack_conv_weights(const float *w, void *packed, int Cout, int Cin, int KH, int KW, int CK, int BN, int mode,
                            void *stream);
int cdnet_pack_conv_weights_scaled(const float *w, const float *cout_scale, void *packed, int Cout, int Cin, int KH, int KW, int CK,
                                   int BN, int mode, void *stream);
typedef struct cdnet_pack_job {
    const float *w;
    void *packed;
    int Cout, Cin, KH, KW, CK, BN, mode, pad_;
} cdnet_pack_job;
size_t cdnet_pack_batch_table_bytes(int n_jobs);
int cdnet_pack_conv_weights_batch(const cdnet_pack_job *jobs, int n_jobs, void *table, size_t table_bytes, int upload,
                                  void *stream);
int cdnet_conv_forward(const cdnet_conv_args *args, void *stream);

typedef struct cdnet_dilated_conv_args {
    const void *in;
    const void *w;
    const float *scale;
    const float *shift;
    void *out;
    int N, H, W;
    int Cin, in_cstride;
    int Cout, out_cstride, out_coff;
    int taps, dilation;
    int leaky;
    float slope;
    int f32, out_nchw;
} cdnet_dilated_conv_args;
size_t cdnet_dilated_packed_weight_elems(int Cin, int Cout, int taps, int f32);
int cdnet_dilated_pack_weights(const float *w, void *packed, int Cin, int Cout, int taps, int f32, void *stream);
int cdnet_dilated_conv_forward(const cdnet_dilated_conv_args *args, void *stream);


typedef struct cdnet_dilated_bwd_data_args {
    const void *g;
    const void *w;
    void *dx;
    int N, H, W;
    int Cout, g_cstride;
    int Cin, dx_cstride, dx_coff;
    int taps, dilation;
    int accumulate;
    int f32;
} cdnet_dilated_bwd_data_args;
int cdnet_dilated_pack_weights_bwd(const float *w, void *packed, int Cin, int Cout, int taps, int f32, void *stream);
int cdnet_dilated_conv_backward_data(const cdnet_dilated_bwd_data_args *args, void *stream);

typedef struct cdnet_dilated_wgrad_args {
    const float *x;
    const float *g;
    float *dw;
    void *ws;
    size_t ws_bytes;
    int N, H, W;
    int Cin, x_cstride;
    int Cout, g_cstride;
    int taps, dilation;
} cdnet_dilated_wgrad_args;
size_t cdnet_dilated_wgrad_workspace_bytes(int N, int H, int W, int Cin, int Cout, int taps);
int cdnet_dilated_conv_backward_weight(const cdnet_dilated_wgrad_args *args, void *stream);

typedef struct cdnet_slice_bn_fwd_args {
    const float *z;
    float *out;
    const float *gamma, *beta;
    float *running_mean, *running_var;
    float *mean, *invstd;
    float *ws;
    size_t ws_floats;
    long long P;
    int C, z_cstride, out_cstride, out_coff;
    float eps, momentum, p_drop;
    int layer;
    unsigned long long key;
} cdnet_slice_bn_fwd_args;
typedef struct cdnet_slice_bn_bwd_args {
    const float *dy;
    const float *z;
    const float *mean, *invstd, *gamma;
    float *dgamma, *dbeta;
    float *g;
    float *ws;
    size_t ws_floats;
    long long P;
    int C, z_cstride, dy_cstride, dy_coff, g_cstride;
    float slope, p_drop;
    int layer;
    unsigned long long key;
} cdnet_slice_bn_bwd_args;
size_t cdnet_slice_bn_workspace_floats(long long P, int C);
int cdnet_slice_bn_train_forward(const cdnet_slice_bn_fwd_args *args, void *stream);
int cdnet_slice_bn_train_backward(const cdnet_slice_bn_bwd_args *args, void *stream);
int cdnet_dropout_mask(unsigned long long key, int layer, size_t count, float p_drop, uint8_t *mask, void *stream);

int cdnet_input_pack(const float *x, int N, int C, int H, int W, void *out_bf16_nhwc16, void *stream);
int cdnet_input_pack_f32(const float *x, int N, int C, int H, int W, float *out_f32_nhwc16, void *stream);
int cdnet_bn_fold_eval(const float *gamma, const float *beta, const float *running_mean, const float *running_var,
                       const float *conv_bias, float eps, int C, float *scale, float *shift, void *stream);
int cdnet_bn_finalize_train(const float *stats, int T, int C, float count, const float *gamma, const float *beta,
                            const float *conv_bias, float eps, float momentum, float *running_mean,
                            float *running_var, float *scale, float *shift, float *save_mean, float *save_invstd,
                            void *stream);

typedef struct cdnet_head_feat {
    const uint16_t *raw;
    const uint16_t *res;
    const float *scale;
    const float *shift;
    int relu;
    int f16;
} cdnet_head_feat;

#define CDNET_HEAD_WEIGHT_FLOATS 855
int cdnet_dam_head_forward(const cdnet_head_feat *f1, const cdnet_head_feat *f2, const cdnet_head_feat *f3,
                           const float *head_weights, int N, int H, int W, float *mask, float *point,
                           float *direction, void *stream);
int cdnet_final_conv1x1(const cdnet_head_feat *f, const float *w, const float *b, int K, int N, int H, int W,
                        float *out, void *stream);
size_t cdnet_bias_grad_workspace_floats(int C);
int cdnet_bias_grad(const uint16_t *grad_out, size_t npix, int C, float *workspace, size_t workspace_floats, float *db, void *stream);
int cdnet_bias_grad_f32(const float *grad_out, size_t npix, int C, float *workspace, size_t workspace_floats, float *db, void *stream);
size_t cdnet_final_conv1x1_backward_workspace_floats(void);
int cdnet_final_conv1x1_backward(const cdnet_head_feat *f, const float *w, const float *dlogits, int K, int N, int H, int W,
                                 uint16_t *df, float *workspace, size_t workspace_floats, float *dw, float *db, void *stream);

int cdnet_conv_ws_eligible(const cdnet_conv_args *args);

int cdnet_src_materialize(const cdnet_conv_src *src, int N, int H, int W, uint16_t *out, void *stream);

size_t cdnet_conv_wgrad_slab_floats(int C_src, int Cout, int taps, int npar, int ci_tiles, int ksplit);
int cdnet_conv_backward_weight(const cdnet_conv_src *src, int src_coff, int Csrc_real, int Cin_real,
                               const uint16_t *grad_out, int Cout, int N, int H, int W, int taps, int npar,
                               int ostride, int ci_tiles, int ksplit, float *slab, float *dw, int mode, void *stream);

#define CDNET_WGRAD_FAMILY_GEN  1
#define CDNET_WGRAD_FAMILY_WS   2
#define CDNET_WGRAD_FAMILY_F32  3
#define CDNET_WGRAD_FAMILY_WS32 4
int cdnet_conv_backward_weight_last_form(void);

#define CDNET_WGRAD_DEFER_REDUCE 0x100
typedef struct cdnet_wgrad_reduce_desc {
    const float *slab;
    float *dw;
    int ksplit, npar, ci_blocks, co_blocks, taps, CI, CO, Csrc_real, Cin_real, src_coff, Cout, mode;
    int block0, blocks;
} cdnet_wgrad_reduce_desc;
int cdnet_wgrad_reduce_desc_fill(int C_src, int src_coff, int Csrc_real, int Cin_real, int Cout, int taps, int npar, int ci_tiles,
                                 int ksplit, const float *slab, float *dw, int mode, int block0, cdnet_wgrad_reduce_desc *out);
int cdnet_wgrad_reduce_batch(const cdnet_wgrad_reduce_desc *table_dev, int n, int total_blocks, void *stream);

typedef struct cdnet_grad_in {
    const uint16_t *g;
    int Hg, Wg;
    int oy, ox;
    int pooled;
    int coff, cstride;
    int pad_;
} cdnet_grad_in;

typedef struct cdnet_bn_bwd_args {
    const uint16_t *raw;
    const uint16_t *res;
    const float *scale, *shift;
    const float *mean, *invstd;
    cdnet_grad_in gin[3];
    int ngin;
    int f16, relu;
    int N, H, W, C;
} cdnet_bn_bwd_args;

size_t cdnet_bn_backward_workspace_floats(int C);
int cdnet_bn_backward_stats(const cdnet_bn_bwd_args *args, const float *gamma, float *dgamma, float *dbeta, float *workspace,
                            size_t workspace_floats, float *ktab, void *stream);
int cdnet_bn_backward_apply(const cdnet_bn_bwd_args *args, const float *ktab, uint16_t *draw, void *stream);
int cdnet_bn_backward_finalize(const cdnet_bn_bwd_args *args, const float *gamma, float *dgamma, float *dbeta, const float *partial,
                               int nb, float *ktab, void *stream);
int cdnet_bn_backward(const cdnet_bn_bwd_args *args, const float *gamma, float *dgamma, float *dbeta, float *workspace,
                      size_t workspace_floats, uint16_t *draw, uint16_t *dz_out, void *stream);

size_t cdnet_dam_head_backward_workspace_floats(int N, int H, int W);
int cdnet_dam_head_backward(const cdnet_head_feat *f1, const cdnet_head_feat *f2, const cdnet_head_feat *f3,
                            const float *head_weights, const float *dmask, const float *dpoint, const float *ddir,
                            int N, int H, int W, uint16_t *df1, uint16_t *df2, uint16_t *df3, float *workspace,
                            size_t workspace_floats, float *dhead_weights, void *stream);
int cdnet_dam_head_backward_fused_blocks(void);
int cdnet_dam_head_backward_fused_scratch_bytes(void);
size_t cdnet_dam_head_backward_fused_workspace_floats(void);
int cdnet_dam_head_backward_fused(const cdnet_head_feat *f1, const cdnet_head_feat *f2, const cdnet_head_feat *f3,
                                  const float *head_weights, const float *dmask, const float *dpoint, const float *ddir, int N, int H,
                                  int W, float *df1, float *df2, float *dz3, float *workspace, size_t workspace_floats,
                                  float *dhead_weights, void *stream);

size_t cdnet_dam_loss_workspace_floats(int B, int P);
int cdnet_dam_loss(const float *mask, const float *point, const float *direction, const uint8_t *label,
                   const uint8_t *dirlab, const uint16_t *point_target_f16, const uint8_t *weight_u8, int B, int H, int W,
                   int quirk_sample0, float *workspace, size_t workspace_floats, float *losses, float *dmask,
                   float *dpoint, float *ddir, void *stream);
size_t cdnet_dam_loss_classes_workspace_floats(int B, int P, int direction_classes);
int cdnet_dam_loss_classes(const float *mask, const float *point, const float *direction, const uint8_t *label,
                           const uint8_t *dirlab, const uint16_t *point_target_f16, const uint8_t *weight_u8, int B, int H, int W,
                           int direction_classes, int quirk_sample0, float *workspace, size_t workspace_floats, float *losses,
                           float *dmask, float *dpoint, float *ddir, void *stream);

#define CDNET_LOSS_WMAP 1u
#define CDNET_LOSS_CE   2u
#define CDNET_LOSS_DICE 4u

int cdnet_dam_loss_terms(const float *mask, const float *point, const float *direction, const uint8_t *label,
                         const uint8_t *dirlab, const uint16_t *point_target_f16, const uint8_t *weight_u8, int B, int H, int W,
                         int direction_classes, int quirk_sample0, float *workspace, size_t workspace_floats, float *losses,
                         float *dmask, float *dpoint, float *ddir, void *stream, unsigned terms);

size_t cdnet_mask_loss_workspace_floats(int B, int P);
int cdnet_mask_loss(const float *mask_logits, const uint8_t *label, const uint8_t *weight_u8, int B, int H, int W, unsigned terms,
                    float *workspace, size_t workspace_floats, float *losses, float *dmask, void *stream);

size_t cdnet_variance_loss_workspace_bytes(int B, int K, int H, int W);
int cdnet_variance_loss(const float *mask_logits, const uint8_t *label, int fg_value, int B, int K, int H, int W, float alpha,
                        void *workspace, size_t workspace_bytes, float *loss_var, float *total, float *dmask, int32_t *root_out,
                        int32_t *counts, void *stream);

size_t cdnet_boundary_loss_workspace_bytes(int kind, int B, int K, int H, int W);
int cdnet_boundary_loss(const float *mask_logits, const uint8_t *label, int kind, int B, int K, int H, int W, float beta,
                        void *workspace, size_t workspace_bytes, float *loss_out, float *total, float *dmask, void *stream);
int cdnet_boundary_loss_scratch_bytes(void);

#define CDNET_VAL_SUMS 42
size_t cdnet_dam_val_sums_workspace_floats(int B, int P);
int cdnet_dam_val_sums(const float *mask, const float *point, const float *dirn, const uint8_t *label, const uint8_t *dirlab,
                       const uint16_t *point_target_f16, const uint8_t *weight_u8, const int *dir_rank_host, int B, int H, int W,
                       float *workspace, size_t workspace_floats, float *sums, void *stream);
size_t cdnet_dam_val_sums_classes_workspace_floats(int B, int P, int direction_classes);
int cdnet_dam_val_sums_classes(const float *mask, const float *point, const float *dirn, const uint8_t *label, const uint8_t *dirlab,
                               const uint16_t *point_target_f16, const uint8_t *weight_u8, const int *dir_rank_host,
                               int direction_classes, int B, int H, int W, float *workspace, size_t workspace_floats, float *sums,
                               void *stream);

int cdnet_adam_step(float *param, const float *grad, float *exp_avg, float *exp_avg_sq, size_t n, float lr, float beta1,
                    float beta2, float eps, float weight_decay, int step, float grad_scale, void *stream);

int cdnet_moment_step(float *param, const float *grad, float *exp_avg, float *exp_avg_sq, float *slow, size_t n, double beta1,
                      double beta2, float grad_scale, int move, int rect, float decay, float step_size, float v_div, float eps,
                      int sync, float alpha, void *stream);
int cdnet_sgd_step(float *param, const float *grad, float *momentum_buffer, size_t n, float lr, float momentum, float weight_decay,
                   int step, float grad_scale, void *stream);

int cdnet_window_pack(const float *img, int C, int H, int W, int view_xform, int tile_h, int tile_w, int stride, int ny,
                      int nx, void *out_bf16_nhwc16, void *stream);
int cdnet_window_pack_f32(const float *img, int C, int H, int W, int view_xform, int tile_h, int tile_w, int stride, int ny,
                          int nx, float *out_f32_nhwc16, void *stream);
int cdnet_window_stitch(const float *tiles, int K, int tile_h, int tile_w, int stride, int overlap, int ny, int nx, int Hv,
                        int Wv, float *out, void *stream);

typedef struct cdnet_aug_sample {
    double minv[6];
    const uint8_t *img;
    const uint8_t *weight;
    const void *label;
    int32_t H, W, img_stride, weight_stride, label_stride, label_i32;
    float color[4];
    int32_t hflip, vflip, filter, y0, x0;
    float alpha, sigma;
    uint32_t seed;
} cdnet_aug_sample;
size_t cdnet_augment_workspace_bytes(int B, int size, int max_radius);
int cdnet_augment_batch(const cdnet_aug_sample *samples, const cdnet_aug_sample *samples_host, int B, int size, const float *norm_host,
                        void *workspace, size_t workspace_bytes, float *image, uint8_t *weight, void *label, int label_i32, int32_t *varied,
                        float *field, void *stream);

typedef struct cdnet_aug_geo {
    double paff[6];
    double rinv[6];
    int32_t Hr, Wr, fy0, fx0;
    uint32_t flags;
    int32_t reserved;
} cdnet_aug_geo;
size_t cdnet_augment_geo_workspace_bytes(int B, int size, int max_radius, int field_edge);
int cdnet_augment_batch_geo(const cdnet_aug_sample *samples, const cdnet_aug_sample *samples_host, const cdnet_aug_geo *geo,
                            const cdnet_aug_geo *geo_host, int field_edge, int B, int size, const float *norm_host, void *workspace,
                            size_t workspace_bytes, float *image, uint8_t *weight, void *label, int label_i32, int32_t *varied, float *field,
                            void *stream);

size_t cdnet_label_encoding_workspace_bytes(int N, int H, int W, int max_instances);
int cdnet_label_encoding(const uint8_t *label_ch0, int N, int H, int W, int max_instances, const double *rays_host,
                         const double *gauss_host, void *workspace, size_t workspace_bytes, uint8_t *label3,
                         uint16_t *point_f16, uint8_t *direction, int32_t *inst_out, int32_t *counts_out, void *stream);
size_t cdnet_label_encoding_instances_workspace_bytes(int N, int H, int W, int max_instances);
int cdnet_label_encoding_instances(const int32_t *label_inst, int N, int H, int W, int max_instances, const double *rays_host,
                                   const double *gauss_host, void *workspace, size_t workspace_bytes, uint8_t *label3,
                                   uint16_t *point_f16, uint8_t *direction, int32_t *inst, int32_t *counts, void *stream);

typedef struct cdnet_fuse_term {
    const uint16_t *x;
    int Hs, Ws;
    const float *scale;
    const float *shift;
    int f16, pad_;
} cdnet_fuse_term;
int cdnet_fuse_sum(const cdnet_fuse_term *terms, int nterm, int N, int H, int W, int C, int relu, uint16_t *out, int out_cstride,
                   int out_coff, void *stream);

int cdnet_upsample_bilinear_backward(const uint16_t *dout, int N, int H, int W, int C, int dout_cstride, int dout_coff, int Hs, int Ws,
                                     uint16_t *din, void *stream);
int cdnet_s2d_to_nhwc(const uint16_t *in, int N, int H2, int W2, int C, uint16_t *out, void *stream);
int cdnet_fuse_sum_f32(const cdnet_fuse_term *terms, int nterm, int N, int H, int W, int C, int relu, float *out, int out_cstride,
                       int out_coff, void *stream);
int cdnet_upsample_bilinear_backward_f32(const float *dout, int N, int H, int W, int C, int dout_cstride, int dout_coff, int Hs, int Ws,
                                         float *din, void *stream);
int cdnet_s2d_to_nhwc_f32(const float *in, int N, int H2, int W2, int C, float *out, void *stream);

typedef struct cdnet_grad_term {
    const uint16_t *g;
    int cstride, coff;
} cdnet_grad_term;
int cdnet_grad_sum(const cdnet_grad_term *terms, int nterm, const uint16_t *mask, long long npix, int C, uint16_t *out, void *stream);
int cdnet_grad_sum_f32(const cdnet_grad_term *terms, int nterm, const float *mask, long long npix, int C, float *out, void *stream);

int cdnet_label_pair_histogram(const int32_t *true_lab, const int32_t *pred_lab, int N, int plane, int cap, int hash_slots,
                               int32_t *area_true, int32_t *area_pred, uint32_t *hash_keys, int32_t *hash_counts, int32_t *err_flag,
                               void *stream);
int cdnet_remap_label(const int32_t *lab, int N, int plane, int cap, int32_t *scratch, int32_t *out, int32_t *err_flag, void *stream);
int cdnet_label_areas(const int32_t *lab, int N, int plane, int cap, int32_t *area, int32_t *err_flag, void *stream);
int cdnet_label_apply(const int32_t *lab, int N, int plane, int cap, const int32_t *lut, int32_t *out, void *stream);

size_t cdnet_label_csr_workspace_bytes(int cap);
int cdnet_label_csr(const int32_t *lab, int H, int W, int cap, void *workspace, size_t workspace_bytes, int32_t *tab, int32_t *pix,
                    int32_t *bpix, int32_t *err_flag, void *stream);
int cdnet_hausdorff_tile_pixels(void);
int cdnet_hausdorff_chunk_pixels(void);
int cdnet_hausdorff_pairs(const int32_t *true_lab, const int32_t *true_tab, const int32_t *true_pix, const int32_t *true_bpix,
                          const int32_t *pred_lab, const int32_t *pred_tab, const int32_t *pred_pix, const int32_t *pred_bpix, int H, int W,
// ... 11 lines not shown
```

Baseline: 1097.

## Batch BN partial-sum loads, write bias grad in-kernel, pack split weights per thread

When there are many partial rows, the BN partial-sum reduction now issues eight strided loads per thread before accumulating, which raises memory-level parallelism in the finalize kernels. The BN backward finalize now writes dbeta a second time into the following 1x1 conv's bias grad, so the separate device copy in Python is dropped. The split weight pack now lets one thread emit both the hi and lo bf16 images, which halves the work items and changes the grid sizing. Env-var toggles and a debug entry point are added to restore the old serial paths.

Result: no change. 1105 (median of 6 runs) (+0.7%).

```diff
diff --git a/cdnet_amd/_lib.py b/cdnet_amd/_lib.py
--- a/cdnet_amd/_lib.py
+++ b/cdnet_amd/_lib.py
@@ -120,6 +120,8 @@
     'cdnet_wgrad_reduce_batch': (_i, [_vp, _i, _i, _vp]),
     'cdnet_bn_backward_workspace_floats': (_sz, [_i]),
     'cdnet_bn_backward': (_i, [_vp, _vp, _vp, _vp, _vp, _sz, _vp, _vp, _vp]),
+    'cdnet_bn_backward_dbeta2': (_i, [_vp, _vp, _vp, _vp, _vp, _vp, _sz, _vp, _vp, _vp]),
+    'cdnet_debug_bn_sums_serial': (_i, [_i]),
     'cdnet_dam_head_backward_workspace_floats': (_sz, [_i, _i, _i]),
     'cdnet_dam_head_backward': (_i, [_vp] * 7 + [_i, _i, _i, _vp, _vp, _vp, _vp, _sz, _vp, _vp]),
     'cdnet_dam_head_backward_fused_blocks': (_i, []),
diff --git a/cdnet_amd/csrc/bn_bwd.hip b/cdnet_amd/csrc/bn_bwd.hip
--- a/cdnet_amd/csrc/bn_bwd.hip
+++ b/cdnet_amd/csrc/bn_bwd.hip
@@ -532,14 +532,16 @@
     if (!APPLY) bn_write_partial<8>(A.partial, A.C, VPP, s1, s2);
 }
 
+template <bool GROUPED>
 __global__ __launch_bounds__(256) void bn_bwd_finalize_kernel(const float *__restrict__ partial, int nb, int C, float M, const float *gamma,
-                                                              const float *invstd, float *dgamma, float *dbeta, float *k1, float *k2,
-                                                              float *k3) {
+                                                              const float *invstd, float *dgamma, float *dbeta, float *dbeta2, float *k1,
+                                                              float *k2, float *k3) {
     const int c = blockIdx.x;
     double s1, s2;
-    bn_sum_partials(partial, nb, C, c, s1, s2);
+    bn_sum_partials<GROUPED>(partial, nb, C, c, s1, s2);
     if (threadIdx.x == 0) {
         if (dbeta) dbeta[c] = (float)s1;
+        if (dbeta2) dbeta2[c] = (float)s1;
         if (dgamma) dgamma[c] = (float)s2;
         k1[c] = gamma[c] * invstd[c];
         k2[c] = (float)(s1 / M);
@@ -647,9 +649,10 @@
     }
 }
 
-static void bn_finalize(const BnBwdArgs &A, const float *partial, int nb, const float *gamma, float *dgamma, float *dbeta, float *k,
-                        hipStream_t st) {
-    bn_bwd_finalize_kernel<<<A.C, 256, 0, st>>>(partial, nb, A.C, (float)bn_npix(A), gamma, A.invstd, dgamma, dbeta, k, k + A.C, k + 2 * A.C);
+static void bn_finalize(const BnBwdArgs &A, const float *partial, int nb, const float *gamma, float *dgamma, float *dbeta, float *dbeta2,
+                        float *k, hipStream_t st) {
+    auto *kern = bn_sums_grouped(nb) ? bn_bwd_finalize_kernel<true> : bn_bwd_finalize_kernel<false>;
+    kern<<<A.C, 256, 0, st>>>(partial, nb, A.C, (float)bn_npix(A), gamma, A.invstd, dgamma, dbeta, dbeta2, k, k + A.C, k + 2 * A.C);
 }
 
 static void bn_set_coeffs(BnBwdArgs &A, const float *k) { A.k1 = k; A.k2 = k + A.C; A.k3 = k + 2 * A.C; }
@@ -663,8 +666,8 @@
     return B;
 }
 
-extern "C" int cdnet_bn_backward(const cdnet_bn_bwd_args *a, const float *gamma, float *dgamma, float *dbeta, float *workspace,
-                                 size_t workspace_floats, uint16_t *draw, uint16_t *dz_out, void *stream) {
+static int bn_backward(const cdnet_bn_bwd_args *a, const float *gamma, float *dgamma, float *dbeta, float *dbeta2, float *workspace,
+                       size_t workspace_floats, uint16_t *draw, uint16_t *dz_out, void *stream) {
     BnBwdArgs A;
     int rc = fill_bn_args(a, A, "cdnet_bn_backward");
     if (rc) return rc;
@@ -685,12 +688,29 @@
         A.dz_out = dz_reuse ? dz_out : nullptr;
         float *k = workspace + (size_t)P.nb * 2 * A.C;
         launch<false>(P, A, st);
-        bn_finalize(A, A.partial, P.nb, gamma, dgamma, dbeta, k, st);
+        bn_finalize(A, A.partial, P.nb, gamma, dgamma, dbeta, dbeta2, k, st);
         bn_set_coeffs(A, k);
     }
     A.dz_out = dz_out;
     launch<true>(P, reuse ? bn_dz_as_source(A, dz_out) : A, st);
     return check_launch("cdnet_bn_backward");
+}
+
+extern "C" int cdnet_bn_backward(const cdnet_bn_bwd_args *a, const float *gamma, float *dgamma, float *dbeta, float *workspace,
+                                 size_t workspace_floats, uint16_t *draw, uint16_t *dz_out, void *stream) {
+    return bn_backward(a, gamma, dgamma, dbeta, nullptr, workspace, workspace_floats, draw, dz_out, stream);
+}
+
+extern "C" int cdnet_bn_backward_dbeta2(const cdnet_bn_bwd_args *a, const float *gamma, float *dgamma, float *dbeta, float *dbeta2,
+                                        float *workspace, size_t workspace_floats, uint16_t *draw, uint16_t *dz_out, void *stream) {
+    CDNET_REQUIRE(a && a->mean && dbeta2, "cdnet_bn_backward_dbeta2: needs a BatchNorm layer (mean) and the second destination");
+    return bn_backward(a, gamma, dgamma, dbeta, dbeta2, workspace, workspace_floats, draw, dz_out, stream);
+}
+
+extern "C" int cdnet_debug_bn_sums_serial(int serial) {
+    const int old = bn_sums_serial();
+    bn_sums_serial() = serial ? 1 : 0;
+    return old;
 }
 
 static bool bn_plain_case(const BnBwdArgs &A, bool masked = false) {
@@ -715,7 +735,7 @@
     A.rev = 0;
     bn_ktab_copy_kernel<<<cdiv(A.C, 256), 256, 0, st>>>(A.scale, A.shift, A.mean, A.invstd, A.C, ktab);
     launch<false>(P, A, st);
-    bn_finalize(A, A.partial, P.nb, gamma, dgamma, dbeta, ktab + 4 * A.C, st);
+    bn_finalize(A, A.partial, P.nb, gamma, dgamma, dbeta, nullptr, ktab + 4 * A.C, st);
     return check_launch("cdnet_bn_backward_stats");
 }
 
@@ -725,7 +745,7 @@
     int rc = fill_bn_args(a, A, "cdnet_bn_backward_finalize");
     if (rc) return rc;
     CDNET_REQUIRE(bn_plain_case(A) && gamma && partial && ktab && nb >= 1, "cdnet_bn_backward_finalize: plain case only");
-    bn_finalize(A, partial, nb, gamma, dgamma, dbeta, ktab + 4 * A.C, (hipStream_t)stream);
+    bn_finalize(A, partial, nb, gamma, dgamma, dbeta, nullptr, ktab + 4 * A.C, (hipStream_t)stream);
     return check_launch("cdnet_bn_backward_finalize");
 }
 
diff --git a/cdnet_amd/csrc/bn_sums.h b/cdnet_amd/csrc/bn_sums.h
--- a/cdnet_amd/csrc/bn_sums.h
+++ b/cdnet_amd/csrc/bn_sums.h
@@ -1,15 +1,39 @@
 #pragma once
 #include <hip/hip_runtime.h>
+#include <stdlib.h>
 
 namespace cdnet {
 
+constexpr int BN_SUMS_FEW_ROWS = 1024;
+
+template <int G>
+__device__ __forceinline__ void bn_sum_rows_grouped(const float *__restrict__ part, int T, int C, int c, int lane, double &s, double &q) {
+    for (int t0 = lane; t0 < T; t0 += 256 * G) {
+        float vs[G], vq[G];
+#pragma unroll
+        for (int u = 0; u < G; ++u) {
+            const int t = min(t0 + u * 256, T - 1);
+            vs[u] = part[((size_t)t * 2) * C + c];
+            vq[u] = part[((size_t)t * 2 + 1) * C + c];
+        }
+#pragma unroll
+        for (int u = 0; u < G; ++u)
+            if (t0 + u * 256 < T) { s += (double)vs[u]; q += (double)vq[u]; }
+    }
+}
+
+template <bool GROUPED>
 __device__ __forceinline__ void bn_sum_partials(const float *__restrict__ part, int T, int C, int c, double &s, double &q) {
     __shared__ double s_s[256], s_q[256];
     const int lane = threadIdx.x;
     s = 0.0; q = 0.0;
-    for (int t = lane; t < T; t += 256) {
-        s += (double)part[((size_t)t * 2) * C + c];
-        q += (double)part[((size_t)t * 2 + 1) * C + c];
+    if (!GROUPED) {
+        for (int t = lane; t < T; t += 256) {
+            s += (double)part[((size_t)t * 2) * C + c];
+            q += (double)part[((size_t)t * 2 + 1) * C + c];
+        }
+    } else {
+        bn_sum_rows_grouped<8>(part, T, C, c, lane, s, q);
     }
     s_s[lane] = s; s_q[lane] = q;
     __syncthreads();
@@ -21,4 +45,11 @@
     s = s_s[0]; q = s_q[0];
 }
 
+inline int &bn_sums_serial() {
+    static int v = getenv("CDNET_BN_SUMS_SERIAL") ? atoi(getenv("CDNET_BN_SUMS_SERIAL")) : 0;
+    return v;
 }
+
+inline bool bn_sums_grouped(int T) { return !bn_sums_serial() && T > BN_SUMS_FEW_ROWS; }
+
+}
diff --git a/cdnet_amd/csrc/conv.hip b/cdnet_amd/csrc/conv.hip
--- a/cdnet_amd/csrc/conv.hip
+++ b/cdnet_amd/csrc/conv.hip
@@ -27,7 +27,10 @@
     unsigned short *__restrict__ out = d.out;
     const int Cout = d.Cout, Cin = d.Cin, KH = d.KH, KW = d.KW, CK = d.CK, BN = d.BN, nchunk = d.nchunk, TAPS = d.TAPS, mode = d.mode,
               parity = d.parity;
-    const size_t total = (size_t)d.ntile * nchunk * TAPS * (CK / 16) * 2 * BN * (d.split ? 2 : 1);
+    const int nimg = d.split ? 2 : 1;
+    const bool both = d.split == 1;
+    const size_t total = (size_t)d.ntile * nchunk * TAPS * (CK / 16) * 2 * BN * (both ? 1 : nimg);
+    const size_t img_vecs = (size_t)TAPS * (CK / 16) * 2 * BN;
     for (size_t i = first; i < total; i += stride) {
         size_t r = i;
         int tap = r % TAPS; r /= TAPS;
@@ -35,12 +38,12 @@
         int half = r % 2; r /= 2;
         int kc = r % (CK / 16); r /= (CK / 16);
         int hl = 0;
-        if (d.split) { hl = r % 2; r /= 2; }
+        if (d.split == 2) { hl = r % 2; r /= 2; }
         int chunk = r % nchunk; r /= nchunk;
         int tile = (int)r;
         int co = tile * BN + col;
-        const size_t ovec = ((((((size_t)tile * nchunk + chunk) * (d.split ? 2 : 1) + hl) * TAPS + tap) * (CK / 16) + kc) * 2 + half) * BN + col;
-        unsigned short o8[8];
+        const size_t ovec = ((((((size_t)tile * nchunk + chunk) * nimg + hl) * TAPS + tap) * (CK / 16) + kc) * 2 + half) * BN + col;
+        unsigned short o8[8], l8[8];
 #pragma unroll
         for (int j = 0; j < 8; ++j) {
         int ci = chunk * CK + kc * 16 + half * 8 + j;
@@ -81,12 +84,19 @@
         }
         if (d.scale && co < Cout) v *= d.scale[co];
         const unsigned short hi = f2bf(v);
-        o8[j] = hl ? f2bf(v - bf2f(hi)) : hi;
+        l8[j] = d.split ? f2bf(v - bf2f(hi)) : (unsigned short)0;
+        o8[j] = hl ? l8[j] : hi;
         }
         uint4 ov;
         ov.x = o8[0] | ((unsigned)o8[1] << 16); ov.y = o8[2] | ((unsigned)o8[3] << 16);
         ov.z = o8[4] | ((unsigned)o8[5] << 16); ov.w = o8[6] | ((unsigned)o8[7] << 16);
         reinterpret_cast<uint4 *>(out)[ovec] = ov;
+        if (both) {
+            uint4 lv;
+            lv.x = l8[0] | ((unsigned)l8[1] << 16); lv.y = l8[2] | ((unsigned)l8[3] << 16);
+            lv.z = l8[4] | ((unsigned)l8[5] << 16); lv.w = l8[6] | ((unsigned)l8[7] << 16);
+            reinterpret_cast<uint4 *>(out)[ovec + img_vecs] = lv;
+        }
     }
 }
 
@@ -1263,7 +1273,8 @@
 
 static int fill_pack_desc(PackDesc &d, const float *w, void *packed, int Cout, int Cin, int KH, int KW, int CK, int BN, int mode, int p,
                           const char *who) {
-    const int split = (mode & 16) ? 1 : 0;
+    static const int two_env = getenv("CDNET_PACK_TWO_THREADS") ? atoi(getenv("CDNET_PACK_TWO_THREADS")) : 0;
+    const int split = (mode & 16) ? (((mode & 32) || two_env) ? 2 : 1) : 0;
     mode &= 15;
     CDNET_REQUIRE(w && packed, "%s: null pointer", who);
     CDNET_REQUIRE(CK % 16 == 0 && BN % 32 == 0 && Cin % CK == 0 && mode >= 0 && mode <= 7, "%s: Cin=%d CK=%d BN=%d mode=%d", who, Cin, CK, BN, mode);
@@ -1276,7 +1287,8 @@
     d.Cout = Cout; d.Cin = Cin; d.KH = KH; d.KW = KW; d.CK = CK; d.BN = BN; d.nchunk = nchunk; d.ntile = ntile; d.TAPS = taps; d.mode = mode;
     d.parity = p;
     d.block0 = 0;
-    d.nblocks = (unsigned)((per + 2047) / 2048);
+    const size_t items = per / (split == 1 ? 16 : 8);
+    d.nblocks = (unsigned)((items + 255) / 256);
     if (d.nblocks > 4096) d.nblocks = 4096;
     return CDNET_OK;
 }
diff --git a/cdnet_amd/csrc/dilated_train.hip b/cdnet_amd/csrc/dilated_train.hip
--- a/cdnet_amd/csrc/dilated_train.hip
+++ b/cdnet_amd/csrc/dilated_train.hip
@@ -201,10 +201,11 @@
     }
 }
 
+template <bool GROUPED>
 __global__ __launch_bounds__(256) void bn_bwd_final_kernel(const float *__restrict__ part, int T, int C, float *dgamma, float *dbeta) {
     const int c = blockIdx.x;
     double s, q;
-    bn_sum_partials(part, T, C, c, s, q);
+    bn_sum_partials<GROUPED>(part, T, C, c, s, q);
     if (threadIdx.x == 0) {
         dbeta[c] = (float)s;
         dgamma[c] = (float)q;
@@ -342,7 +343,7 @@
     const float ks = 1.f / (1.f - A.p_drop);
     bn_tile_sums_kernel<true><<<dim3((unsigned)G.T, (unsigned)cdiv(A.C, 32)), 256, 0, st>>>(A.z, A.z_cstride, A.dy, A.dy_cstride, A.dy_coff, A.mean,
                                                                                            A.invstd, A.P, A.C, G.tile, lkey, thr, ks, A.ws);
-    bn_bwd_final_kernel<<<A.C, 256, 0, st>>>(A.ws, G.T, A.C, A.dgamma, A.dbeta);
+    (bn_sums_grouped(G.T) ? bn_bwd_final_kernel<true> : bn_bwd_final_kernel<false>)<<<A.C, 256, 0, st>>>(A.ws, G.T, A.C, A.dgamma, A.dbeta);
     const size_t total = (size_t)A.P * A.C;
     bn_bwd_apply_kernel<<<lin_grid(total, 8192), 256, 0, st>>>(A.z, A.z_cstride, A.dy, A.dy_cstride, A.dy_coff, A.mean, A.invstd, A.gamma, A.dgamma,
                                                           A.dbeta, total, A.C, 1.f / (float)A.P, A.slope, lkey, thr, ks, A.g, A.g_cstride);
diff --git a/cdnet_amd/csrc/model.hip b/cdnet_amd/csrc/model.hip
--- a/cdnet_amd/csrc/model.hip
+++ b/cdnet_amd/csrc/model.hip
@@ -52,6 +52,7 @@
     shift[c] = b[c] + ((bias ? bias[c] : 0.f) - rm[c]) * s;
 }
 
+template <bool GROUPED>
 __global__ __launch_bounds__(256) void bn_finalize_train_kernel(const float *__restrict__ stats, int T, int C, float count,
                                                                 const float *g, const float *b, const float *bias,
                                                                 float eps, float momentum, float *rm, float *rv,
@@ -59,7 +60,7 @@
                                                                 float *invstd_out) {
     const int c = blockIdx.x;
     double s, q;
-    bn_sum_partials(stats, T, C, c, s, q);
+    bn_sum_partials<GROUPED>(stats, T, C, c, s, q);
     if (threadIdx.x == 0) {
         double mean = s / count;
         double var = q / count - mean * mean;
@@ -836,9 +837,9 @@
                                        float *running_var, float *scale, float *shift, float *save_mean,
                                        float *save_invstd, void *stream) {
     CDNET_REQUIRE(stats && gamma && beta && scale && shift && T > 0 && C > 0 && count > 0, "cdnet_bn_finalize_train: bad args");
-    bn_finalize_train_kernel<<<C, 256, 0, (hipStream_t)stream>>>(stats, T, C, count, gamma, beta, conv_bias, eps, momentum,
-                                                                         running_mean, running_var, scale, shift, save_mean,
-                                                                         save_invstd);
+    auto *kern = bn_sums_grouped(T) ? bn_finalize_train_kernel<true> : bn_finalize_train_kernel<false>;
+    kern<<<C, 256, 0, (hipStream_t)stream>>>(stats, T, C, count, gamma, beta, conv_bias, eps, momentum, running_mean, running_var, scale, shift,
+                                             save_mean, save_invstd);
     return check_launch("cdnet_bn_finalize_train");
 }
 
diff --git a/cdnet_amd/models/dam/model_unet_rev1.py b/cdnet_amd/models/dam/model_unet_rev1.py
--- a/cdnet_amd/models/dam/model_unet_rev1.py
+++ b/cdnet_amd/models/dam/model_unet_rev1.py
@@ -60,6 +60,7 @@
         self.c2 = ConvLayer(name + '.conv2', 'conv3', m.conv2.weight, None, m.bn2)
         self.cr = ConvLayer(name + '.conv_1x1', 'conv1', m.conv_1x1.weight, m.conv_1x1.bias, None)
         self.cr.bias_grad_from = self.c2
+        self.c2.bias_grad_to = self.cr
 
     def layers(self):
         return [self.c1, self.c2, self.cr]
diff --git a/cdnet_amd/runtime.py b/cdnet_amd/runtime.py
--- a/cdnet_amd/runtime.py
+++ b/cdnet_amd/runtime.py
@@ -84,6 +84,8 @@
         self.node_relu, self.node_res = True, None
         self.needs_input_grad = True
         self.bias_grad_from = None
+        self.bias_grad_to = None
+        self.bias_grad_written = False
         self.wpb, self.wpb_version, self.cfg_bwd = None, None, None
         self.wp_padded = False
         LAYERS.add(self)
diff --git a/cdnet_amd/trainer.py b/cdnet_amd/trainer.py
--- a/cdnet_amd/trainer.py
+++ b/cdnet_amd/trainer.py
@@ -461,8 +461,8 @@
         draw = self.buf(('draw', L.name), (No, Ho, Wo, Co), runtime.act_dtype())
         ws = self._ws('bn', _lib.load().cdnet_bn_backward_workspace_floats(Co))
         bn = L.bn
-        _lib.call('cdnet_bn_backward', C.byref(a), _lib.ptr(bn.weight.detach()), _lib.ptr(bn.weight.grad), _lib.ptr(bn.bias.grad),
-                  _lib.ptr(ws), ws.numel(), _lib.ptr(draw), None, _lib.stream_ptr())
+        self._call_bn_backward(L, a, _lib.ptr(bn.weight.detach()), _lib.ptr(bn.weight.grad), _lib.ptr(bn.bias.grad),
+                               _lib.ptr(ws), ws.numel(), _lib.ptr(draw), None, _lib.stream_ptr())
         add(L.node_res, _G(g.t, Ho, Wo))
         return draw
 
@@ -513,6 +513,16 @@
         a.N, a.H, a.W, a.C = out.shape
         return a
 
+    @staticmethod
+    def _call_bn_backward(L, a, gamma, dgamma, dbeta, *rest):
+        to = getattr(L, 'bias_grad_to', None)
+        if to is None:
+            _lib.call('cdnet_bn_backward', C.byref(a), gamma, dgamma, dbeta, *rest)
+            return
+        assert L.bn is not None and to.bias_grad_from is L, (L.name, to.name)
+        _lib.call('cdnet_bn_backward_dbeta2', C.byref(a), gamma, dgamma, dbeta, _lib.ptr(to.bias.grad), *rest)
+        to.bias_grad_written = True
+
     def _bn_backward(self, L, out, gl, add):
         No, Ho, Wo, Co = out.shape
         res = getattr(L, 'node_res', None)
@@ -531,9 +541,9 @@
             dz = self.buf(('dz', L.name), (No, Ho, Wo, Co), runtime.act_dtype())
         ws = self._ws('bn', _lib.load().cdnet_bn_backward_workspace_floats(Co))
         bn = L.bn
-        _lib.call('cdnet_bn_backward', C.byref(a), _lib.ptr(bn.weight.detach()) if has_bn else None,
-                  _lib.ptr(bn.weight.grad) if has_bn else None, _lib.ptr(bn.bias.grad) if has_bn else None,
-                  _lib.ptr(ws), ws.numel(), _lib.ptr(draw), _lib.ptr(dz), _lib.stream_ptr())
+        self._call_bn_backward(L, a, _lib.ptr(bn.weight.detach()) if has_bn else None,
+                               _lib.ptr(bn.weight.grad) if has_bn else None, _lib.ptr(bn.bias.grad) if has_bn else None,
+                               _lib.ptr(ws), ws.numel(), _lib.ptr(draw), _lib.ptr(dz), _lib.stream_ptr())
         if res is not None:
             add(getattr(L, 'node_res_grad_to', None) if getattr(L, 'node_res_grad_to', None) is not None else res, _G(dz, Ho, Wo))
             L.node_res_grad_to = None
@@ -586,7 +596,8 @@
         if L.bias is not None and L.bn is None:
             owner = getattr(L, 'bias_grad_from', None)
             if owner is not None:
-                L.bias.grad.copy_(owner.bn.bias.grad)
+                assert owner.bias_grad_to is L and L.bias_grad_written, L.name
+                L.bias_grad_written = False
             else:
                 ws = self._ws('slab', lib.cdnet_bias_grad_workspace_floats(Cout), side=True)
                 _lib.call(_lib.entry('cdnet_bias_grad', g.dtype == torch.float32), _lib.ptr(g), g.numel() // Cout, Cout,
diff --git a/include/cdnet_hip.h b/include/cdnet_hip.h
--- a/include/cdnet_hip.h
+++ b/include/cdnet_hip.h
@@ -120,6 +120,7 @@
 
 size_t cdnet_conv_packed_weight_elems(int Cout, int nchunk, int taps, int CK, int BN, int npar);
 #define CDNET_PACK_SPLIT 16
+#define CDNET_PACK_TWO_THREADS 32
 int cdnet_pack_conv_weights(const float *w, void *packed, int Cout, int Cin, int KH, int KW, int CK, int BN, int mode,
                             void *stream);
 int cdnet_pack_conv_weights_scaled(const float *w, const float *cout_scale, void *packed, int Cout, int Cin, int KH, int KW, int CK,
@@ -299,6 +300,9 @@
                                int nb, float *ktab, void *stream);
 int cdnet_bn_backward(const cdnet_bn_bwd_args *args, const float *gamma, float *dgamma, float *dbeta, float *workspace,
                       size_t workspace_floats, uint16_t *draw, uint16_t *dz_out, void *stream);
+int cdnet_bn_backward_dbeta2(const cdnet_bn_bwd_args *args, const float *gamma, float *dgamma, float *dbeta, float *dbeta2,
+                             float *workspace, size_t workspace_floats, uint16_t *draw, uint16_t *dz_out, void *stream);
+int cdnet_debug_bn_sums_serial(int serial);
 
 size_t cdnet_dam_head_backward_workspace_floats(int N, int H, int W);
 int cdnet_dam_head_backward(const cdnet_head_feat *f1, const cdnet_head_feat *f2, const cdnet_head_feat *f3,
```
